# magicat777/Audio-Analyzer-OMEGA

Measured on NVIDIA B200. Metric: stream-seconds of 48 kHz stereo analysed/sec (multi-res FFT+LUFS+TP), higher is better.
Workload: dtype f32 (FFT, combine, K-weighting in a float32 delta-form state, sample peaks of the true-peak meter; its four transforms per frame pair in f16x2; tensor-core GEMM on (hi, lo) half operands with fp32 accumulators for the few-bin resolutions) + f64 (meter statistics)

## Files before the change

### audio-analyzer-omega_b200/csrc/blockdft_tc_kernel.cuh

```cuda
#pragma once
#include <cuda_runtime.h>
#include <cuda_fp16.h>
#include <stdint.h>

namespace o4 {

#ifndef TC_F16
#define TC_F16 1
#endif
constexpr int TC_BM = 128;
constexpr int TC_BN = 256;
constexpr int TC_KC = TC_F16 ? 32 : 16;
constexpr float TC_LO_SCALE = 2048.f;
constexpr int TC_STAGES = 3;
constexpr int TC_TMEM_COLS = 2 * TC_BN;
constexpr int TC_MAX_GROUPS = 64;
#ifndef TC_EXPERIMENT_KS
#define TC_EXPERIMENT_KS 2
#endif
#define TC_PG TC_STAGES
constexpr int TC_THREADS = 64 * TC_STAGES;
constexpr int TC_WARP_MMA = TC_THREADS / 32;
constexpr int TC_WARP_B = TC_WARP_MMA + 1;
constexpr int TC_WARP_EPI = TC_WARP_MMA + 2;
constexpr int TC_EPI_WARPS = 8;
constexpr int TC_CTA_THREADS = 32 * (TC_WARP_EPI + TC_EPI_WARPS);
static_assert(TC_WARP_EPI % 4 == 0, "epilogue warp w must own TMEM lane quarter w % 4");
constexpr int TC_A_BYTES = TC_BM * 64;
constexpr int TC_B_BYTES = TC_BN * 64;
constexpr int TC_STAGE_BYTES = 2 * TC_A_BYTES + 2 * TC_B_BYTES;
constexpr int TC_XROW = 17;
constexpr int TC_SPAD = 15;
constexpr int TC_STRIP_BYTES = (128 + 2 * TC_SPAD) * TC_XROW * 8;

struct BlockDftTcArgs {
    const float* x;
    long long ch_stride;
    int hop;
    int n_ch;
    int j0, nb;
    int n_halves;
    int n_tiles;
    const uint8_t* Eimg;
    const float* row_inv;
    float e_inv;
    float* Q;
    int qs;
    float2* X;
    int n_frames;
    int nkx;
    short gB[TC_MAX_GROUPS];
    short gX[TC_MAX_GROUPS];
    short gN[TC_MAX_GROUPS];
    short gS[TC_MAX_GROUPS];
};
#ifdef TC_TIMELINE
__device__ long long tc_tl[64][16];
#define TC_STAMP(cond, i) do { if ((cond) && (blockIdx.x & 3) == 0 && (blockIdx.x >> 2) < 64) tc_tl[blockIdx.x >> 2][i] = clock64(); } while (0)
#else
#define TC_STAMP(cond, i) do { } while (0)
#endif

__host__ __device__ __forceinline__ int tc_sw64_offset(int row, int c) {
    return (row >> 3) * 512 + (row & 7) * 64 + ((c ^ ((row >> 1) & 3)) << 4);
}

__device__ __forceinline__ uint32_t tc_smem_u32(const void* p) { return (uint32_t)__cvta_generic_to_shared(p); }

__device__ __forceinline__ void tc_mbar_init(uint64_t* bar, int count) {
    asm volatile("mbarrier.init.shared::cta.b64 [%0], %1;" ::"r"(tc_smem_u32(bar)), "r"(count) : "memory");
}
__device__ __forceinline__ void tc_mbar_expect_tx(uint64_t* bar, uint32_t bytes) {
    asm volatile("mbarrier.arrive.expect_tx.shared::cta.b64 _, [%0], %1;" ::"r"(tc_smem_u32(bar)), "r"(bytes) : "memory");
}
__device__ __forceinline__ void tc_mbar_wait(uint64_t* bar, uint32_t parity) {
    const uint32_t a = tc_smem_u32(bar);
    uint32_t done = 0;
    while (!done) {
        asm volatile(
            "{\n\t.reg .pred p;\n\t"
            "mbarrier.try_wait.parity.shared::cta.b64 p, [%1], %2;\n\t"
            "selp.u32 %0, 1, 0, p;\n\t}"
            : "=r"(done) : "r"(a), "r"(parity) : "memory");
    }
}
__device__ __forceinline__ void tc_bulk_g2s(void* dst, const void* src, uint32_t bytes, uint64_t* bar) {
    asm volatile("cp.async.bulk.shared::cluster.global.mbarrier::complete_tx::bytes [%0], [%1], %2, [%3];"
                 ::"r"(tc_smem_u32(dst)), "l"(src), "r"(bytes), "r"(tc_smem_u32(bar)) : "memory");
}

__device__ __forceinline__ uint64_t tc_desc_sw64(uint32_t smem_addr) {
    uint64_t d = 0;
    d |= (uint64_t)((smem_addr >> 4) & 0x3FFF);
    d |= (uint64_t)1 << 16;
    d |= (uint64_t)(512 >> 4) << 32;
    d |= (uint64_t)1 << 46;
    d |= (uint64_t)4 << 61;
    return d;
}

constexpr uint32_t TC_FMT = TC_F16 ? 0u : 2u;
constexpr uint32_t TC_IDESC = (1u << 4) | (TC_FMT << 7) | (TC_FMT << 10) | ((uint32_t)(TC_BN >> 3) << 17) | ((128u >> 4) << 24);

__device__ __forceinline__ void tc_mma(uint32_t tmem_d, uint64_t da, uint64_t db, uint32_t accumulate) {
    asm volatile(
        "{\n\t.reg .pred p;\n\t"
        "setp.ne.b32 p, %4, 0;\n\t"
#if TC_F16
        "tcgen05.mma.cta_group::1.kind::f16 [%0], %1, %2, %3, p;\n\t}"
#else
        "tcgen05.mma.cta_group::1.kind::tf32 [%0], %1, %2, %3, p;\n\t}"
#endif

        ::"r"(tmem_d), "l"(da), "l"(db), "r"(TC_IDESC), "r"(accumulate) : "memory");
}
__device__ __forceinline__ void tc_commit(uint64_t* bar) {
    asm volatile("tcgen05.commit.cta_group::1.mbarrier::arrive::one.shared::cluster.b64 [%0];" ::"r"(tc_smem_u32(bar)) : "memory");
}

__device__ __forceinline__ void tc_tmem_ld32(uint32_t taddr, uint32_t (&v)[32]) {
    asm volatile(
        "tcgen05.ld.sync.aligned.32x32b.x32.b32 "
        "{%0, %1, %2, %3, %4, %5, %6, %7, %8, %9, %10, %11, %12, %13, %14, %15, "
        "%16, %17, %18, %19, %20, %21, %22, %23, %24, %25, %26, %27, %28, %29, %30, %31}, [%32];"
        : "=r"(v[0]), "=r"(v[1]), "=r"(v[2]), "=r"(v[3]), "=r"(v[4]), "=r"(v[5]), "=r"(v[6]), "=r"(v[7]),
          "=r"(v[8]), "=r"(v[9]), "=r"(v[10]), "=r"(v[11]), "=r"(v[12]), "=r"(v[13]), "=r"(v[14]), "=r"(v[15]),
          "=r"(v[16]), "=r"(v[17]), "=r"(v[18]), "=r"(v[19]), "=r"(v[20]), "=r"(v[21]), "=r"(v[22]), "=r"(v[23]),
          "=r"(v[24]), "=r"(v[25]), "=r"(v[26]), "=r"(v[27]), "=r"(v[28]), "=r"(v[29]), "=r"(v[30]), "=r"(v[31])
        : "r"(taddr) : "memory");
}

__device__ __forceinline__ void tc_mbar_arrive(uint64_t* bar) {
    asm volatile("mbarrier.arrive.shared::cta.b64 _, [%0];" ::"r"(tc_smem_u32(bar)) : "memory");
}

__device__ __forceinline__ void tc_split_h2(float a0, float a1, uint32_t& hi, uint32_t& lo) {
    const __half2 h = __floats2half2_rn(a0, a1);
    const float2 hf = __half22float2(h);
    const __half2 l = __floats2half2_rn((a0 - hf.x) * TC_LO_SCALE, (a1 - hf.y) * TC_LO_SCALE);
    hi = *reinterpret_cast<const uint32_t*>(&h);
    lo = *reinterpret_cast<const uint32_t*>(&l);
}
__device__ __forceinline__ float tc_acc(uint32_t v, uint32_t c, float rs) {
#if TC_F16
    return fmaf(__uint_as_float(c), 1.f / TC_LO_SCALE, __uint_as_float(v)) * rs;
#else
    return __uint_as_float(v) + __uint_as_float(c);
#endif
}
__device__ __forceinline__ float hop_row_scale(float m) {
    int e = (int)((__float_as_uint(m) >> 23) & 0xffu);
    float inv = 1.f;
    if (m > 0.f && e < 255) {
        e = e > 250 ? 250 : e;
        inv = __uint_as_float((uint32_t)(e + 1) << 23);
    }
    return inv;
}
struct HopScaleArgs { const float* x; long long ch_stride; int hop, n_ch, j0, nb, ncols; float* inv; };
__global__ void __launch_bounds__(256)
hopblock_scale_kernel(const HopScaleArgs a) {
    const int lane = threadIdx.x & 31;
    const long long row = (long long)blockIdx.x * 8 + (threadIdx.x >> 5);
    if (row >= (long long)a.n_ch * a.ncols) return;
    const int ch = (int)(row / a.ncols), j = (int)(row % a.ncols);
    const float4* px = reinterpret_cast<const float4*>(a.x + (long long)ch * a.ch_stride + ((long long)a.j0 + j) * a.hop);
    float m = 0.f;
    for (int i = lane; i < a.hop / 4; i += 32) {
        const float4 v = __ldg(px + i);
        m = fmaxf(fmaxf(m, fmaxf(fabsf(v.x), fabsf(v.y))), fmaxf(fabsf(v.z), fabsf(v.w)));
    }
#pragma unroll
    for (int o = 16; o > 0; o >>= 1) m = fmaxf(m, __shfl_xor_sync(0xffffffffu, m, o));
    if (lane == 0) a.inv[(size_t)ch * a.nb + j] = hop_row_scale(m);
}


template <int B>
__device__ __forceinline__ void tc_frame_sums(const BlockDftTcArgs& a, const float2* S, int r, int row0, int ch, int nbin, int xb0,
                                              int shift = -1) {
    constexpr int PER = 16 / B;
#pragma unroll
    for (int task = 0; task < 2; ++task) {
        if (task == 1 && r >= B - 1) break;
        const int R = task == 0 ? r : 128 + r;
        const long long f = (long long)a.j0 + row0 + R + (shift > 0 ? shift : 0);
        if (f < 0 || f >= a.n_frames) continue;
        const bool whole = (R - B + 1 >= 0) && (R <= 127) && shift < 0;
        const float2* Sf = S + (R - B + 1 + TC_SPAD) * TC_XROW;
#pragma unroll
        for (int q = 0; q < PER; ++q) {
            if (q >= nbin) break;
            float2 u[B];
#pragma unroll
            for (int b = 0; b < B; ++b) u[b] = Sf[b * TC_XROW + q * B + b];
#pragma unroll
            for (int w = B / 2; w > 0; w >>= 1)
#pragma unroll
                for (int b = 0; b < w; ++b) { u[b].x += u[b + w].x; u[b].y += u[b + w].y; }
            float2* dst = a.X + ((size_t)ch * a.nkx + xb0 + q) * a.n_frames + f;
            if (whole) *dst = u[0];
            else { atomicAdd(&dst->x, u[0].x); atomicAdd(&dst->y, u[0].y); }
        }
    }
}

__global__ void __launch_bounds__(TC_CTA_THREADS, 1)
blockdft_tc_kernel(const __grid_constant__ BlockDftTcArgs a) {
    extern __shared__ __align__(16) uint8_t tc_smem_raw[];
    uint8_t* tiles = tc_smem_raw + ((1024u - (tc_smem_u32(tc_smem_raw) & 1023u)) & 1023u);
    float2* S_all = reinterpret_cast<float2*>(tiles + TC_STAGES * TC_STAGE_BYTES);
    uint64_t* bar_a = reinterpret_cast<uint64_t*>(tiles + TC_STAGES * TC_STAGE_BYTES + (TC_EPI_WARPS / 4) * TC_STRIP_BYTES);
    uint64_t* bar_b = bar_a + TC_STAGES;
    uint64_t* bar_m = bar_b + TC_STAGES;
    uint64_t* bar_full = bar_m + TC_STAGES;
    uint64_t* bar_empty = bar_full + 1;
    uint32_t* tmem_slot = reinterpret_cast<uint32_t*>(bar_empty + 1);

    const int tid = threadIdx.x, warp = tid >> 5, lane = tid & 31;
    const int tiles_per_ch = (a.nb + TC_BM - 1) / TC_BM;
    const int n_kc = a.hop / TC_KC;

    if (warp == TC_WARP_B && lane == 0) {
        for (int s = 0; s < TC_STAGES; ++s) {
            tc_mbar_init(bar_a + s, TC_THREADS / 32 / TC_PG); tc_mbar_init(bar_b + s, 1); tc_mbar_init(bar_m + s, 1);
        }
        tc_mbar_init(bar_full, 1);
        tc_mbar_init(bar_empty, TC_EPI_WARPS);
        asm volatile("fence.mbarrier_init.release.cluster;" ::: "memory");
    }
    if (warp == 0) {
        __syncwarp();
        asm volatile("tcgen05.alloc.cta_group::1.sync.aligned.shared::cta.b32 [%0], %1;" ::"r"(tc_smem_u32(tmem_slot)), "n"(TC_TMEM_COLS) : "memory");
        asm volatile("tcgen05.relinquish_alloc_permit.cta_group::1.sync.aligned;" ::: "memory");
    }
    asm volatile("tcgen05.fence::before_thread_sync;" ::: "memory");
    __syncthreads();
    asm volatile("tcgen05.fence::after_thread_sync;" ::: "memory");
    const uint32_t tmem = *tmem_slot;

    if (warp == TC_WARP_B) {
        if (lane == 0) {
            int kcg = 0;
            for (int tile = blockIdx.x; tile < a.n_tiles; tile += gridDim.x) {
                const uint8_t* eimg = a.Eimg + (size_t)(tile % a.n_halves) * n_kc * 2 * TC_B_BYTES;
                for (int kb = 0; kb < n_kc; ++kb, ++kcg) {
                    const int sb = kcg % TC_STAGES;
                    if (kcg >= TC_STAGES) tc_mbar_wait(bar_m + sb, (uint32_t)(kcg / TC_STAGES - 1) & 1);
#ifdef TC_EXPERIMENT_B_DIV
                    tc_mbar_expect_tx(bar_b + sb, 2 * TC_B_BYTES / TC_EXPERIMENT_B_DIV);
                    tc_bulk_g2s(tiles + sb * TC_STAGE_BYTES + 2 * TC_A_BYTES, eimg + (size_t)kb * 2 * TC_B_BYTES, 2 * TC_B_BYTES / TC_EXPERIMENT_B_DIV, bar_b + sb);
#else
                    tc_mbar_expect_tx(bar_b + sb, 2 * TC_B_BYTES);
                    tc_bulk_g2s(tiles + sb * TC_STAGE_BYTES + 2 * TC_A_BYTES, eimg + (size_t)kb * 2 * TC_B_BYTES, 2 * TC_B_BYTES, bar_b + sb);
#endif
                }
            }
        }
    } else if (warp == TC_WARP_MMA) {
        if (lane == 0) {
            int kcg = 0, it = 0;
            for (int tile = blockIdx.x; tile < a.n_tiles; tile += gridDim.x, ++it) {
                TC_STAMP(it == 1, 0);
                TC_STAMP(it == 2, 6);
                if (it > 0) {
                    tc_mbar_wait(bar_empty, (uint32_t)(it - 1) & 1);
                    asm volatile("tcgen05.fence::after_thread_sync;" ::: "memory");
                }
                for (int kc = 0; kc < n_kc; ++kc, ++kcg) {
                    const int s = kcg % TC_STAGES;
                    const uint32_t use = (uint32_t)(kcg / TC_STAGES);
                    tc_mbar_wait(bar_a + s, use & 1);
                    tc_mbar_wait(bar_b + s, use & 1);
                    asm volatile("tcgen05.fence::after_thread_sync;" ::: "memory");
                    TC_STAMP(it == 1 && kc == 0, 1);
                    const uint32_t sa = tc_smem_u32(tiles + s * TC_STAGE_BYTES);
#pragma unroll
                    for (int ks = 0; ks < TC_EXPERIMENT_KS; ++ks) {
                        const uint64_t d_ahi = tc_desc_sw64(sa + ks * 32);
                        const uint64_t d_alo = tc_desc_sw64(sa + TC_A_BYTES + ks * 32);
                        const uint64_t d_bhi = tc_desc_sw64(sa + 2 * TC_A_BYTES + ks * 32);
                        const uint64_t d_blo = tc_desc_sw64(sa + 2 * TC_A_BYTES + TC_B_BYTES + ks * 32);
                        tc_mma(tmem, d_ahi, d_bhi, (kc | ks) != 0);
                        tc_mma(tmem + TC_BN, d_ahi, d_blo, (kc | ks) != 0);
                        tc_mma(tmem + TC_BN, d_alo, d_bhi, 1);
                    }
                    tc_commit(bar_m + s);
                }
                tc_commit(bar_full);
                TC_STAMP(it == 1, 2);
            }
        }
    } else if (warp < TC_WARP_MMA) {
        constexpr int PGT = TC_THREADS / TC_PG;
        constexpr int NQ = TC_BM * 4 / PGT;
        constexpr int PF4 = TC_F16 ? 2 : 1;
        const int pg = tid / PGT, tg = tid % PGT;
        int a_off[NQ];
#pragma unroll
        for (int q = 0; q < NQ; ++q) a_off[q] = tc_sw64_offset((tg + PGT * q) >> 2, (tg + PGT * q) & 3);
        int it = 0;
        for (int tile = blockIdx.x; tile < a.n_tiles; tile += gridDim.x, ++it) {
            const int bid = tile / a.n_halves;
            const int row0 = (bid % tiles_per_ch) * TC_BM;
            const int ch = bid / tiles_per_ch;
            const float* xa = a.x + (long long)ch * a.ch_stride + (long long)a.j0 * a.hop;
            const float4* a_src[NQ];
            float sc[NQ];
#pragma unroll
            for (int q = 0; q < NQ; ++q) {
                const int p = tg + PGT * q;
                int r = row0 + (p >> 2);
                if (r >= a.nb) r = a.nb - 1;
                a_src[q] = reinterpret_cast<const float4*>(xa + (long long)r * a.hop) + (p & 3) * PF4;
#if TC_F16
                sc[q] = __ldg(a.row_inv + (size_t)ch * a.nb + r);
#else
                sc[q] = 1.f;
#endif
            }
#if TC_F16
#pragma unroll
            for (int q = 0; q < NQ; ++q) sc[q] = __uint_as_float(0x7F000000u - __float_as_uint(sc[q]));
#endif
            const int kcg0 = it * n_kc;
            for (int kc = ((pg - kcg0) % TC_PG + TC_PG) % TC_PG; kc < n_kc; kc += TC_PG) {
                const int kcg = kcg0 + kc;
                const int s = kcg % TC_STAGES;
                uint8_t* st = tiles + s * TC_STAGE_BYTES;
                float4 cur[NQ][PF4];
#ifndef TC_EXPERIMENT_NO_LDG
#pragma unroll
                for (int q = 0; q < NQ; ++q)
#pragma unroll
                    for (int h = 0; h < PF4; ++h) cur[q][h] = __ldg(a_src[q] + kc * (TC_KC / 4) + h);
#else
#pragma unroll
                for (int q = 0; q < NQ; ++q)
#pragma unroll
                    for (int h = 0; h < PF4; ++h) cur[q][h] = make_float4(0.f, 0.f, 0.f, 0.f);
#endif
                if (kcg >= TC_STAGES) tc_mbar_wait(bar_m + s, (uint32_t)(kcg / TC_STAGES - 1) & 1);
#pragma unroll
                for (int q = 0; q < NQ; ++q) {
#if TC_F16
                    uint4 hi, lo;
                    tc_split_h2(cur[q][0].x * sc[q], cur[q][0].y * sc[q], hi.x, lo.x);
                    tc_split_h2(cur[q][0].z * sc[q], cur[q][0].w * sc[q], hi.y, lo.y);
                    tc_split_h2(cur[q][1].x * sc[q], cur[q][1].y * sc[q], hi.z, lo.z);
                    tc_split_h2(cur[q][1].z * sc[q], cur[q][1].w * sc[q], hi.w, lo.w);
                    *reinterpret_cast<uint4*>(st + a_off[q]) = hi;
                    *reinterpret_cast<uint4*>(st + TC_A_BYTES + a_off[q]) = lo;
#else
                    float4 hi, lo;
                    hi.x = __uint_as_float(__float_as_uint(cur[q][0].x) & 0xFFFFE000u); lo.x = cur[q][0].x - hi.x;
                    hi.y = __uint_as_float(__float_as_uint(cur[q][0].y) & 0xFFFFE000u); lo.y = cur[q][0].y - hi.y;
                    hi.z = __uint_as_float(__float_as_uint(cur[q][0].z) & 0xFFFFE000u); lo.z = cur[q][0].z - hi.z;
                    hi.w = __uint_as_float(__float_as_uint(cur[q][0].w) & 0xFFFFE000u); lo.w = cur[q][0].w - hi.w;
                    *reinterpret_cast<float4*>(st + a_off[q]) = hi;
                    *reinterpret_cast<float4*>(st + TC_A_BYTES + a_off[q]) = lo;
#endif
                }
                asm volatile("fence.proxy.async.shared::cta;" ::: "memory");
                __syncwarp();
                if (lane == 0) tc_mbar_arrive(bar_a + s);
            }
        }
    } else {
        const int quad = warp & 3, grp = (warp - TC_WARP_EPI) >> 2;
        const int r = quad * 32 + lane;
        constexpr int NCG = TC_BN / 32 / (TC_EPI_WARPS / 4);
        const uint32_t taddr0 = tmem + ((uint32_t)(quad * 32) << 16) + (uint32_t)(grp * NCG * 32);
        float2* S = S_all + grp * (TC_STRIP_BYTES / 8);
        for (int i = (tid - TC_WARP_EPI * 32) & 127; i < TC_SPAD * TC_XROW; i += 128) {
            S[i] = make_float2(0.f, 0.f);
            S[(128 + TC_SPAD) * TC_XROW + i] = make_float2(0.f, 0.f);
        }
        int it = 0;
        for (int tile = blockIdx.x; tile < a.n_tiles; tile += gridDim.x, ++it) {
            const int half = tile % a.n_halves;
            const int bid = tile / a.n_halves;
            const int row0 = (bid % tiles_per_ch) * TC_BM;
            const int ch = bid / tiles_per_ch;
            const int row = row0 + r;
            float rs = 1.f;
#if TC_F16
            rs = __ldg(a.row_inv + (size_t)ch * a.nb + (row < a.nb ? row : a.nb - 1)) * a.e_inv;
#endif
            float* qrow = a.X ? nullptr : a.Q + ((size_t)ch * a.nb + (row < a.nb ? row : 0)) * a.qs + half * TC_BN;
            tc_mbar_wait(bar_full, (uint32_t)it & 1);
            asm volatile("tcgen05.fence::after_thread_sync;" ::: "memory");
            TC_STAMP(it == 1 && tid == TC_WARP_EPI * 32, 3);
            uint32_t v[32], c[32];
            tc_tmem_ld32(taddr0, v);
            tc_tmem_ld32(taddr0 + TC_BN, c);
#pragma unroll 1
            for (int cg = 0; cg < NCG; ++cg) {
                TC_STAMP(it == 1 && cg == 2 && tid == TC_WARP_EPI * 32, 8);
                asm volatile("tcgen05.wait::ld.sync.aligned;" ::: "memory");
                TC_STAMP(it == 1 && cg == 2 && tid == TC_WARP_EPI * 32, 9);
                const int gi = half * (TC_BN / 32) + grp * NCG + cg;
                const int B = a.X ? a.gB[gi] : 0;
#ifdef TC_EXPERIMENT_NO_EPI
                const bool live = false;
#else
                const bool live = B > 0;
#endif
                if (a.X) {
                    if (live) {
#pragma unroll
                        for (int i = 0; i < 16; ++i)
                            S[(r + TC_SPAD) * TC_XROW + i] = make_float2(tc_acc(v[2 * i], c[2 * i], rs), tc_acc(v[2 * i + 1], c[2 * i + 1], rs));
                    }
                } else if (row < a.nb) {
                    float4* dst = reinterpret_cast<float4*>(qrow + (grp * NCG + cg) * 32);
#pragma unroll
                    for (int i = 0; i < 8; ++i)
                        dst[i] = make_float4(tc_acc(v[4 * i], c[4 * i], rs), tc_acc(v[4 * i + 1], c[4 * i + 1], rs),
                                             tc_acc(v[4 * i + 2], c[4 * i + 2], rs), tc_acc(v[4 * i + 3], c[4 * i + 3], rs));
                }
                TC_STAMP(it == 1 && cg == 2 && tid == TC_WARP_EPI * 32, 10);
                if (cg + 1 < NCG) {
                    tc_tmem_ld32(taddr0 + (uint32_t)((cg + 1) * 32), v);
                    tc_tmem_ld32(taddr0 + (uint32_t)(TC_BN + (cg + 1) * 32), c);
                } else {
                    asm volatile("tcgen05.fence::before_thread_sync;" ::: "memory");
                    __syncwarp();
                    if (lane == 0) tc_mbar_arrive(bar_empty);
                    TC_STAMP(it == 1 && tid == TC_WARP_EPI * 32, 4);
                }
                if (a.X) {
                    TC_STAMP(it == 1 && cg == 2 && tid == TC_WARP_EPI * 32, 11);
                    asm volatile("bar.sync %0, 128;" ::"r"(grp + 1) : "memory");
                    TC_STAMP(it == 1 && cg == 2 && tid == TC_WARP_EPI * 32, 12);
                    if (live) {
                        const int nbin = a.gN[gi], xb0 = a.gX[gi];
                        if (B == 16) tc_frame_sums<16>(a, S, r, row0, ch, nbin, xb0, a.gS[gi]);
                        else if (B == 8) tc_frame_sums<8>(a, S, r, row0, ch, nbin, xb0);
                        else if (B == 4) tc_frame_sums<4>(a, S, r, row0, ch, nbin, xb0);
                        else tc_frame_sums<2>(a, S, r, row0, ch, nbin, xb0);
                    }
                    TC_STAMP(it == 1 && cg == 2 && tid == TC_WARP_EPI * 32, 13);
                    asm volatile("bar.sync %0, 128;" ::"r"(grp + 1) : "memory");
                    TC_STAMP(it == 1 && cg == 2 && tid == TC_WARP_EPI * 32, 14);
                }
            }
            TC_STAMP(it == 1 && tid == TC_WARP_EPI * 32, 5);
        }
    }
    asm volatile("tcgen05.fence::before_thread_sync;" ::: "memory");
    __syncthreads();
    if (warp == 0)
        asm volatile("tcgen05.dealloc.cta_group::1.sync.aligned.b32 %0, %1;" ::"r"(tmem), "n"(TC_TMEM_COLS) : "memory");
}

inline size_t blockdft_tc_smem_bytes() { return (size_t)TC_STAGES * TC_STAGE_BYTES + (TC_EPI_WARPS / 4) * TC_STRIP_BYTES + (3 * TC_STAGES + 2) * 8 + 16 + 1024; }

}
```

### audio-analyzer-omega_b200/csrc/kweight32_kernel.cuh

```cuda
#pragma once
#include <cuda_runtime.h>
#include "kweight_kernel.cuh"
#include "blockdft_tc_kernel.cuh"

namespace o4 {

struct Kw32Sec {
    float b0, a2, gamma, bb;
    float phi[5][4];
    float c16[4], c17[4];
    float g[KW_SUBMAX][2];
    float2 ga0[16], ga1[16];
};

struct Kweight32Args {
    const float* x;
    long long ch_stride, frame_stride, frame_off0;
    int n_ch, n_frames, first_frame, frames_per_warp;
    const float* hann;
    double* lufs_out;
    int rms_gate, _align;
    float* hop_inv;
    int hop_inv_nb, hop_inv_j0;
    Kw32Sec s[2];
};

__device__ __forceinline__ float2 kw32_mat(const float* m, float2 s) {
    return make_float2(fmaf(m[0], s.x, m[1] * s.y), fmaf(m[2], s.x, m[3] * s.y));
}

struct Kw32R { float r0; float2 a[16]; float2 b[16]; };

__device__ __forceinline__ float& kwr(Kw32R& q, int i) {
    if (i == 0) return q.r0;
    if (i <= 16) return q.a[i - 1].x;
    if (i <= 32) return q.b[i - 17].x;
    if (i <= 48) return q.b[i - 33].y;
    return q.a[i - 49].y;
}
__device__ __forceinline__ float2 bc2(float v) { return make_float2(v, v); }

template <bool BACKWARD>
__device__ __forceinline__ void kw32_pass(Kw32R& q, const Kw32Sec& c, int lane) {
    const int pos = BACKWARD ? 31 - lane : lane;
    const float b0 = c.b0, a2 = c.a2, ngamma = -c.gamma, bb = c.bb;
    float xa_in, dxa_in;
    {
        const float p1 = BACKWARD ? __shfl_down_sync(0xffffffffu, kwr(q, 0), 1) : __shfl_up_sync(0xffffffffu, kwr(q, KW_L - 1), 1);
        const float p2 = BACKWARD ? __shfl_down_sync(0xffffffffu, kwr(q, 1), 1) : __shfl_up_sync(0xffffffffu, kwr(q, KW_L - 2), 1);
        const float x0 = BACKWARD ? kwr(q, KW_L - 1) : kwr(q, 0);
        xa_in = pos == 0 ? x0 : p1;
        dxa_in = pos == 0 ? 0.f : p1 - p2;
    }
    const float2 s0 = make_float2(-b0 * xa_in, 0.f);
    float2 xaA, dxaA, xaB, dxaB;
    if (!BACKWARD) {
        xaA = make_float2(xa_in, kwr(q, 48)); dxaA = make_float2(dxa_in, kwr(q, 48) - kwr(q, 47));
        xaB = make_float2(kwr(q, 16), kwr(q, 32)); dxaB = make_float2(kwr(q, 16) - kwr(q, 15), kwr(q, 32) - kwr(q, 31));
    } else {
        xaA = make_float2(kwr(q, 17), xa_in); dxaA = make_float2(kwr(q, 17) - kwr(q, 18), dxa_in);
        xaB = make_float2(kwr(q, 33), kwr(q, 49)); dxaB = make_float2(kwr(q, 33) - kwr(q, 34), kwr(q, 49) - kwr(q, 50));
    }
    float2 zA = bc2(0.f), dA = bc2(0.f), yA = make_float2(b0 * xaA.x, b0 * xaA.y);
    float2 zB = bc2(0.f), dB = bc2(0.f), yB = make_float2(b0 * xaB.x, b0 * xaB.y);
    if (!BACKWARD) {
        const float x = q.r0;
        const float t = fmaf(a2, dA.x, dxaA.x);
        const float d = fmaf(ngamma, yA.x, t);
        const float z = fmaf(bb, d, zA.x);
        const float y = fmaf(b0, x, z);
        dxaA.x = x - xaA.x; xaA.x = x; zA.x = z; dA.x = d; yA.x = y;
        q.r0 = y;
    }
    const float2 A2 = bc2(a2), NG = bc2(ngamma), BB = bc2(bb), B0 = bc2(b0);
#pragma unroll
    for (int n = 0; n < 16; ++n) {
        const int k = BACKWARD ? 15 - n : n;
        {
            const float2 x = q.a[k];
            const float2 t = __ffma2_rn(A2, dA, dxaA);
            const float2 d = __ffma2_rn(NG, yA, t);
            const float2 z = __ffma2_rn(BB, d, zA);
            const float2 y = __ffma2_rn(B0, x, z);
            dxaA = __fadd2_rn(x, make_float2(-xaA.x, -xaA.y)); xaA = x; zA = z; dA = d; yA = y;
            q.a[k] = y;
        }
        {
            const float2 x = q.b[k];
            const float2 t = __ffma2_rn(A2, dB, dxaB);
            const float2 d = __ffma2_rn(NG, yB, t);
            const float2 z = __ffma2_rn(BB, d, zB);
            const float2 y = __ffma2_rn(B0, x, z);
            dxaB = __fadd2_rn(x, make_float2(-xaB.x, -xaB.y)); xaB = x; zB = z; dB = d; yB = y;
            q.b[k] = y;
        }
    }
    if (BACKWARD) {
        const float x = q.r0;
        const float t = fmaf(a2, dA.x, dxaA.x);
        const float d = fmaf(ngamma, yA.x, t);
        const float z = fmaf(bb, d, zA.x);
        const float y = fmaf(b0, x, z);
        zA.x = z; dA.x = d;
        q.r0 = y;
    }
    float2 e[KW_NSUB];
    if (!BACKWARD) { e[0] = make_float2(zA.x, dA.x); e[1] = make_float2(zB.x, dB.x); e[2] = make_float2(zB.y, dB.y); e[3] = make_float2(zA.y, dA.y); }
    else           { e[0] = make_float2(zA.y, dA.y); e[1] = make_float2(zB.y, dB.y); e[2] = make_float2(zB.x, dB.x); e[3] = make_float2(zA.x, dA.x); }
    float2 v = e[0];
#pragma unroll
    for (int m = 1; m < KW_NSUB; ++m) {
        const int j = BACKWARD ? KW_NSUB - 1 - m : m;
        const float* cm = (kw_off(j + 1) - kw_off(j) == 17) ? c.c17 : c.c16;
        const float2 w = kw32_mat(cm, v);
        v = make_float2(w.x + e[m].x, w.y + e[m].y);
    }
    if (pos == 0) {
        const float2 w = kw32_mat(c.phi[0], s0);
        v.x += w.x; v.y += w.y;
    }
#pragma unroll
    for (int jj = 0; jj < 5; ++jj) {
        const int dd = 1 << jj;
        const float rx = BACKWARD ? __shfl_down_sync(0xffffffffu, v.x, dd) : __shfl_up_sync(0xffffffffu, v.x, dd);
        const float ry = BACKWARD ? __shfl_down_sync(0xffffffffu, v.y, dd) : __shfl_up_sync(0xffffffffu, v.y, dd);
        if (pos >= dd) {
            const float2 w = kw32_mat(c.phi[jj], make_float2(rx, ry));
            v.x += w.x; v.y += w.y;
        }
    }
    float2 sin[KW_NSUB];
    sin[0].x = BACKWARD ? __shfl_down_sync(0xffffffffu, v.x, 1) : __shfl_up_sync(0xffffffffu, v.x, 1);
    sin[0].y = BACKWARD ? __shfl_down_sync(0xffffffffu, v.y, 1) : __shfl_up_sync(0xffffffffu, v.y, 1);
    if (pos == 0) sin[0] = s0;
#pragma unroll
    for (int m = 1; m < KW_NSUB; ++m) {
        const int jp = BACKWARD ? KW_NSUB - m : m - 1;
        const float* cm = (kw_off(jp + 1) - kw_off(jp) == 17) ? c.c17 : c.c16;
        const float2 w = kw32_mat(cm, sin[m - 1]);
        sin[m] = make_float2(w.x + e[m - 1].x, w.y + e[m - 1].y);
    }
    const float2 s_c0 = BACKWARD ? sin[3] : sin[0], s_c1 = BACKWARD ? sin[2] : sin[1];
    const float2 s_c2 = BACKWARD ? sin[1] : sin[2], s_c3 = BACKWARD ? sin[0] : sin[3];
    const float2 SXA = make_float2(s_c0.x, s_c3.x), SYA = make_float2(s_c0.y, s_c3.y);
    const float2 SXB = make_float2(s_c1.x, s_c2.x), SYB = make_float2(s_c1.y, s_c2.y);
    if (!BACKWARD) {
        q.r0 = fmaf(c.g[0][0], s_c0.x, fmaf(c.g[0][1], s_c0.y, q.r0));
#pragma unroll
        for (int k = 0; k < 16; ++k) {
            q.a[k] = __ffma2_rn(c.ga0[k], SXA, __ffma2_rn(c.ga1[k], SYA, q.a[k]));
            q.b[k] = __ffma2_rn(bc2(c.g[k][0]), SXB, __ffma2_rn(bc2(c.g[k][1]), SYB, q.b[k]));
        }
    } else {
#pragma unroll
        for (int k = 0; k < 16; ++k) {
            const float2 G0 = bc2(c.g[15 - k][0]), G1 = bc2(c.g[15 - k][1]);
            q.a[k] = __ffma2_rn(G0, SXA, __ffma2_rn(G1, SYA, q.a[k]));
            q.b[k] = __ffma2_rn(G0, SXB, __ffma2_rn(G1, SYB, q.b[k]));
        }
        q.r0 = fmaf(c.g[16][0], s_c0.x, fmaf(c.g[16][1], s_c0.y, q.r0));
    }
}

__device__ __forceinline__ void kw32_odd_pad(Kw32R& q, int lane) {
    if (lane == 0) {
#pragma unroll
        for (int j = 0; j < KW_PAD; ++j) kwr(q, j) = 2.f * kwr(q, KW_PAD) - kwr(q, 2 * KW_PAD - j);
    }
    if (lane == 31) {
        constexpr int E = KW_LAST - KW_PAD;
#pragma unroll
        for (int j = 0; j < KW_PAD; ++j) kwr(q, E + 1 + j) = 2.f * kwr(q, E) - kwr(q, E - 1 - j);
#pragma unroll
        for (int i = KW_LAST + 1; i < KW_L; ++i) kwr(q, i) = kwr(q, KW_LAST);
    }
}

__device__ __forceinline__ void kw32_fill_slack(Kw32R& q, int lane) {
    if (lane == 31) {
#pragma unroll
        for (int i = KW_LAST + 1; i < KW_L; ++i) kwr(q, i) = kwr(q, KW_LAST);
    }
}

__device__ __forceinline__ void kw32_zero_pads(Kw32R& q, int lane) {
    if (lane == 0) {
#pragma unroll
        for (int i = 0; i < KW_PAD; ++i) kwr(q, i) = 0.f;
    }
    if (lane == 31) {
#pragma unroll
        for (int i = KW_LAST - KW_PAD + 1; i < KW_L; ++i) kwr(q, i) = 0.f;
    }
}

constexpr int KW32_WARPS = 4;
#ifndef KW32_MIN_BLOCKS
#define KW32_MIN_BLOCKS 3
#endif

__global__ void __launch_bounds__(KW32_WARPS * 32, KW32_MIN_BLOCKS)
kweight32_kernel(const __grid_constant__ Kweight32Args a) {
    extern __shared__ __align__(16) unsigned char smem_raw[];
    float* hann_x = reinterpret_cast<float*>(smem_raw);
    float* stage_all = hann_x + 32 * KW_L;
    const int lane = threadIdx.x & 31;
    const int warp = threadIdx.x >> 5;
    float* stg = stage_all + warp * KW_STG;

    for (int p = threadIdx.x; p < 32 * KW_L; p += blockDim.x) {
        const int n = p - KW_PAD;
        hann_x[p] = (n >= 0 && n < KW_W) ? a.hann[n] : 0.f;
    }
    __syncthreads();

    const int frames_per_cta = a.frames_per_warp * KW32_WARPS;
    const int tiles_per_ch = (a.n_frames + frames_per_cta - 1) / frames_per_cta;
    const int ch = blockIdx.x / tiles_per_ch;
    const int tile = blockIdx.x % tiles_per_ch;

    for (int it = 0; it < a.frames_per_warp; ++it) {
        const int f = tile * frames_per_cta + it * KW32_WARPS + warp;
        if (f >= a.n_frames || f < a.first_frame) continue;
        const long long off = (long long)ch * a.ch_stride + a.frame_off0 + (long long)f * a.frame_stride;

        const float4* px = reinterpret_cast<const float4*>(a.x + off);
        float4* s4 = reinterpret_cast<float4*>(stg + KW_PAD + KW_STG_SHIFT);
        float4 tmp[KW_W / 4 / 32];
#pragma unroll
        for (int j = 0; j < KW_W / 4 / 32; ++j) tmp[j] = __ldg(px + lane + 32 * j);
        if (a.hop_inv) {
            float m = 0.f;
#pragma unroll
            for (int j = 3 * KW_W / 4 / 4 / 32; j < KW_W / 4 / 32; ++j)
                m = fmaxf(fmaxf(m, fmaxf(fabsf(tmp[j].x), fabsf(tmp[j].y))), fmaxf(fabsf(tmp[j].z), fabsf(tmp[j].w)));
#pragma unroll
            for (int o = 16; o > 0; o >>= 1) m = fmaxf(m, __shfl_xor_sync(0xffffffffu, m, o));
            if (lane == 0) a.hop_inv[(size_t)ch * a.hop_inv_nb + (f - a.hop_inv_j0)] = hop_row_scale(m);
        }
        if (lane < KW_PAD) stg[KW_STG_SHIFT + lane] = 0.f;
        if (lane < KW_SLACK + KW_PAD + KW_STG_SHIFT) stg[KW_STG_SHIFT + KW_PAD + KW_W + lane] = 0.f;
#pragma unroll
        for (int j = 0; j < KW_W / 4 / 32; ++j) s4[lane + 32 * j] = tmp[j];
        __syncwarp();
        float* sl = stg + KW_STG_SHIFT + KW_L * lane;
        const float* hl = hann_x + KW_L * lane;
        Kw32R r;
        float sumsq = 0.f;
#pragma unroll
        for (int i = 0; i < KW_L; ++i) {
            const float xv = sl[i] * hl[i];
            sumsq = fmaf(xv, xv, sumsq);
            kwr(r, i) = xv;
        }
        __syncwarp();
#pragma unroll
        for (int o = 16; o > 0; o >>= 1) sumsq += __shfl_xor_sync(0xffffffffu, sumsq, o);
        const bool gated = a.rms_gate && sqrtf(sumsq * (1.f / KW_W)) < 1e-6f;

        double ms = 0.0;
        if (!gated) {
#ifdef KW32_UNROLL_SECTIONS
#pragma unroll
#else
#pragma unroll 1
#endif
            for (int si = 0; si < 2; ++si) {
                const Kw32Sec& c = a.s[si];
                kw32_odd_pad(r, lane);
                kw32_pass<false>(r, c, lane);
                kw32_fill_slack(r, lane);
                kw32_pass<true>(r, c, lane);
                if (si == 0) {
                    kw32_zero_pads(r, lane);
#pragma unroll
                    for (int i = 0; i < KW_L; ++i) sl[i] = kwr(r, i);
                }
            }
            kw32_zero_pads(r, lane);
            float acc = 0.f;
#pragma unroll
            for (int i = 0; i < KW_L; ++i) {
                const float fv = sl[i];
                const float w = fmaf(kwr(r, i) - fv, 0.3f, fv);
                acc = fmaf(w, w, acc);
            }
#pragma unroll
            for (int o = 16; o > 0; o >>= 1) acc += __shfl_xor_sync(0xffffffffu, acc, o);
            ms = (double)acc / (double)KW_W;
            __syncwarp();
        }
        if (lane == 0)
            a.lufs_out[(size_t)ch * a.n_frames + f] = (ms > 1e-10) ? (-0.691 + 10.0 * log10(ms)) : -100.0;
    }
}

inline size_t kweight32_smem_bytes() {
    return (size_t)32 * KW_L * sizeof(float) + (size_t)KW32_WARPS * KW_STG * sizeof(float);
}

}
```

### audio-analyzer-omega_b200/csrc/omega4_cuda.cu

```cuda
#include "../../include/omega4_cuda.h"

#include <cuda_runtime.h>
#include <math.h>
#include <stdio.h>
#include <stdlib.h>
#include <string.h>

#include <algorithm>
#include <map>
#include <mutex>
#include <set>
#include <string>
#include <vector>

#include "bars_kernel.cuh"
#include "blockdft_kernel.cuh"
#include "blockdft_tc_kernel.cuh"
#include "fft_core.cuh"
#include "kweight_kernel.cuh"
#include "kweight32_kernel.cuh"
#include "misc_kernels.cuh"
#include "multires_kernel.cuh"
#include "stats_kernel.cuh"
#include "truepeak_kernel.cuh"
#include "truepeak16_kernel.cuh"
#include "waterfall_kernel.cuh"

using namespace o4;

static thread_local std::string g_err;

static int fail(int code, const std::string& msg) {
    g_err = msg;
    return code;
}
#define CK(expr)                                                                                   \
    do {                                                                                           \
        cudaError_t e__ = (expr);                                                                  \
        if (e__ != cudaSuccess) {                                                                  \
            char b__[512];                                                                         \
            snprintf(b__, sizeof b__, "%s failed: %s (%s:%d)", #expr, cudaGetErrorString(e__),     \
                     __FILE__, __LINE__);                                                          \
            return fail(OMEGA4_ERR_CUDA, b__);                                                     \
        }                                                                                          \
    } while (0)

extern "C" const char* omega4_last_error(void) { return g_err.c_str(); }
extern "C" int omega4_abi_version(void) { return OMEGA4_ABI_VERSION; }
extern "C" int omega4_device_count(void) {
    int n = 0;
    if (cudaGetDeviceCount(&n) != cudaSuccess) { cudaGetLastError(); return 0; }
    return n;
}

static int ilog2(int n) { int l = 0; while ((1 << l) < n) ++l; return l; }
static bool is_pow2(int n) { return n > 0 && (n & (n - 1)) == 0; }

struct Twiddles { float2* twM = nullptr; float2* twN = nullptr; float2* tw4W = nullptr; };
static std::mutex g_tw_mu;
static std::map<std::pair<int, int>, Twiddles> g_tw;

static int get_twiddles(int device, int log2m, Twiddles* out) {
    std::lock_guard<std::mutex> lk(g_tw_mu);
    auto key = std::make_pair(device, log2m);
    auto it = g_tw.find(key);
    if (it != g_tw.end()) { *out = it->second; return OMEGA4_OK; }
    const int M = 1 << log2m, N = 2 * M;
    const double two_pi = 6.283185307179586476925287;
    std::vector<float2> a(M), b(M / 2 + 1), c(3 * M + 1);
    for (int e = 0; e < M; ++e) a[e] = make_float2((float)cos(two_pi * e / M), (float)-sin(two_pi * e / M));
    for (int k = 0; k <= M / 2; ++k) b[k] = make_float2((float)cos(two_pi * k / N), (float)-sin(two_pi * k / N));
    for (int j = 0; j <= 3 * M; ++j) c[j] = make_float2((float)cos(two_pi * j / (4.0 * N)), (float)sin(two_pi * j / (4.0 * N)));
    Twiddles t;
    CK(cudaMalloc(&t.twM, a.size() * sizeof(float2)));
    CK(cudaMalloc(&t.twN, b.size() * sizeof(float2)));
    CK(cudaMalloc(&t.tw4W, c.size() * sizeof(float2)));
    CK(cudaMemcpy(t.twM, a.data(), a.size() * sizeof(float2), cudaMemcpyHostToDevice));
    CK(cudaMemcpy(t.twN, b.data(), b.size() * sizeof(float2), cudaMemcpyHostToDevice));
    CK(cudaMemcpy(t.tw4W, c.data(), c.size() * sizeof(float2), cudaMemcpyHostToDevice));
    g_tw[key] = t;
    *out = t;
    return OMEGA4_OK;
}

template <int L>
static int launch_multires_t(const MultiresArgs& a, cudaStream_t s) {
    using S = FftShape<L>;
    const int fpc = a.rounds * S::CONC;
    const long long tiles = (a.n_frames + fpc - 1) / fpc;
    const long long grid = tiles * a.n_ch;
    if (grid <= 0) return OMEGA4_OK;
    if (grid > 2147483647LL) return fail(OMEGA4_ERR_INVALID, "multires grid too large");
    if constexpr (L <= 12) {
        const size_t smem = multires_local_smem_bytes<L>(a.need_cnt, a.n_tb);
        CK(cudaFuncSetAttribute(multires_local_kernel<L>, cudaFuncAttributeMaxDynamicSharedMemorySize, (int)smem));
        multires_local_kernel<L><<<(unsigned)grid, 256, smem, s>>>(a);
    } else {
        const size_t smem = multires_smem_bytes<L>(a.need_cnt);
        CK(cudaFuncSetAttribute(multires_kernel<L>, cudaFuncAttributeMaxDynamicSharedMemorySize, (int)smem));
        multires_kernel<L><<<(unsigned)grid, S::NT, smem, s>>>(a);
    }
    CK(cudaGetLastError());
    return OMEGA4_OK;
}

static int launch_multires(int log2m, const MultiresArgs& a, cudaStream_t s) {
    switch (log2m) {
        case 8: return launch_multires_t<8>(a, s);
        case 9: return launch_multires_t<9>(a, s);
        case 10: return launch_multires_t<10>(a, s);
        case 11: return launch_multires_t<11>(a, s);
        case 12: return launch_multires_t<12>(a, s);
        case 13: return launch_multires_t<13>(a, s);
        case 14: return launch_multires_t<14>(a, s);
    }
    return fail(OMEGA4_ERR_UNSUPPORTED, "fft size must be a power of two in 512 .. 32768");
}

static int default_rounds(int n_frames, int conc) {
    int r = 16;
    while (r > 1 && (long long)r * conc > n_frames) r >>= 1;
    return r;
}

static void fill_truepeak_steps(TruePeakArgs* t) {
    const double two_pi = 6.283185307179586476925287;
    for (int p = 1; p <= 3; ++p) {
        for (int j = 0; j < 16; ++j) {
            const int jj = j < 8 ? j : j - 16;
            t->step[p - 1][j] = make_float2((float)cos(two_pi * p * jj / 64.0), (float)sin(two_pi * p * jj / 64.0));
        }
        t->nyq[p - 1] = (float)cos(two_pi * p / 8.0);
    }
}

static int launch_truepeak(const TruePeakArgs& a, cudaStream_t s) {
    constexpr int L = 11;
    using S = FftShape<L>;
    const size_t smem = truepeak_smem_bytes<L>();
    CK(cudaFuncSetAttribute(truepeak_kernel<L>, cudaFuncAttributeMaxDynamicSharedMemorySize, (int)smem));
    const int ppc = a.rounds * S::CONC;
    const int n_pairs = (a.n_frames + 1) / 2;
    const long long grid = (long long)((n_pairs + ppc - 1) / ppc) * a.n_ch;
    if (grid <= 0) return OMEGA4_OK;
    if (grid > 2147483647LL) return fail(OMEGA4_ERR_INVALID, "truepeak grid too large");
    truepeak_kernel<L><<<(unsigned)grid, S::NT, smem, s>>>(a);
    CK(cudaGetLastError());
    return OMEGA4_OK;
}

static int launch_truepeak16(const TruePeakArgs& a, cudaStream_t s) {
    constexpr int L = 11;
    using S = FftShape<L>;
    const size_t smem = truepeak16_smem_bytes<L>();
    CK(cudaFuncSetAttribute(truepeak16_kernel<L>, cudaFuncAttributeMaxDynamicSharedMemorySize, (int)smem));
    const int ppc = a.rounds * S::CONC;
    const int n_pairs = (a.n_frames + 1) / 2;
    const long long grid = (long long)((n_pairs + ppc - 1) / ppc) * a.n_ch;
    if (grid <= 0) return OMEGA4_OK;
    if (grid > 2147483647LL) return fail(OMEGA4_ERR_INVALID, "truepeak grid too large");
    truepeak16_kernel<L><<<(unsigned)grid, S::NT, smem, s>>>(a);
    CK(cudaGetLastError());
    return OMEGA4_OK;
}

template <bool F64, bool WT>
static int launch_kweight_t(const KweightArgs& a, cudaStream_t s) {
    const size_t smem = kweight_smem_bytes();
    CK(cudaFuncSetAttribute(kweight_kernel<F64, WT>, cudaFuncAttributeMaxDynamicSharedMemorySize, (int)smem));
    const int fpc = a.frames_per_warp * KW_WARPS;
    const long long grid = (long long)((a.n_frames + fpc - 1) / fpc) * a.n_ch;
    if (grid <= 0) return OMEGA4_OK;
    if (grid > 2147483647LL) return fail(OMEGA4_ERR_INVALID, "kweight grid too large");
    kweight_kernel<F64, WT><<<(unsigned)grid, KW_WARPS * 32, smem, s>>>(a);
    CK(cudaGetLastError());
    return OMEGA4_OK;
}

static int launch_kweight(const KweightArgs& a, cudaStream_t s) {
    if (a.x_is_f64) return a.weighted_out ? launch_kweight_t<true, true>(a, s) : launch_kweight_t<true, false>(a, s);
    return a.weighted_out ? launch_kweight_t<false, true>(a, s) : launch_kweight_t<false, false>(a, s);
}

static int launch_kweight32(const Kweight32Args& a, cudaStream_t s) {
    const size_t smem = kweight32_smem_bytes();
    CK(cudaFuncSetAttribute(kweight32_kernel, cudaFuncAttributeMaxDynamicSharedMemorySize, (int)smem));
    const int fpc = a.frames_per_warp * KW32_WARPS;
    const long long grid = (long long)((a.n_frames + fpc - 1) / fpc) * a.n_ch;
    if (grid <= 0) return OMEGA4_OK;
    if (grid > 2147483647LL) return fail(OMEGA4_ERR_INVALID, "kweight grid too large");
    kweight32_kernel<<<(unsigned)grid, KW32_WARPS * 32, smem, s>>>(a);
    CK(cudaGetLastError());
    return OMEGA4_OK;
}

static int launch_stats(const StatsArgs& a, cudaStream_t s) {
    if (a.n_ch <= 0) return OMEGA4_OK;
    if (!a.fresh && a.n_frames == 1 && a.first_frame == 0 && !getenv("OMEGA4_STATS_WALK")) {
        stats_push1_kernel<<<a.n_ch, ST_P1_THREADS, 0, s>>>(a);
    } else if (a.fresh) {
        const size_t smem = stats_smem_bytes<false>();
        CK(cudaFuncSetAttribute(stats_kernel<false>, cudaFuncAttributeMaxDynamicSharedMemorySize, (int)smem));
        stats_kernel<false><<<a.n_ch, ST_THREADS, smem, s>>>(a);
    } else {
        const size_t smem = stats_smem_bytes<true>();
        CK(cudaFuncSetAttribute(stats_kernel<true>, cudaFuncAttributeMaxDynamicSharedMemorySize, (int)smem));
        stats_kernel<true><<<a.n_ch, ST_THREADS, smem, s>>>(a);
    }
    CK(cudaGetLastError());
    return OMEGA4_OK;
}

static int launch_s16_convert(const int16_t* in, long long stream_stride, int il, int n_streams, long long n_frames,
                              float* out, long long out_stride, cudaStream_t s) {
    if (n_streams <= 0 || n_frames <= 0) return OMEGA4_OK;
    if (n_streams > 65535) return fail(OMEGA4_ERR_INVALID, "too many streams for one int16 conversion launch (max 65535)");
    const long long per_stream = n_frames * il;
    dim3 grid((unsigned)((per_stream + 1023) / 1024), (unsigned)n_streams);
    s16_deinterleave_kernel<<<grid, 256, 0, s>>>(in, stream_stride, il, n_frames, out, out_stride);
    CK(cudaGetLastError());
    return OMEGA4_OK;
}

static void mat2_mul(const double* a, const double* b, double* c) {
    double r[4] = {a[0] * b[0] + a[1] * b[2], a[0] * b[1] + a[1] * b[3],
                   a[2] * b[0] + a[3] * b[2], a[2] * b[1] + a[3] * b[3]};
    memcpy(c, r, sizeof r);
}

static void build_biquad(const double* b, const double* a, int order, KwBiquad* q) {
    memset(q, 0, sizeof *q);
    const double a0 = a[0];
    q->b0 = b[0] / a0; q->b1 = b[1] / a0; q->b2 = order >= 2 ? b[2] / a0 : 0.0;
    q->a1 = a[1] / a0; q->a2 = order >= 2 ? a[2] / a0 : 0.0;
    q->pad = 3 * (order + 1);
    if (order >= 2) {
        double zi0, zi1;
        const double m00 = 1.0 + q->a1, m01 = -1.0, m10 = q->a2, m11 = 1.0;
        const double r0 = q->b1 - q->a1 * q->b0, r1 = q->b2 - q->a2 * q->b0;
        const double det = m00 * m11 - m01 * m10;
        zi0 = (r0 * m11 - m01 * r1) / det;
        zi1 = (m00 * r1 - m10 * r0) / det;
        q->yi0 = -zi1 / q->a2;
        q->yi1 = (-zi0 + q->a1 * zi1 / q->a2) / q->a2;
    } else {
        const double zi0 = (q->b1 - q->a1 * q->b0) / (1.0 + q->a1);
        q->yi0 = -zi0 / q->a1;
        q->yi1 = 0.0;
    }
    const double Cm[4] = {-q->a1, -q->a2, 1.0, 0.0};
    double P[4] = {Cm[0], Cm[1], Cm[2], Cm[3]};
    for (int i = 0; i < KW_L; ++i) {
        if (i < KW_SUBMAX) { q->g[i][0] = P[0]; q->g[i][1] = P[1]; }
        if (i + 1 == 16) memcpy(q->c16, P, sizeof P);
        if (i + 1 == 17) memcpy(q->c17, P, sizeof P);
        if (i + 1 < KW_L) mat2_mul(Cm, P, P);
    }
    memcpy(q->phi[0], P, sizeof P);
    for (int j = 1; j < 5; ++j) mat2_mul(q->phi[j - 1], q->phi[j - 1], q->phi[j]);
    auto inv_pow = [&](int k, double* out) {
        if (k == 0) { out[0] = 1; out[1] = 0; out[2] = 0; out[3] = 1; return; }
        if (order >= 2) {
            const double det1 = Cm[0] * Cm[3] - Cm[1] * Cm[2];
            const double Ci[4] = {Cm[3] / det1, -Cm[1] / det1, -Cm[2] / det1, Cm[0] / det1};
            double R[4] = {Ci[0], Ci[1], Ci[2], Ci[3]};
            for (int i = 1; i < k; ++i) mat2_mul(Ci, R, R);
            memcpy(out, R, sizeof R);
        } else {
            out[0] = pow(-q->a1, -(double)k); out[1] = 0; out[2] = 0; out[3] = 0;
        }
    };
    inv_pow(KW_PAD - q->pad, q->cinv_f);
    inv_pow(KW_SLACK + KW_PAD - q->pad, q->cinv_b);
}

struct ResInfo {
    int n = 0, log2m = 0, bins = 0;
    float weight = 1.f;
    float* window = nullptr;
    float* binw = nullptr;
    int n_tb = 0;
    int* tb_idx = nullptr;
    int* tb_lo = nullptr;
    float* tb_frac = nullptr;
    int need_lo = 0, need_cnt = 0;
    Twiddles tw;
};

struct SparseRes {
    int r = 0, nk = 0, nt = 0, B = 0, col0 = 0;
    bool td = false;
    int xoff = 0;
    float2* T = nullptr;
    float* kw = nullptr;
    int* tb_pos = nullptr;
};

struct SparseSet {
    int n = 0;
    SparseRes sp[OMEGA4_MAX_RES];
    int of_res[OMEGA4_MAX_RES];
    int cols = 0, qs = 0;
    float* E = nullptr;
    uint8_t* Eimg = nullptr;
    float e_inv = 1.f;
    int n_halves = 0;
    bool fusable = false;
    int nkx = 0;
    short gB[TC_MAX_GROUPS], gX[TC_MAX_GROUPS], gN[TC_MAX_GROUPS], gS[TC_MAX_GROUPS];
    SparseSet() { for (int i = 0; i < OMEGA4_MAX_RES; ++i) of_res[i] = -1; }
    void release() {
        for (int i = 0; i < OMEGA4_MAX_RES; ++i) { cudaFree(sp[i].T); cudaFree(sp[i].kw); cudaFree(sp[i].tb_pos); }
        cudaFree(E); cudaFree(Eimg);
    }
};

struct DevBuf {
    void* p = nullptr;
    size_t cap = 0;
    int ensure(size_t bytes) {
        if (bytes <= cap) return OMEGA4_OK;
        if (p) cudaFree(p);
        p = nullptr; cap = 0;
        CK(cudaMalloc(&p, bytes));
        cap = bytes;
        return OMEGA4_OK;
    }
    void release() { if (p) cudaFree(p); p = nullptr; cap = 0; }
};

struct omega4_bars {
    int device = 0, T = 0, n_valid = 0, p_lo = 0, normalize_max = 0;
    float p_frac = 0.f, scale = 0.8f;
    int* bands = nullptr; float* gain = nullptr; float* sf = nullptr; float* sfc = nullptr;
    DevBuf h_spec, h_out, h_peak, h_state, state_in;
};

static int bars_launch(omega4_bars* b, cudaStream_t s, const float* spec, int n_ch, int n_hops, float* state, int fresh,
                       float* band_values, float* peak_values, DevBuf* state_copy) {
    BarsArgs a;
    memset(&a, 0, sizeof a);
    a.T = b->T; a.n_ch = n_ch; a.n_hops = n_hops; a.n_valid = b->n_valid; a.bands = b->bands; a.gain = b->gain;
    a.sf = b->sf; a.sfc = b->sfc; a.p_lo = b->p_lo; a.p_frac = b->p_frac; a.scale = b->scale;
    a.normalize_max = b->normalize_max; a.fresh = (fresh || !state) ? 1 : 0;
    a.spec = spec; a.bars_out = band_values; a.peaks_out = peak_values; a.state = state;
    const size_t st_bytes = (size_t)n_ch * (1 + b->n_valid) * sizeof(float);
    const size_t smem = bars_smem_bytes(b->T, b->n_valid);
    if (smem > 200 * 1024) return fail(OMEGA4_ERR_UNSUPPORTED, "spectrum too long for the bars kernel");
    if (b->T > 32 * BARS_MAXV) return fail(OMEGA4_ERR_UNSUPPORTED, "spectrum too long for the bars kernel (max 1024 bins)");
    if (b->T <= 512) CK(cudaFuncSetAttribute(bars_kernel<16>, cudaFuncAttributeMaxDynamicSharedMemorySize, (int)smem));
    else CK(cudaFuncSetAttribute(bars_kernel<32>, cudaFuncAttributeMaxDynamicSharedMemorySize, (int)smem));
    a.seg = n_ch >= 1024 ? 4 * BARS_SEG : BARS_SEG;
    const long long grid = (long long)n_ch * ((n_hops + a.seg - 1) / a.seg);
    if (grid > 2147483647LL) return fail(OMEGA4_ERR_INVALID, "bars grid too large");
    if (a.state && !a.fresh && n_hops > a.seg) {
        int rc = state_copy->ensure(st_bytes); if (rc) return rc;
        CK(cudaMemcpyAsync(state_copy->p, a.state, st_bytes, cudaMemcpyDeviceToDevice, s));
        a.state_in = (const float*)state_copy->p;
    }
    if (b->T <= 512) bars_kernel<16><<<(unsigned)grid, BARS_WARPS * 32, smem, s>>>(a);
    else bars_kernel<32><<<(unsigned)grid, BARS_WARPS * 32, smem, s>>>(a);
    CK(cudaGetLastError());
    return OMEGA4_OK;
}

struct BarsReq {
    omega4_bars* b = nullptr;
    float* band_values = nullptr; float* peak_values = nullptr; float* state = nullptr;
    int fresh = 1;
};

struct KernelTime { char name[32]; cudaEvent_t e0, e1; };

struct SideCtx {
    cudaStream_t side = nullptr;
    cudaEvent_t ev_fork = nullptr, ev_tp = nullptr, ev_join = nullptr;
    int ensure() {
        if (side) return OMEGA4_OK;
        CK(cudaStreamCreateWithFlags(&side, cudaStreamNonBlocking));
        CK(cudaEventCreateWithFlags(&ev_fork, cudaEventDisableTiming));
        CK(cudaEventCreateWithFlags(&ev_tp, cudaEventDisableTiming));
        CK(cudaEventCreateWithFlags(&ev_join, cudaEventDisableTiming));
        return OMEGA4_OK;
    }
    void release() {
        if (side) cudaStreamDestroy(side);
        if (ev_fork) cudaEventDestroy(ev_fork);
        if (ev_tp) cudaEventDestroy(ev_tp);
        if (ev_join) cudaEventDestroy(ev_join);
        side = nullptr; ev_fork = ev_tp = ev_join = nullptr;
    }
};

struct omega4_plan {
    int device = 0;
    int sample_rate = 48000, hop = 512, n_res = 0, T = 0, W = OMEGA4_METER_WINDOW;
    double gate = -70.0;
    ResInfo res[OMEGA4_MAX_RES];
    bool disjoint = true;
    int* csr_ptr = nullptr; int* csr_res = nullptr; int* csr_lo = nullptr; float* csr_frac = nullptr;
    double* hann64 = nullptr;
    float* hann32 = nullptr;
    KwBiquad kw_default[2];
    KwBiquad kw[4];
    int kw_nsec = 2, kw_blend = 1, kw_gate = 1;
    double kw_gain = 1.0;
    Twiddles tw_meter;
    float2* tp_rot = nullptr;
    unsigned* tp_rot_h = nullptr;
    SparseSet set_cc;
    SparseSet set_tc;
    bool tensor_default = true;
    DevBuf scratch_lufs, scratch_tp, scratch_mag[OMEGA4_MAX_RES], scratch_q, scratch_f32, scratch_comb, scratch_bstate, scratch_inv;
    DevBuf h_in, h_comb, h_meters, h_state, h_mag[OMEGA4_MAX_RES], h_f64a, h_f64b, h_f64c;
    struct Slot {
        cudaStream_t s = nullptr;
        DevBuf in, in16, comb, met, lufs, tp, state, q, mag[OMEGA4_MAX_RES];
        DevBuf bars, peaks, bstate, bstate_copy;
        SideCtx sc;
    };
#ifndef OMEGA4_HOST_SLOTS
#define OMEGA4_HOST_SLOTS 4
#endif
    static constexpr int N_SLOTS = OMEGA4_HOST_SLOTS;
    Slot slots[N_SLOTS];
    size_t host_chunk_bytes = (size_t)1024 << 20;
    SideCtx sc;
    long long launches = 0;
    std::vector<KernelTime> times;
    size_t n_times = 0;
};

static void set_weighting_k(omega4_plan* p) {
    p->kw[0] = p->kw_default[0]; p->kw[1] = p->kw_default[1];
    p->kw_nsec = 2; p->kw_blend = 1; p->kw_gate = 1; p->kw_gain = 1.0;
}

static double max_pole_radius(const KwBiquad& q) {
    if (q.a2 == 0.0) return fabs(q.a1);
    const double disc = q.a1 * q.a1 - 4.0 * q.a2;
    if (disc < 0.0) return sqrt(q.a2);
    return fmax(fabs(-q.a1 + sqrt(disc)), fabs(-q.a1 - sqrt(disc))) * 0.5;
}

static void to_float(const KwBiquad& s, KwBiquadF* d) {
    d->b0 = (float)s.b0; d->b1 = (float)s.b1; d->b2 = (float)s.b2; d->a1 = (float)s.a1; d->a2 = (float)s.a2;
    d->yi0 = (float)s.yi0; d->yi1 = (float)s.yi1; d->pad = s.pad; d->_align = 0;
    for (int j = 0; j < 5; ++j) for (int e = 0; e < 4; ++e) d->phi[j][e] = (float)s.phi[j][e];
    for (int e = 0; e < 4; ++e) {
        d->cinv_f[e] = (float)s.cinv_f[e]; d->cinv_b[e] = (float)s.cinv_b[e];
        d->c16[e] = (float)s.c16[e]; d->c17[e] = (float)s.c17[e];
    }
    for (int i = 0; i < KW_SUBMAX; ++i) { d->g[i][0] = (float)s.g[i][0]; d->g[i][1] = (float)s.g[i][1]; }
}

static bool is_highpass_biquad(const KwBiquad& q) {
    return q.pad == 9 && q.a2 != 0.0 && fabs(q.b1 + 2.0 * q.b0) <= 1e-12 * fabs(q.b0) && fabs(q.b2 - q.b0) <= 1e-12 * fabs(q.b0);
}

static void build_kw32(const KwBiquad& q, Kw32Sec* o) {
    const double alpha = 1.0 + q.a1 + q.a2, beta = 1.0 - q.a2;
    const double bb = -q.b0 * beta, gamma = alpha / bb;
    o->b0 = (float)q.b0; o->a2 = (float)q.a2; o->gamma = (float)gamma; o->bb = (float)bb;
    const double M[4] = {1.0 - alpha, bb * q.a2, -gamma, q.a2};
    double P[4] = {M[0], M[1], M[2], M[3]};
    for (int i = 0; i < KW_L; ++i) {
        if (i < KW_SUBMAX) { o->g[i][0] = (float)P[0]; o->g[i][1] = (float)P[1]; }
        if (i + 1 == 16) for (int e = 0; e < 4; ++e) o->c16[e] = (float)P[e];
        if (i + 1 == 17) for (int e = 0; e < 4; ++e) o->c17[e] = (float)P[e];
        if (i + 1 < KW_L) mat2_mul(M, P, P);
    }
    for (int k = 0; k < 16; ++k) {
        o->ga0[k] = make_float2(o->g[k + 1][0], o->g[k][0]);
        o->ga1[k] = make_float2(o->g[k + 1][1], o->g[k][1]);
    }
    double Q[4] = {P[0], P[1], P[2], P[3]};
    for (int j = 0; j < 5; ++j) {
        for (int e = 0; e < 4; ++e) o->phi[j][e] = (float)Q[e];
        mat2_mul(Q, Q, Q);
    }
}

static bool use_kweight32(const omega4_plan* p) {
    return p->W == KW_W && p->kw_nsec == 2 && p->kw_blend && p->kw_gain == 1.0 && is_highpass_biquad(p->kw[0]) &&
           is_highpass_biquad(p->kw[1]) && !getenv("OMEGA4_KW_F64");
}

static void fill_weighting(const omega4_plan* p, KweightArgs* k) {
    k->n_sec = p->kw_nsec; k->blend = p->kw_blend; k->rms_gate = p->kw_gate; k->gain = p->kw_gain;
    for (int i = 0; i < p->kw_nsec; ++i) { k->f[i] = p->kw[i]; to_float(p->kw[i], &k->ff[i]); }
    int from = p->kw_nsec;
    while (from > 1 && max_pole_radius(p->kw[from - 1]) < 0.95) --from;
    k->f32_from = getenv("OMEGA4_KW_F64") ? p->kw_nsec : from;
}

static int upload(void** dst, const void* src, size_t bytes) {
    CK(cudaMalloc(dst, bytes ? bytes : 1));
    if (bytes) CK(cudaMemcpy(*dst, src, bytes, cudaMemcpyHostToDevice));
    return OMEGA4_OK;
}

static size_t boff_of(const omega4_plan_desc* d, int r) {
    size_t o = 0;
    for (int i = 0; i < r; ++i) o += (size_t)d->fft_sizes[i] / 2 + 1;
    return o;
}

static int build_sparse_set(omega4_plan* p, const omega4_plan_desc* d, const std::vector<std::vector<int>>& idx,
                            const std::vector<std::vector<int>>& lo, bool tensor, SparseSet* set) {
    const int H = d->hop;
    if ((H % (tensor ? TC_KC : BD_KC)) != 0) return OMEGA4_OK;
    const int max_cols = tensor ? TC_MAX_GROUPS * 32 : 128;
    const bool allow_td = tensor && !getenv("OMEGA4_BLOCKDFT_FD");
    int order[OMEGA4_MAX_RES];
    for (int r = 0; r < d->n_res; ++r) order[r] = r;
    for (int i = 0; i < d->n_res; ++i)
        for (int j = i + 1; j < d->n_res; ++j)
            if (p->res[order[j]].n > p->res[order[i]].n) { int t = order[i]; order[i] = order[j]; order[j] = t; }
    std::vector<std::vector<float>> ecols;
    int cols = 0;
    size_t woff2[OMEGA4_MAX_RES];
    { size_t o = 0; for (int r = 0; r < d->n_res; ++r) { woff2[r] = o; o += d->fft_sizes[r]; } }
    for (int oi = 0; oi < d->n_res; ++oi) {
        const int r = order[oi];
        const ResInfo& ri = p->res[r];
        const int N = ri.n;
        if (N % H != 0 || N / H < 2 || N / H > 64) continue;
        std::vector<int> bins;
        for (int l : lo[r]) if (l >= 0) { bins.push_back(l); bins.push_back(l + 1); }
        std::sort(bins.begin(), bins.end());
        bins.erase(std::unique(bins.begin(), bins.end()), bins.end());
        if (bins.empty()) continue;
        const float* w = d->windows + woff2[r];
        const double two_pi = 6.283185307179586476925287;
        const int nk = (int)bins.size();
        const double fft_cost = 2.5 * N * (ri.log2m + 1);
        if (allow_td && N / H <= 64 && (double)(2 * nk * (N / H)) * H <= 6.6 * fft_cost &&
            ((cols + 31) & ~31) + 2 * nk * (N / H) <= max_cols) {
            cols = (cols + 31) & ~31;
            SparseRes& sp = set->sp[set->n];
            sp.r = r; sp.nk = nk; sp.nt = N / H; sp.B = N / H; sp.col0 = cols; sp.td = true;
            const int rc_cols = 2 * nk * sp.B;
            std::vector<float> ec((size_t)H * rc_cols);
            std::vector<float> kw(nk);
            for (int ki = 0; ki < nk; ++ki) {
                kw[ki] = d->bin_weights ? d->bin_weights[boff_of(d, r) + bins[ki]] : 1.f;
                for (int b = 0; b < sp.B; ++b)
                    for (int n2 = 0; n2 < H; ++n2) {
                        const int i = H * b + n2;
                        const long long ph = ((long long)bins[ki] * i) % N;
                        const double ang = -two_pi * (double)ph / (double)N;
                        ec[(size_t)n2 * rc_cols + 2 * (ki * sp.B + b)] = (float)((double)w[i] * cos(ang));
                        ec[(size_t)n2 * rc_cols + 2 * (ki * sp.B + b) + 1] = (float)((double)w[i] * sin(ang));
                    }
            }
            std::vector<int> pos(idx[r].size(), -1);
            for (size_t j = 0; j < lo[r].size(); ++j)
                if (lo[r][j] >= 0) pos[j] = (int)(std::lower_bound(bins.begin(), bins.end(), lo[r][j]) - bins.begin());
            int rc = upload((void**)&sp.kw, kw.data(), kw.size() * sizeof(float)); if (rc) return rc;
            rc = upload((void**)&sp.tb_pos, pos.data(), pos.size() * sizeof(int)); if (rc) return rc;
            set->of_res[r] = set->n++;
            ecols.push_back(std::move(ec));
            cols += rc_cols;
            cols = (cols + 31) & ~31;
            continue;
        }
        const double phi = 6.283185307179586476925287 / (double)(N - 1);
        double G[3][4] = {{0}};
        for (int i = 0; i < N; ++i) {
            const double c[3] = {1.0, cos(phi * i), cos(2.0 * phi * i)};
            for (int u = 0; u < 3; ++u) { for (int v = 0; v < 3; ++v) G[u][v] += c[u] * c[v]; G[u][3] += c[u] * (double)w[i]; }
        }
        bool singular = false;
        for (int u = 0; u < 3 && !singular; ++u) {
            int piv = u;
            for (int v = u + 1; v < 3; ++v) if (fabs(G[v][u]) > fabs(G[piv][u])) piv = v;
            if (fabs(G[piv][u]) < 1e-9) { singular = true; break; }
            if (piv != u) for (int c2 = 0; c2 < 4; ++c2) { double t = G[u][c2]; G[u][c2] = G[piv][c2]; G[piv][c2] = t; }
            for (int v = 0; v < 3; ++v) {
                if (v == u) continue;
                const double f = G[v][u] / G[u][u];
                for (int c2 = 0; c2 < 4; ++c2) G[v][c2] -= f * G[u][c2];
            }
        }
        if (singular) continue;
        double am[3] = {G[0][3] / G[0][0], G[1][3] / G[1][1], G[2][3] / G[2][2]};
        double resid = 0.0;
        for (int i = 0; i < N; ++i) {
            const double fit = am[0] + am[1] * cos(phi * i) + am[2] * cos(2.0 * phi * i);
            resid = fmax(resid, fabs(fit - (double)w[i]));
        }
        if (resid > 1.5e-7) continue;
        int tm[5]; double tc[5]; int nt = 0;
        tm[nt] = 0; tc[nt] = am[0]; ++nt;
        for (int m = 1; m <= 2; ++m)
            if (fabs(am[m]) > 1e-9) { tm[nt] = m; tc[nt] = 0.5 * am[m]; ++nt; tm[nt] = -m; tc[nt] = 0.5 * am[m]; ++nt; }
        const int rc_cols = 2 * nk * nt;
        if (!tensor && (double)rc_cols * H * 2.0 > fft_cost) continue;
        if (tensor && (double)rc_cols * H > 6.6 * fft_cost) continue;
        if (cols + rc_cols > max_cols) continue;
        SparseRes& sp = set->sp[set->n];
        sp.r = r; sp.nk = nk; sp.nt = nt; sp.B = N / H; sp.col0 = cols;
        std::vector<float> ec((size_t)H * rc_cols);
        std::vector<float2> T((size_t)nk * sp.B * nt);
        std::vector<float> kw(nk);
        for (int ki = 0; ki < nk; ++ki) {
            kw[ki] = d->bin_weights ? d->bin_weights[boff_of(d, r) + bins[ki]] : 1.f;
            for (int t = 0; t < nt; ++t) {
                const double th = tm[t] * phi - two_pi * (double)bins[ki] / (double)N;
                for (int n2 = 0; n2 < H; ++n2) {
                    const double ang = fmod(th * n2, two_pi);
                    ec[(size_t)n2 * rc_cols + 2 * (ki * nt + t)] = (float)cos(ang);
                    ec[(size_t)n2 * rc_cols + 2 * (ki * nt + t) + 1] = (float)sin(ang);
                }
                for (int b = 0; b < sp.B; ++b) {
                    const double ang = fmod(th * (double)H * b, two_pi);
                    T[((size_t)ki * sp.B + b) * nt + t] = make_float2((float)(tc[t] * cos(ang)), (float)(tc[t] * sin(ang)));
                }
            }
        }
        std::vector<int> pos(idx[r].size(), -1);
        for (size_t j = 0; j < lo[r].size(); ++j)
            if (lo[r][j] >= 0) pos[j] = (int)(std::lower_bound(bins.begin(), bins.end(), lo[r][j]) - bins.begin());
        int rc = upload((void**)&sp.T, T.data(), T.size() * sizeof(float2)); if (rc) return rc;
        rc = upload((void**)&sp.kw, kw.data(), kw.size() * sizeof(float)); if (rc) return rc;
        rc = upload((void**)&sp.tb_pos, pos.data(), pos.size() * sizeof(int)); if (rc) return rc;
        set->of_res[r] = set->n++;
        ecols.push_back(std::move(ec));
        cols += rc_cols;
    }
    if (set->n == 0) return OMEGA4_OK;
    set->cols = cols;
    if (!tensor) {
        set->qs = cols <= 32 ? 32 : (cols <= 64 ? 64 : 128);
        std::vector<float> E((size_t)H * set->qs, 0.f);
        for (int si = 0; si < set->n; ++si) {
            const SparseRes& sp = set->sp[si];
            const int rc_cols = 2 * sp.nk * sp.nt;
            for (int n2 = 0; n2 < H; ++n2)
                memcpy(&E[(size_t)n2 * set->qs + sp.col0], &ecols[si][(size_t)n2 * rc_cols], rc_cols * sizeof(float));
        }
        return upload((void**)&set->E, E.data(), E.size() * sizeof(float));
    }
    set->n_halves = (cols + TC_BN - 1) / TC_BN;
    set->qs = set->n_halves * TC_BN;
    {
        bool ok = set->n_halves * (TC_BN / 32) <= TC_MAX_GROUPS;
        int xo = 0;
        for (int si = 0; si < set->n; ++si) {
            SparseRes& sp = set->sp[si];
            ok = ok && sp.td && (sp.B == 2 || sp.B == 4 || sp.B == 8 || sp.B == 16 || sp.B == 32 || sp.B == 64) && (sp.col0 % 32) == 0;
            sp.xoff = xo; xo += sp.nk;
        }
        set->nkx = xo;
        for (int g = 0; g < TC_MAX_GROUPS; ++g) { set->gB[g] = 0; set->gX[g] = 0; set->gN[g] = 0; set->gS[g] = -1; }
        if (ok)
            for (int si = 0; si < set->n; ++si) {
                const SparseRes& sp = set->sp[si];
                if (sp.B > 16) {
                    const int parts = sp.B / 16;
                    for (int k0 = 0; k0 < sp.nk; ++k0)
                        for (int pt = 0; pt < parts; ++pt) {
                            const int g = (sp.col0 + 2 * (k0 * sp.B + 16 * pt)) / 32;
                            set->gB[g] = 16; set->gX[g] = (short)(sp.xoff + k0); set->gN[g] = 1;
                            set->gS[g] = (short)(sp.B - 16 * (pt + 1));
                        }
                    continue;
                }
                const int per = 16 / sp.B;
                for (int k0 = 0; k0 < sp.nk; k0 += per) {
                    const int g = (sp.col0 + 2 * k0 * sp.B) / 32;
                    set->gB[g] = (short)sp.B; set->gX[g] = (short)(sp.xoff + k0);
                    set->gN[g] = (short)((sp.nk - k0 < per) ? sp.nk - k0 : per);
                }
            }
        set->fusable = ok && !getenv("OMEGA4_BLOCKDFT_UNFUSED");
    }
    const int nkc = H / TC_KC;
    std::vector<uint8_t> img((size_t)set->n_halves * nkc * 2 * TC_B_BYTES, 0);
#if TC_F16
    float emax = 0.f;
    for (const auto& ec : ecols) for (float v : ec) emax = fmaxf(emax, fabsf(v));
    int eexp = 0;
    if (emax > 0.f) frexpf(emax, &eexp);
    const float escale = ldexpf(1.f, -eexp);
    set->e_inv = ldexpf(1.f, eexp);
#endif
    for (int si = 0; si < set->n; ++si) {
        const SparseRes& sp = set->sp[si];
        const int rc_cols = 2 * sp.nk * sp.nt;
        for (int cc = 0; cc < rc_cols; ++cc) {
            const int col = sp.col0 + cc, h = col / TC_BN, n = col % TC_BN;
            for (int k = 0; k < H; ++k) {
                const float v = ecols[si][(size_t)k * rc_cols + cc];
#if TC_F16
                const float vs = v * escale;
                const __half hh = __float2half_rn(vs);
                const __half hl = __float2half_rn((vs - __half2float(hh)) * TC_LO_SCALE);
                const int kc = k / TC_KC, e = k % TC_KC;
                const size_t base = ((size_t)(h * nkc + kc) * 2) * TC_B_BYTES;
                const int off = tc_sw64_offset(n, e >> 3) + (e & 7) * 2;
                memcpy(&img[base + off], &hh, 2);
                memcpy(&img[base + TC_B_BYTES + off], &hl, 2);
#else
                uint32_t bits; memcpy(&bits, &v, 4); bits &= 0xFFFFE000u;
                float hi; memcpy(&hi, &bits, 4);
                const float lo2 = v - hi;
                const int kc = k / TC_KC, e = k % TC_KC;
                const size_t base = ((size_t)(h * nkc + kc) * 2) * TC_B_BYTES;
                const int off = tc_sw64_offset(n, e >> 2) + (e & 3) * 4;
                memcpy(&img[base + off], &hi, 4);
                memcpy(&img[base + TC_B_BYTES + off], &lo2, 4);
#endif
            }
        }
    }
    return upload((void**)&set->Eimg, img.data(), img.size());
}

static int plan_build(omega4_plan* p, const omega4_plan_desc* d) {
    if (d->n_res < 1 || d->n_res > OMEGA4_MAX_RES) return fail(OMEGA4_ERR_INVALID, "n_res must be 1..8");
    if (d->hop <= 0 || (d->hop % 4) != 0) return fail(OMEGA4_ERR_INVALID, "hop must be a positive multiple of 4");
    if (d->target_bins < 1) return fail(OMEGA4_ERR_INVALID, "target_bins must be >= 1");
    if (d->meter_window != OMEGA4_METER_WINDOW) return fail(OMEGA4_ERR_UNSUPPORTED, "meter_window must be 2048");
    if (!d->fft_sizes || !d->windows || !d->tb_count || !d->res_weight || !d->meter_hann || !d->kw_coeffs)
        return fail(OMEGA4_ERR_INVALID, "plan_desc has NULL tables");
    p->sample_rate = d->sample_rate; p->hop = d->hop; p->n_res = d->n_res; p->T = d->target_bins;
    p->gate = d->gate_threshold;
    std::vector<int> owners(d->target_bins, 0);
    size_t woff = 0, boff = 0, toff = 0;
    std::vector<std::vector<int>> idx(d->n_res), lo(d->n_res);
    std::vector<std::vector<float>> fr(d->n_res);
    for (int r = 0; r < d->n_res; ++r) {
        ResInfo& ri = p->res[r];
        const int n = d->fft_sizes[r];
        if (!is_pow2(n) || n < 512 || n > 32768) return fail(OMEGA4_ERR_UNSUPPORTED, "fft size must be a power of two in 512 .. 32768");
        ri.n = n; ri.log2m = ilog2(n) - 1; ri.bins = n / 2 + 1; ri.weight = d->res_weight[r];
        if (ri.weight <= 0.f) return fail(OMEGA4_ERR_INVALID, "resolution weight must be positive");
        int rc = upload((void**)&ri.window, d->windows + woff, (size_t)n * sizeof(float));
        if (rc) return rc;
        if (d->bin_weights) { rc = upload((void**)&ri.binw, d->bin_weights + boff, (size_t)ri.bins * sizeof(float)); if (rc) return rc; }
        woff += n; boff += ri.bins;
        const int cnt = d->tb_count[r];
        if (cnt < 0) return fail(OMEGA4_ERR_INVALID, "negative tb_count");
        for (int j = 0; j < cnt; ++j) {
            const int ti = d->tb_idx[toff + j], l = d->tb_lo[toff + j];
            if (ti < 0 || ti >= d->target_bins || l < 0 || l + 1 >= ri.bins)
                return fail(OMEGA4_ERR_INVALID, "combine table entry out of range");
            idx[r].push_back(ti); lo[r].push_back(l); fr[r].push_back(d->tb_frac[toff + j]);
            owners[ti]++;
        }
        toff += cnt;
        rc = get_twiddles(p->device, ri.log2m, &ri.tw);
        if (rc) return rc;
    }
    p->disjoint = true;
    for (int t = 0; t < d->target_bins; ++t) if (owners[t] > 1) p->disjoint = false;
    {
        std::vector<int> ptr(d->target_bins + 1, 0), cres, clo;
        std::vector<float> cfr;
        for (int t = 0; t < d->target_bins; ++t) {
            for (int r = 0; r < d->n_res; ++r)
                for (size_t j = 0; j < idx[r].size(); ++j)
                    if (idx[r][j] == t) { cres.push_back(r); clo.push_back(lo[r][j]); cfr.push_back(fr[r][j]); }
            ptr[t + 1] = (int)cres.size();
        }
        int rc = upload((void**)&p->csr_ptr, ptr.data(), ptr.size() * sizeof(int)); if (rc) return rc;
        rc = upload((void**)&p->csr_res, cres.data(), cres.size() * sizeof(int)); if (rc) return rc;
        rc = upload((void**)&p->csr_lo, clo.data(), clo.size() * sizeof(int)); if (rc) return rc;
        rc = upload((void**)&p->csr_frac, cfr.data(), cfr.size() * sizeof(float)); if (rc) return rc;
    }
    for (int r = 0; r < d->n_res; ++r) {
        ResInfo& ri = p->res[r];
        int mn = 1 << 30, mx = -1;
        for (int l : lo[r]) { if (l < mn) mn = l; if (l > mx) mx = l; }
        if (mx >= 0) { ri.need_lo = mn; ri.need_cnt = mx + 2 - mn; } else { ri.need_lo = 0; ri.need_cnt = 0; }
        if (r == 0)
            for (int t = 0; t < d->target_bins; ++t)
                if (owners[t] == 0) { idx[0].push_back(t); lo[0].push_back(-1); fr[0].push_back(0.f); }
        ri.n_tb = (int)idx[r].size();
        int rc = upload((void**)&ri.tb_idx, idx[r].data(), idx[r].size() * sizeof(int)); if (rc) return rc;
        rc = upload((void**)&ri.tb_lo, lo[r].data(), lo[r].size() * sizeof(int)); if (rc) return rc;
        rc = upload((void**)&ri.tb_frac, fr[r].data(), fr[r].size() * sizeof(float)); if (rc) return rc;
    }
    if (p->disjoint) {
        int rc = build_sparse_set(p, d, idx, lo, false, &p->set_cc); if (rc) return rc;
        rc = build_sparse_set(p, d, idx, lo, true, &p->set_tc); if (rc) return rc;
    }
    int rc = upload((void**)&p->hann64, d->meter_hann, (size_t)p->W * sizeof(double)); if (rc) return rc;
    std::vector<float> h32(p->W);
    for (int i = 0; i < p->W; ++i) h32[i] = (float)d->meter_hann[i];
    rc = upload((void**)&p->hann32, h32.data(), h32.size() * sizeof(float)); if (rc) return rc;
    build_biquad(d->kw_coeffs + 0, d->kw_coeffs + 3, 2, &p->kw_default[0]);
    build_biquad(d->kw_coeffs + 6, d->kw_coeffs + 9, 2, &p->kw_default[1]);
    set_weighting_k(p);
    rc = get_twiddles(p->device, ilog2(p->W), &p->tw_meter); if (rc) return rc;
    {
        const int W = p->W;
        std::vector<float2> rot((size_t)3 * W);
        const double two_pi = 6.283185307179586476925287;
        for (int ph = 1; ph <= 3; ++ph)
            for (int k = 0; k < W; ++k) {
                float2 v;
                if (k == W / 2) v = make_float2((float)cos(two_pi * ph / 8.0), 0.f);
                else {
                    const double f = (k < W / 2) ? (double)k : (double)k - W;
                    const double ang = two_pi * f * ph / (4.0 * W);
                    v = make_float2((float)cos(ang), (float)sin(ang));
                }
                rot[(size_t)(ph - 1) * W + k] = v;
            }
        rc = upload((void**)&p->tp_rot, rot.data(), rot.size() * sizeof(float2)); if (rc) return rc;
        std::vector<unsigned> roth(rot.size());
        for (size_t i = 0; i < rot.size(); ++i) {
            const __half2 h = __floats2half2_rn(rot[i].x, rot[i].y);
            memcpy(&roth[i], &h, sizeof(unsigned));
        }
        rc = upload((void**)&p->tp_rot_h, roth.data(), roth.size() * sizeof(unsigned)); if (rc) return rc;
    }
    return OMEGA4_OK;
}

extern "C" omega4_plan* omega4_plan_create(const omega4_plan_desc* desc, int device) {
    if (!desc) { fail(OMEGA4_ERR_INVALID, "desc is NULL"); return nullptr; }
    int ndev = 0;
    if (cudaGetDeviceCount(&ndev) != cudaSuccess || ndev == 0) {
        cudaGetLastError();
        fail(OMEGA4_ERR_NO_DEVICE, "no CUDA device visible: libomega4_cuda has no CPU fallback");
        return nullptr;
    }
    if (device < 0 || device >= ndev) { fail(OMEGA4_ERR_INVALID, "bad device index"); return nullptr; }
    if (cudaSetDevice(device) != cudaSuccess) { fail(OMEGA4_ERR_CUDA, "cudaSetDevice failed"); return nullptr; }
    omega4_plan* p = new omega4_plan();
    p->device = device;
    if (const char* e = getenv("OMEGA4_TENSOR")) p->tensor_default = atoi(e) != 0;
    if (const char* e = getenv("OMEGA4_HOST_CHUNK_MB")) {
        long mb = atol(e);
        if (mb >= 16 && mb <= 16384) p->host_chunk_bytes = (size_t)mb << 20;
    }
    if (plan_build(p, desc) != OMEGA4_OK) { std::string keep = g_err; omega4_plan_destroy(p); g_err = keep; return nullptr; }
    return p;
}

static void stream_ctx_release(omega4_plan* p);

extern "C" void omega4_plan_destroy(omega4_plan* p) {
    if (!p) return;
    cudaSetDevice(p->device);
    stream_ctx_release(p);
    for (int r = 0; r < OMEGA4_MAX_RES; ++r) {
        ResInfo& ri = p->res[r];
        cudaFree(ri.window); cudaFree(ri.binw); cudaFree(ri.tb_idx); cudaFree(ri.tb_lo); cudaFree(ri.tb_frac);
        p->scratch_mag[r].release(); p->h_mag[r].release();
    }
    cudaFree(p->csr_ptr); cudaFree(p->csr_res); cudaFree(p->csr_lo); cudaFree(p->csr_frac);
    cudaFree(p->hann64); cudaFree(p->hann32); cudaFree(p->tp_rot); cudaFree(p->tp_rot_h);
    p->scratch_lufs.release(); p->scratch_tp.release(); p->scratch_q.release(); p->scratch_f32.release(); p->scratch_inv.release();
    p->scratch_comb.release(); p->scratch_bstate.release();
    p->set_cc.release(); p->set_tc.release();
    p->h_in.release(); p->h_comb.release(); p->h_meters.release(); p->h_state.release();
    p->h_f64a.release(); p->h_f64b.release(); p->h_f64c.release();
    for (auto& sl : p->slots) {
        sl.in.release(); sl.comb.release(); sl.met.release(); sl.lufs.release(); sl.tp.release(); sl.state.release();
        sl.q.release(); sl.in16.release(); sl.sc.release();
        sl.bars.release(); sl.peaks.release(); sl.bstate.release(); sl.bstate_copy.release();
        for (auto& m : sl.mag) m.release();
        if (sl.s) cudaStreamDestroy(sl.s);
    }
    for (auto& t : p->times) { cudaEventDestroy(t.e0); cudaEventDestroy(t.e1); }
    p->sc.release();
    cudaGetLastError();
    delete p;
}

extern "C" long long omega4_plan_launches(const omega4_plan* p) { return p ? p->launches : 0; }

extern "C" int omega4_plan_set_weighting(omega4_plan* p, const omega4_weighting* w) {
    if (!p) return fail(OMEGA4_ERR_INVALID, "plan is NULL");
    if (!w) { set_weighting_k(p); return OMEGA4_OK; }
    if (w->n_sections < 0 || w->n_sections > 4) return fail(OMEGA4_ERR_INVALID, "0..4 weighting sections");
    if (w->blend && w->n_sections != 2) return fail(OMEGA4_ERR_INVALID, "the K blend needs exactly two sections");
    KwBiquad tmp[4];
    for (int i = 0; i < w->n_sections; ++i) {
        const int order = w->order[i];
        if (order != 1 && order != 2) return fail(OMEGA4_ERR_UNSUPPORTED, "weighting sections must be first or second order");
        if (w->a[i][0] == 0.0 || w->a[i][1] == 0.0 || (order == 2 && w->a[i][2] == 0.0))
            return fail(OMEGA4_ERR_UNSUPPORTED, "weighting sections need non-zero denominator coefficients");
        build_biquad(w->b[i], w->a[i], order, &tmp[i]);
    }
    for (int i = 0; i < w->n_sections; ++i) p->kw[i] = tmp[i];
    p->kw_nsec = w->n_sections; p->kw_blend = w->blend ? 1 : 0; p->kw_gate = w->rms_gate ? 1 : 0;
    p->kw_gain = w->blend ? 1.0 : w->gain;
    return OMEGA4_OK;
}

struct Bracket {
    omega4_plan* p; cudaStream_t s; bool on; KernelTime* kt = nullptr;
    Bracket(omega4_plan* p_, cudaStream_t s_, bool on_, const char* name) : p(p_), s(s_), on(on_) {
        p->launches++;
        if (!on) return;
        if (p->n_times == p->times.size()) {
            KernelTime t; memset(&t, 0, sizeof t);
            cudaEventCreate(&t.e0); cudaEventCreate(&t.e1);
            p->times.push_back(t);
        }
        kt = &p->times[p->n_times++];
        snprintf(kt->name, sizeof kt->name, "%s", name);
        cudaEventRecord(kt->e0, s);
    }
    ~Bracket() { if (on && kt) cudaEventRecord(kt->e1, s); }
};

extern "C" int omega4_plan_kernel_times(omega4_plan* p, char* names, float* ms, int max_n) {
    if (!p) return fail(OMEGA4_ERR_INVALID, "plan is NULL");
    int n = 0;
    for (size_t i = 0; i < p->n_times && n < max_n; ++i, ++n) {
        float t = 0.f;
        if (cudaEventElapsedTime(&t, p->times[i].e0, p->times[i].e1) != cudaSuccess) { cudaGetLastError(); t = -1.f; }
        if (names) { memcpy(names + 32 * n, p->times[i].name, 32); }
        if (ms) ms[n] = t;
    }
    return n;
}

template <int BN>
static int launch_blockdft_gemm_t(const BlockDftGemmArgs& a, cudaStream_t s) {
    const size_t smem = blockdft_gemm_smem_bytes<BN>();
    CK(cudaFuncSetAttribute(blockdft_gemm_kernel<BN>, cudaFuncAttributeMaxDynamicSharedMemorySize, (int)smem));
    const long long grid = (long long)((a.nb + BD_BM - 1) / BD_BM) * a.n_ch;
    if (grid > 2147483647LL) return fail(OMEGA4_ERR_INVALID, "blockdft grid too large");
    blockdft_gemm_kernel<BN><<<(unsigned)grid, BD_THREADS, smem, s>>>(a);
    CK(cudaGetLastError());
    return OMEGA4_OK;
}

static int launch_blockdft_gemm(int bn, const BlockDftGemmArgs& a, cudaStream_t s) {
    if (a.nb <= 0 || a.n_ch <= 0) return OMEGA4_OK;
    switch (bn) {
        case 32: return launch_blockdft_gemm_t<32>(a, s);
        case 64: return launch_blockdft_gemm_t<64>(a, s);
        case 128: return launch_blockdft_gemm_t<128>(a, s);
    }
    return fail(OMEGA4_ERR_INVALID, "bad blockdft column tile");
}

static int analyze_device(omega4_plan* p, cudaStream_t s, const float* x, long long ch_stride, int n_ch,
                          int n_hops, int hist, float* combined, float* const* mags, float* meters,
                          double* lufs, double* tp, double* state, int flags, DevBuf* qbuf, SideCtx* sc) {
    const bool timing = (flags & OMEGA4_FLAG_TIME_KERNELS) != 0;
    if (timing) p->n_times = 0;
    if (((uintptr_t)x & 15) != 0 || (ch_stride % 4) != 0)
        return fail(OMEGA4_ERR_INVALID, "samples must be 16-byte aligned with ch_stride a multiple of 4");
    const bool want_meters = meters || lufs || tp;
    const bool concurrent = want_meters && (flags & OMEGA4_FLAG_CONCURRENT_METERS);
    const bool stats_aside = !concurrent && meters && combined && !(flags & OMEGA4_FLAG_SERIAL_STATS);
    cudaStream_t ms = s;
    cudaStream_t ss = s;
    if (concurrent || stats_aside) {
        int rc = sc->ensure(); if (rc) return rc;
        ss = sc->side;
    }
    if (concurrent) {
        ms = sc->side;
        CK(cudaEventRecord(sc->ev_fork, s));
        CK(cudaStreamWaitEvent(ms, sc->ev_fork, 0));
    }
    const bool fused = p->disjoint;
    int first[OMEGA4_MAX_RES];
    bool use_sparse[OMEGA4_MAX_RES] = {false};
    bool any_sparse = false;
    const bool tensor = p->set_tc.n > 0 && (p->tensor_default ? !(flags & OMEGA4_FLAG_NO_TENSOR) : (flags & OMEGA4_FLAG_TENSOR) != 0);
    const SparseSet& set = tensor ? p->set_tc : p->set_cc;
    for (int r = 0; r < p->n_res; ++r) {
        use_sparse[r] = combined && fused && set.of_res[r] >= 0 && !(mags && mags[r]) &&
                        !(flags & OMEGA4_FLAG_NO_BLOCKDFT);
        any_sparse = any_sparse || use_sparse[r];
        long long need = (long long)p->res[r].n - hist;
        first[r] = need <= 0 ? 0 : (int)((need + p->hop - 1) / p->hop - 1);
    }
    int sp_j0 = 1 << 30;
    for (int r = 0; r < p->n_res; ++r)
        if (use_sparse[r]) { const int j = first[r] + 1 - set.sp[set.of_res[r]].B; if (j < sp_j0) sp_j0 = j; }
    const int sp_nb = any_sparse ? n_hops - sp_j0 : 0;
    float* row_inv = nullptr;
    int inv_from_kw = -1;
#if TC_F16
    if (tensor && any_sparse && sp_nb > 0) {
        int rc = p->scratch_inv.ensure((size_t)n_ch * sp_nb * sizeof(float)); if (rc) return rc;
        row_inv = (float*)p->scratch_inv.p;
    }
#endif
    if (want_meters) {
        const size_t nser = (size_t)n_ch * n_hops * sizeof(double);
        if (!lufs) { int rc = p->scratch_lufs.ensure(nser); if (rc) return rc; lufs = (double*)p->scratch_lufs.p; }
        if (!tp) { int rc = p->scratch_tp.ensure(nser); if (rc) return rc; tp = (double*)p->scratch_tp.p; }
        long long need = (long long)p->W - hist;
        const int first_m = need <= 0 ? 0 : (int)((need + p->hop - 1) / p->hop - 1);
        if (use_kweight32(p)) {
            Kweight32Args k;
            memset(&k, 0, sizeof k);
            k.x = x; k.ch_stride = ch_stride; k.frame_stride = p->hop;
            k.frame_off0 = (long long)p->hop - p->W;
            k.n_ch = n_ch; k.n_frames = n_hops; k.first_frame = first_m;
            k.frames_per_warp = n_hops >= 64 ? 8 : (n_hops >= 8 ? 2 : 1);
            k.hann = p->hann32; k.lufs_out = lufs; k.rms_gate = p->kw_gate;
            if (row_inv && !concurrent && p->hop * 4 == p->W && first_m < n_hops && !getenv("OMEGA4_NO_SCALE_FOLD")) {
                k.hop_inv = row_inv; k.hop_inv_nb = sp_nb; k.hop_inv_j0 = sp_j0;
                inv_from_kw = first_m;
            }
            build_kw32(p->kw[0], &k.s[0]); build_kw32(p->kw[1], &k.s[1]);
            Bracket b(p, ms, timing, "kweight_lufs");
            int rc = launch_kweight32(k, ms);
            if (rc) return rc;
        } else {
            KweightArgs k;
            memset(&k, 0, sizeof k);
            k.x = x; k.x_is_f64 = 0; k.ch_stride = ch_stride; k.frame_stride = p->hop;
            k.frame_off0 = (long long)p->hop - p->W;
            k.n_ch = n_ch; k.n_frames = n_hops; k.first_frame = first_m;
            k.frames_per_warp = n_hops >= 64 ? 8 : (n_hops >= 8 ? 2 : 1);
            k.hann = p->hann64; k.lufs_out = lufs; k.weighted_out = nullptr;
            fill_weighting(p, &k);
            Bracket b(p, ms, timing, "kweight_lufs");
            int rc = launch_kweight(k, ms);
            if (rc) return rc;
        }
        {
            TruePeakArgs t;
            memset(&t, 0, sizeof t);
            t.x = x; t.x_is_f64 = 0; t.ch_stride = ch_stride; t.frame_stride = p->hop;
            t.frame_off0 = (long long)p->hop - p->W;
            t.n_ch = n_ch; t.n_frames = n_hops; t.first_frame = first_m;
            t.rounds = default_rounds((n_hops + 1) / 2, 2);
            t.window = p->hann32; t.twM = p->tw_meter.twM; t.rot = p->tp_rot; t.rot_h = p->tp_rot_h;
            fill_truepeak_steps(&t);
            t.tp_out = tp;
            Bracket b(p, s, timing, "true_peak");
            const bool exact_tp = (flags & OMEGA4_FLAG_EXACT_TRUE_PEAK) || getenv("OMEGA4_TP_F32");
            int rc = exact_tp ? launch_truepeak(t, s) : launch_truepeak16(t, s);
            if (rc) return rc;
        }
        if (meters) {
            if (concurrent || stats_aside) {
                CK(cudaEventRecord(sc->ev_tp, s));
                CK(cudaStreamWaitEvent(ss, sc->ev_tp, 0));
            }
            StatsArgs st;
            memset(&st, 0, sizeof st);
            st.lufs = lufs; st.tp = tp; st.n_ch = n_ch; st.n_frames = n_hops; st.first_frame = first_m;
            st.gate = p->gate; st.out = meters;
            st.fresh = (state == nullptr) || (flags & OMEGA4_FLAG_FRESH_METERS) ? 1 : 0;
            if (!state) {
                int rc = p->h_state.ensure((size_t)n_ch * ST_STATE * sizeof(double));
                if (rc) return rc;
                state = (double*)p->h_state.p;
            }
            st.state = state;
            Bracket b(p, ss, timing, "meter_stats");
            int rc = launch_stats(st, ss);
            if (rc) return rc;
        }
        if (concurrent || stats_aside) CK(cudaEventRecord(sc->ev_join, ss));
    }
    float* mag_ptr[OMEGA4_MAX_RES];
    for (int r = 0; r < p->n_res; ++r) {
        ResInfo& ri = p->res[r];
        mag_ptr[r] = mags ? mags[r] : nullptr;
        if (combined && !fused && !mag_ptr[r]) {
            int rc = p->scratch_mag[r].ensure((size_t)n_ch * n_hops * ri.bins * sizeof(float));
            if (rc) return rc;
            mag_ptr[r] = (float*)p->scratch_mag[r].p;
        }
        if (!combined && !mag_ptr[r]) continue;
        if (use_sparse[r]) continue;
        MultiresArgs a;
        memset(&a, 0, sizeof a);
        a.x = x; a.ch_stride = ch_stride; a.frame_stride = p->hop; a.frame_off0 = (long long)p->hop - ri.n;
        a.n_ch = n_ch; a.n_frames = n_hops; a.first_frame = first[r];
        a.rounds = default_rounds(n_hops, (1 << ri.log2m) >= 4096 ? 1 : 4096 >> ri.log2m);
        a.window = ri.window; a.binw = ri.binw; a.twM = ri.tw.twM; a.twN = ri.tw.twN;
        a.mag_out = mag_ptr[r]; a.cplx_out = nullptr;
        a.comb_out = (combined && fused) ? combined : nullptr;
        a.T = p->T; a.n_tb = ri.n_tb; a.tb_idx = ri.tb_idx; a.tb_lo = ri.tb_lo; a.tb_frac = ri.tb_frac;
        a.wnum = ri.weight; a.wden = ri.weight;
        a.need_lo = ri.need_lo; a.need_cnt = (combined && fused) ? ri.need_cnt : 0;
        char name[32];
        snprintf(name, sizeof name, "multires_fft_%d", ri.n);
        Bracket b(p, s, timing, name);
        int rc = launch_multires(ri.log2m, a, s);
        if (rc) return rc;
    }
    if (any_sparse) {
        const int j0 = sp_j0, nb = sp_nb;
        const float* Q = nullptr;
        const bool fusedx = tensor && set.fusable;
        if (nb > 0) {
            const size_t qbytes = fusedx ? (size_t)n_ch * set.nkx * n_hops * sizeof(float2)
                                         : (size_t)n_ch * nb * set.qs * sizeof(float);
            int rc = qbuf->ensure(qbytes);
            if (rc) return rc;
            Q = (float*)qbuf->p;
            if (tensor) {
                BlockDftTcArgs g;
                memset(&g, 0, sizeof g);
                g.x = x; g.ch_stride = ch_stride; g.hop = p->hop; g.n_ch = n_ch; g.j0 = j0; g.nb = nb;
                g.n_halves = set.n_halves; g.Eimg = set.Eimg; g.Q = (float*)qbuf->p; g.qs = set.qs;
#if TC_F16
                {
                    HopScaleArgs h;
                    h.x = x; h.ch_stride = ch_stride; h.hop = p->hop; h.n_ch = n_ch; h.j0 = j0; h.nb = nb;
                    h.ncols = inv_from_kw >= 0 ? inv_from_kw - j0 : nb;
                    h.inv = row_inv;
                    g.row_inv = h.inv; g.e_inv = set.e_inv;
                    const long long rows = (long long)n_ch * h.ncols;
                    if (rows > 0) {
                        Bracket b(p, s, timing, "blockdft_row_scale");
                        hopblock_scale_kernel<<<(unsigned)((rows + 7) / 8), 256, 0, s>>>(h);
                        CK(cudaGetLastError());
                    }
                }
#endif
                if (fusedx) {
                    g.X = (float2*)qbuf->p; g.n_frames = n_hops; g.nkx = set.nkx;
                    memcpy(g.gB, set.gB, sizeof g.gB); memcpy(g.gX, set.gX, sizeof g.gX); memcpy(g.gN, set.gN, sizeof g.gN);
                    memcpy(g.gS, set.gS, sizeof g.gS);
                    CK(cudaMemsetAsync(qbuf->p, 0, qbytes, s));
                }
                const size_t smem = blockdft_tc_smem_bytes();
                CK(cudaFuncSetAttribute(blockdft_tc_kernel, cudaFuncAttributeMaxDynamicSharedMemorySize, (int)smem));
                const long long n_tiles = (long long)((nb + TC_BM - 1) / TC_BM) * n_ch * set.n_halves;
                if (n_tiles > 2147483647LL) return fail(OMEGA4_ERR_INVALID, "blockdft grid too large");
                g.n_tiles = (int)n_tiles;
                static int n_sm = 0;
                if (!n_sm) { int dev = 0; CK(cudaGetDevice(&dev)); CK(cudaDeviceGetAttribute(&n_sm, cudaDevAttrMultiProcessorCount, dev)); }
                const bool persistent = !getenv("OMEGA4_TC_ONE_TILE_PER_CTA");
                const long long grid = persistent ? std::min<long long>(n_tiles, n_sm) : n_tiles;
                Bracket b(p, s, timing, "blockdft_tc_gemm");
                blockdft_tc_kernel<<<(unsigned)grid, TC_CTA_THREADS, smem, s>>>(g);
                CK(cudaGetLastError());
#ifdef TC_TIMELINE
                {
                    static long long h[64][16];
                    CK(cudaStreamSynchronize(s));
                    CK(cudaMemcpyFromSymbol(h, tc_tl, sizeof h));
                    const int n = (int)std::min<long long>(64, (grid + 3) / 4);
                    const char* nm[12] = {"wait_empty+operands", "mma_issue_loop", "commit->full_seen", "tmem_drain", "epilogue_rest", "tile_period",
                                          "cg2 wait::ld", "cg2 acc+sts", "cg2 ld issue", "cg2 bar1", "cg2 sums", "cg2 bar2"};
                    const int from[12] = {0, 1, 2, 3, 4, 0, 8, 9, 10, 11, 12, 13}, to[12] = {1, 2, 3, 4, 5, 6, 9, 10, 11, 12, 13, 14};
                    for (int k = 0; k < 12; ++k) {
                        std::vector<long long> d;
                        for (int i = 0; i < n; ++i) d.push_back(h[i][to[k]] - h[i][from[k]]);
                        std::sort(d.begin(), d.end());
                        fprintf(stderr, "tc_timeline %-20s median %lld  p10 %lld  p90 %lld\n", nm[k], d[n / 2], d[n / 10], d[n * 9 / 10]);
                    }
                }
#endif
            } else {
                BlockDftGemmArgs g;
                memset(&g, 0, sizeof g);
                g.x = x; g.ch_stride = ch_stride; g.hop = p->hop; g.n_ch = n_ch; g.j0 = j0; g.nb = nb;
                g.E = set.E; g.Q = (float*)qbuf->p;
                Bracket b(p, s, timing, "blockdft_gemm");
                rc = launch_blockdft_gemm(set.qs, g, s);
                if (rc) return rc;
            }
        }
        for (int r = 0; r < p->n_res; ++r) {
            if (!use_sparse[r]) continue;
            const ResInfo& ri = p->res[r];
            const SparseRes& sp = set.sp[set.of_res[r]];
            if (sp.td && fusedx) {
                BlockDftFinishArgs a;
                memset(&a, 0, sizeof a);
                a.X = (const float2*)Q; a.nkx = set.nkx; a.xoff = sp.xoff; a.nk = sp.nk; a.kw = sp.kw;
                a.n_ch = n_ch; a.n_frames = n_hops; a.first_frame = first[r];
                a.comb_out = combined; a.Tbins = p->T; a.n_tb = ri.n_tb; a.tb_idx = ri.tb_idx; a.tb_pos = sp.tb_pos;
                a.tb_frac = ri.tb_frac; a.wnum = ri.weight; a.wden = ri.weight;
                const size_t smem = blockdft_finish_smem_bytes(sp.nk);
                CK(cudaFuncSetAttribute(blockdft_finish_kernel, cudaFuncAttributeMaxDynamicSharedMemorySize, (int)smem));
                const long long grid = (long long)((n_hops + BD_FIN_FRAMES - 1) / BD_FIN_FRAMES) * n_ch;
                if (grid > 2147483647LL) return fail(OMEGA4_ERR_INVALID, "blockdft finish grid too large");
                char name[32];
                snprintf(name, sizeof name, "blockdft_asm_%d", ri.n);
                Bracket b(p, s, timing, name);
                blockdft_finish_kernel<<<(unsigned)grid, 256, smem, s>>>(a);
                CK(cudaGetLastError());
                continue;
            }
            if (sp.td) {
                BlockDftSumArgs a;
                memset(&a, 0, sizeof a);
                a.Q = Q; a.qs = set.qs; a.col0 = sp.col0; a.nb = nb > 0 ? nb : 0; a.j0 = j0;
                a.nk = sp.nk; a.B = sp.B; a.kw = sp.kw;
                a.n_ch = n_ch; a.n_frames = n_hops; a.first_frame = first[r];
                a.comb_out = combined; a.Tbins = p->T; a.n_tb = ri.n_tb; a.tb_idx = ri.tb_idx; a.tb_pos = sp.tb_pos;
                a.tb_frac = ri.tb_frac; a.wnum = ri.weight; a.wden = ri.weight;
                a.fa = blockdft_sum_frames(sp.nk, sp.B);
                const size_t smem = blockdft_sum_smem_bytes(sp.nk, sp.B, a.fa);
                CK(cudaFuncSetAttribute(blockdft_sum_kernel, cudaFuncAttributeMaxDynamicSharedMemorySize, (int)smem));
                const long long grid = (long long)((n_hops + a.fa - 1) / a.fa) * n_ch;
                if (grid > 2147483647LL) return fail(OMEGA4_ERR_INVALID, "blockdft assemble grid too large");
                char name[32];
                snprintf(name, sizeof name, "blockdft_asm_%d", ri.n);
                Bracket b(p, s, timing, name);
                blockdft_sum_kernel<<<(unsigned)grid, 256, smem, s>>>(a);
                CK(cudaGetLastError());
                continue;
            }
            BlockDftAsmArgs a;
            memset(&a, 0, sizeof a);
            a.Q = Q; a.qs = set.qs; a.col0 = sp.col0; a.nb = nb > 0 ? nb : 0; a.j0 = j0;
            a.nk = sp.nk; a.nt = sp.nt; a.B = sp.B; a.T = sp.T; a.kw = sp.kw;
            a.n_ch = n_ch; a.n_frames = n_hops; a.first_frame = first[r];
            a.comb_out = combined; a.Tbins = p->T; a.n_tb = ri.n_tb; a.tb_idx = ri.tb_idx; a.tb_pos = sp.tb_pos;
            a.tb_frac = ri.tb_frac; a.wnum = ri.weight; a.wden = ri.weight;
            a.fa = blockdft_assemble_frames(sp.nk, sp.nt, sp.B);
            const size_t smem = blockdft_assemble_smem_bytes(sp.nk, sp.nt, sp.B, a.fa);
            auto kern = sp.nt == 5 ? blockdft_assemble_kernel<5> : (sp.nt == 3 ? blockdft_assemble_kernel<3> : blockdft_assemble_kernel<1>);
            CK(cudaFuncSetAttribute(kern, cudaFuncAttributeMaxDynamicSharedMemorySize, (int)smem));
            const long long grid = (long long)((n_hops + a.fa - 1) / a.fa) * n_ch;
            if (grid > 2147483647LL) return fail(OMEGA4_ERR_INVALID, "blockdft assemble grid too large");
            char name[32];
            snprintf(name, sizeof name, "blockdft_asm_%d", ri.n);
            Bracket b(p, s, timing, name);
            kern<<<(unsigned)grid, 256, smem, s>>>(a);
            CK(cudaGetLastError());
        }
    }
    if (combined && !fused) {
        CombineArgs c;
        memset(&c, 0, sizeof c);
        for (int r = 0; r < p->n_res; ++r) {
            c.mag[r] = mag_ptr[r]; c.bins[r] = p->res[r].bins; c.first_frame[r] = first[r]; c.weight[r] = p->res[r].weight;
        }
        c.n_hops = n_hops; c.n_rows = n_ch * n_hops; c.T = p->T;
        c.csr_ptr = p->csr_ptr; c.csr_res = p->csr_res; c.csr_lo = p->csr_lo; c.csr_frac = p->csr_frac;
        c.out = combined;
        const long long total = (long long)c.n_rows * c.T;
        Bracket b(p, s, timing, "combine");
        combine_kernel<<<(unsigned)((total + 255) / 256), 256, 0, s>>>(c);
        CK(cudaGetLastError());
    }
    if (concurrent || stats_aside) CK(cudaStreamWaitEvent(s, sc->ev_join, 0));
    return OMEGA4_OK;
}

static int analyze_any(omega4_plan* p, void* stream, int mem, const float* samples, const int16_t* s16, int il,
                       long long ch_stride, int n_ch, int n_hops, int hist_samples, float* combined,
                       float* const* magnitudes, float* meters, double* lufs_inst, double* tp_db,
                       double* meter_state, int flags, const BarsReq* br = nullptr) {
    if (!p) return fail(OMEGA4_ERR_INVALID, "plan is NULL");
    if (br && !br->b) br = nullptr;
    if (br) {
        if (!br->band_values) return fail(OMEGA4_ERR_INVALID, "band_values is NULL");
        if (br->b->device != p->device || br->b->T != p->T)
            return fail(OMEGA4_ERR_INVALID, "the bars object must live on the plan's device and take spectra of target_bins values");
    }
    if ((!samples && !s16) || n_ch < 0 || n_hops < 0 || hist_samples < 0) return fail(OMEGA4_ERR_INVALID, "bad samples / sizes");
    if (s16 && (il < 1 || il > 64 || n_ch % il != 0)) return fail(OMEGA4_ERR_INVALID, "bad interleave");
    if (n_ch == 0 || n_hops == 0) return OMEGA4_OK;
    CK(cudaSetDevice(p->device));
    cudaStream_t s = (cudaStream_t)stream;
    if (mem == OMEGA4_MEM_DEVICE) {
        if (s16) {
            const long long hist_al = ((long long)hist_samples + 3) / 4 * 4;
            const long long len = (long long)hist_samples + (long long)n_hops * p->hop;
            const long long dstride = (hist_al + (long long)n_hops * p->hop + 3) / 4 * 4;
            int rc = p->scratch_f32.ensure((size_t)n_ch * dstride * sizeof(float)); if (rc) return rc;
            float* d_in = (float*)p->scratch_f32.p;
            p->launches++;
            rc = launch_s16_convert(s16 - (long long)hist_samples * il, ch_stride, il, n_ch / il, len,
                                    d_in + (hist_al - hist_samples), dstride, s);
            if (rc) return rc;
            samples = d_in + hist_al; ch_stride = dstride;
        }
        float* d_comb = combined;
        if (br && !d_comb) {
            int rc = p->scratch_comb.ensure((size_t)n_ch * n_hops * p->T * sizeof(float)); if (rc) return rc;
            d_comb = (float*)p->scratch_comb.p;
        }
        int rc = analyze_device(p, s, samples, ch_stride, n_ch, n_hops, hist_samples, d_comb, magnitudes, meters,
                                lufs_inst, tp_db, meter_state, flags, &p->scratch_q, &p->sc);
        if (rc || !br) return rc;
        p->launches++;
        return bars_launch(br->b, s, d_comb, n_ch, n_hops, br->state, br->fresh, br->band_values, br->peak_values, &p->scratch_bstate);
    }
    if (mem != OMEGA4_MEM_HOST) return fail(OMEGA4_ERR_INVALID, "mem must be OMEGA4_MEM_HOST or OMEGA4_MEM_DEVICE");

    CK(cudaStreamSynchronize(s));
    const long long hist = hist_samples;
    const long long hist_al = (hist + 3) / 4 * 4;
    const long long new_len = (long long)n_hops * p->hop;
    const long long dstride = (hist_al + new_len + 3) / 4 * 4;
    size_t per_ch = (size_t)dstride * sizeof(float) + (size_t)n_hops * 2 * sizeof(double) + ST_STATE * sizeof(double);
    if (combined || br) per_ch += (size_t)n_hops * p->T * sizeof(float);
    if (br) per_ch += (size_t)n_hops * br->b->n_valid * sizeof(float) * (br->peak_values ? 2 : 1);
    {
        const bool tensor_sel = p->set_tc.n > 0 && (p->tensor_default ? !(flags & OMEGA4_FLAG_NO_TENSOR) : (flags & OMEGA4_FLAG_TENSOR) != 0);
        const SparseSet& sset = tensor_sel ? p->set_tc : p->set_cc;
        if ((combined || br) && sset.n > 0 && !(flags & OMEGA4_FLAG_NO_BLOCKDFT))
            per_ch += (tensor_sel && sset.fusable) ? (size_t)(n_hops + 64) * sset.nkx * sizeof(float2)
                                                   : (size_t)(n_hops + 64) * sset.qs * sizeof(float);
    }
    if (meters) per_ch += (size_t)n_hops * 5 * sizeof(float);
    bool want_mag[OMEGA4_MAX_RES] = {false};
    for (int r = 0; r < p->n_res; ++r) {
        want_mag[r] = (magnitudes && magnitudes[r]) || ((combined || br) && !p->disjoint);
        if (want_mag[r]) per_ch += (size_t)n_hops * p->res[r].bins * sizeof(float);
    }
    if (s16) per_ch += (size_t)(hist + new_len) * sizeof(int16_t);
    int chunk = (int)(p->host_chunk_bytes / per_ch);
    if (chunk < 1) chunk = 1;
    if (chunk > n_ch) chunk = n_ch;
    if (s16) { chunk = chunk / il * il; if (chunk < il) chunk = il; }
    const bool want_series = meters || lufs_inst || tp_db;
    int idx = 0;
    for (int c0 = 0; c0 < n_ch; c0 += chunk, ++idx) {
        const int nc = (n_ch - c0 < chunk) ? n_ch - c0 : chunk;
        omega4_plan::Slot& sl = p->slots[idx % omega4_plan::N_SLOTS];
        if (!sl.s) CK(cudaStreamCreateWithFlags(&sl.s, cudaStreamNonBlocking));
        const size_t rows = (size_t)nc * n_hops;
        int rc = sl.in.ensure((size_t)nc * dstride * sizeof(float)); if (rc) return rc;
        float* d_in = (float*)sl.in.p;
        if (s16) {
            const int ns = nc / il;
            const size_t row16 = (size_t)(hist + new_len) * il;
            rc = sl.in16.ensure((size_t)ns * row16 * sizeof(int16_t)); if (rc) return rc;
            CK(cudaMemcpy2DAsync(sl.in16.p, row16 * sizeof(int16_t),
                                 s16 + (long long)(c0 / il) * ch_stride - hist * il, ch_stride * sizeof(int16_t),
                                 row16 * sizeof(int16_t), ns, cudaMemcpyHostToDevice, sl.s));
            p->launches++;
            rc = launch_s16_convert((const int16_t*)sl.in16.p, (long long)row16, il, ns, hist + new_len,
                                    d_in + (hist_al - hist), dstride, sl.s);
            if (rc) return rc;
        } else {
            CK(cudaMemcpy2DAsync(d_in + (hist_al - hist), dstride * sizeof(float),
                                 samples + (long long)c0 * ch_stride - hist, ch_stride * sizeof(float),
                                 (size_t)(hist + new_len) * sizeof(float), nc, cudaMemcpyHostToDevice, sl.s));
        }
        float* d_comb = nullptr; float* d_met = nullptr; double* d_state = nullptr;
        double* d_lufs = nullptr; double* d_tp = nullptr;
        float* d_mag[OMEGA4_MAX_RES] = {nullptr};
        if (combined || br) { rc = sl.comb.ensure(rows * p->T * sizeof(float)); if (rc) return rc; d_comb = (float*)sl.comb.p; }
        float* d_bars = nullptr; float* d_peaks = nullptr; float* d_bstate = nullptr;
        const size_t bst_row = br ? (size_t)(1 + br->b->n_valid) : 0;
        if (br) {
            rc = sl.bars.ensure(rows * br->b->n_valid * sizeof(float)); if (rc) return rc; d_bars = (float*)sl.bars.p;
            if (br->peak_values) { rc = sl.peaks.ensure(rows * br->b->n_valid * sizeof(float)); if (rc) return rc; d_peaks = (float*)sl.peaks.p; }
            if (br->state) {
                rc = sl.bstate.ensure((size_t)nc * bst_row * sizeof(float)); if (rc) return rc; d_bstate = (float*)sl.bstate.p;
                if (!br->fresh)
                    CK(cudaMemcpyAsync(d_bstate, br->state + (size_t)c0 * bst_row, (size_t)nc * bst_row * sizeof(float), cudaMemcpyHostToDevice, sl.s));
            }
        }
        if (meters) { rc = sl.met.ensure(rows * 5 * sizeof(float)); if (rc) return rc; d_met = (float*)sl.met.p; }
        if (want_series) {
            rc = sl.lufs.ensure(rows * sizeof(double)); if (rc) return rc; d_lufs = (double*)sl.lufs.p;
            rc = sl.tp.ensure(rows * sizeof(double)); if (rc) return rc; d_tp = (double*)sl.tp.p;
        }
        if (meters) {
            rc = sl.state.ensure((size_t)nc * ST_STATE * sizeof(double)); if (rc) return rc;
            d_state = (double*)sl.state.p;
            if (meter_state && !(flags & OMEGA4_FLAG_FRESH_METERS))
                CK(cudaMemcpyAsync(d_state, meter_state + (size_t)c0 * ST_STATE, (size_t)nc * ST_STATE * sizeof(double),
                                   cudaMemcpyHostToDevice, sl.s));
        }
        bool any_mag = false;
        for (int r = 0; r < p->n_res; ++r)
            if (want_mag[r]) {
                rc = sl.mag[r].ensure(rows * p->res[r].bins * sizeof(float)); if (rc) return rc;
                d_mag[r] = (float*)sl.mag[r].p; any_mag = true;
            }
        const int fl = (flags & ~OMEGA4_FLAG_CONCURRENT_METERS) | ((meter_state == nullptr) ? OMEGA4_FLAG_FRESH_METERS : 0);
        rc = analyze_device(p, sl.s, d_in + hist_al, dstride, nc, n_hops, (int)hist, d_comb, any_mag ? d_mag : nullptr,
                            d_met, d_lufs, d_tp, d_state, fl, &sl.q, &sl.sc);
        if (rc) return rc;
        const size_t r0 = (size_t)c0 * n_hops;
        if (br) {
            p->launches++;
            rc = bars_launch(br->b, sl.s, d_comb, nc, n_hops, d_bstate, br->fresh, d_bars, d_peaks, &sl.bstate_copy);
            if (rc) return rc;
            const size_t nv = (size_t)br->b->n_valid;
            CK(cudaMemcpyAsync(br->band_values + r0 * nv, d_bars, rows * nv * sizeof(float), cudaMemcpyDeviceToHost, sl.s));
            if (br->peak_values) CK(cudaMemcpyAsync(br->peak_values + r0 * nv, d_peaks, rows * nv * sizeof(float), cudaMemcpyDeviceToHost, sl.s));
            if (br->state) CK(cudaMemcpyAsync(br->state + (size_t)c0 * bst_row, d_bstate, (size_t)nc * bst_row * sizeof(float), cudaMemcpyDeviceToHost, sl.s));
        }
        if (combined) CK(cudaMemcpyAsync(combined + r0 * p->T, d_comb, rows * p->T * sizeof(float), cudaMemcpyDeviceToHost, sl.s));
        if (meters) CK(cudaMemcpyAsync(meters + r0 * 5, d_met, rows * 5 * sizeof(float), cudaMemcpyDeviceToHost, sl.s));
        if (lufs_inst) CK(cudaMemcpyAsync(lufs_inst + r0, d_lufs, rows * sizeof(double), cudaMemcpyDeviceToHost, sl.s));
        if (tp_db) CK(cudaMemcpyAsync(tp_db + r0, d_tp, rows * sizeof(double), cudaMemcpyDeviceToHost, sl.s));
        if (meters && meter_state)
            CK(cudaMemcpyAsync(meter_state + (size_t)c0 * ST_STATE, d_state, (size_t)nc * ST_STATE * sizeof(double),
                               cudaMemcpyDeviceToHost, sl.s));
        if (magnitudes)
            for (int r = 0; r < p->n_res; ++r)
                if (magnitudes[r])
                    CK(cudaMemcpyAsync(magnitudes[r] + r0 * p->res[r].bins, d_mag[r], rows * p->res[r].bins * sizeof(float),
                                       cudaMemcpyDeviceToHost, sl.s));
    }
    for (auto& sl : p->slots)
        if (sl.s) CK(cudaStreamSynchronize(sl.s));
    return OMEGA4_OK;
}

extern "C" int omega4_analyze(omega4_plan* p, void* stream, int mem, const float* samples, long long ch_stride,
                              int n_ch, int n_hops, int hist_samples, float* combined, float* const* magnitudes,
                              float* meters, double* lufs_inst, double* tp_db, double* meter_state, int flags) {
    if (!samples) return fail(OMEGA4_ERR_INVALID, "bad samples / sizes");
    return analyze_any(p, stream, mem, samples, nullptr, 1, ch_stride, n_ch, n_hops, hist_samples, combined, magnitudes,
                       meters, lufs_inst, tp_db, meter_state, flags);
}

extern "C" int omega4_analyze_s16(omega4_plan* p, void* stream, int mem, const int16_t* frames, long long stream_stride,
                                  int n_streams, int n_interleaved, int n_hops, int hist_frames, float* combined,
                                  float* const* magnitudes, float* meters, double* lufs_inst, double* tp_db,
                                  double* meter_state, int flags) {
    if (!frames || n_streams < 0 || n_interleaved < 1) return fail(OMEGA4_ERR_INVALID, "bad frames / sizes");
    if (mem == OMEGA4_MEM_DEVICE && ((uintptr_t)frames & 1)) return fail(OMEGA4_ERR_INVALID, "frames must be 2-byte aligned");
    return analyze_any(p, stream, mem, nullptr, frames, n_interleaved, stream_stride, n_streams * n_interleaved, n_hops,
                       hist_frames, combined, magnitudes, meters, lufs_inst, tp_db, meter_state, flags);
}

extern "C" int omega4_analyze_io(omega4_plan* p, void* stream, int mem, const omega4_io* io) {
    if (!io) return fail(OMEGA4_ERR_INVALID, "io is NULL");
    if ((io->samples != nullptr) == (io->frames_s16 != nullptr))
        return fail(OMEGA4_ERR_INVALID, "exactly one of samples / frames_s16 must be given");
    BarsReq br;
    br.b = io->bars; br.band_values = io->band_values; br.peak_values = io->peak_values; br.state = io->bars_state;
    br.fresh = (!io->bars_state || (io->flags & OMEGA4_FLAG_FRESH_BARS)) ? 1 : 0;
    if (io->frames_s16) {
        if (io->n_interleaved < 1 || io->n_ch % io->n_interleaved != 0) return fail(OMEGA4_ERR_INVALID, "bad interleave");
        if (mem == OMEGA4_MEM_DEVICE && ((uintptr_t)io->frames_s16 & 1)) return fail(OMEGA4_ERR_INVALID, "frames must be 2-byte aligned");
        return analyze_any(p, stream, mem, nullptr, io->frames_s16, io->n_interleaved, io->stride, io->n_ch, io->n_hops, io->hist,
                           io->combined, io->magnitudes, io->meters, io->lufs_inst, io->tp_db, io->meter_state, io->flags, &br);
    }
    return analyze_any(p, stream, mem, io->samples, nullptr, 1, io->stride, io->n_ch, io->n_hops, io->hist, io->combined,
                       io->magnitudes, io->meters, io->lufs_inst, io->tp_db, io->meter_state, io->flags, &br);
}

struct StreamCtx {
    cudaStream_t s = nullptr;
    float* h_in = nullptr; float* h_out = nullptr;
    size_t h_in_cap = 0, h_out_cap = 0;
    DevBuf d_in, d_out;
    double* h64 = nullptr; size_t h64_cap = 0;
    DevBuf d64;
    std::map<unsigned, cudaGraphExec_t> graphs;
    std::set<unsigned> seen;
    void drop_graphs() { for (auto& kv : graphs) cudaGraphExecDestroy(kv.second); graphs.clear(); seen.clear(); }
    int ensure(size_t in_bytes, size_t out_bytes) {
        if (!s) CK(cudaStreamCreateWithFlags(&s, cudaStreamNonBlocking));
        if (in_bytes > h_in_cap) { if (h_in) cudaFreeHost(h_in); h_in = nullptr; h_in_cap = 0; CK(cudaMallocHost(&h_in, in_bytes)); h_in_cap = in_bytes; }
        if (out_bytes > h_out_cap) { if (h_out) cudaFreeHost(h_out); h_out = nullptr; h_out_cap = 0; CK(cudaMallocHost(&h_out, out_bytes)); h_out_cap = out_bytes; }
        int rc = d_in.ensure(in_bytes); if (rc) return rc;
        return d_out.ensure(out_bytes);
    }
    int ensure64(size_t bytes) {
        if (!s) CK(cudaStreamCreateWithFlags(&s, cudaStreamNonBlocking));
        if (bytes > h64_cap) { if (h64) cudaFreeHost(h64); h64 = nullptr; h64_cap = 0; CK(cudaMallocHost(&h64, bytes)); h64_cap = bytes; }
        return d64.ensure(bytes);
    }
    void release() {
        drop_graphs();
        if (h_in) cudaFreeHost(h_in); if (h_out) cudaFreeHost(h_out); if (h64) cudaFreeHost(h64);
        d_in.release(); d_out.release(); d64.release();
        if (s) cudaStreamDestroy(s);
        h_in = h_out = nullptr; h64 = nullptr; s = nullptr; h_in_cap = h_out_cap = h64_cap = 0;
    }
};
// ... 577 lines not shown
```

### audio-analyzer-omega_b200/csrc/truepeak16_kernel.cuh

```cuda
#pragma once
#include <cuda_fp16.h>
#include "truepeak_kernel.cuh"

namespace o4 {

struct c2h { __half2 x, y; };

__device__ __forceinline__ c2h hc_add(c2h a, c2h b) { c2h r; r.x = __hadd2(a.x, b.x); r.y = __hadd2(a.y, b.y); return r; }
__device__ __forceinline__ c2h hc_sub(c2h a, c2h b) { c2h r; r.x = __hsub2(a.x, b.x); r.y = __hsub2(a.y, b.y); return r; }
__device__ __forceinline__ c2h hc_mul_mi(c2h a) { c2h r; r.x = a.y; r.y = __hneg2(a.x); return r; }
__device__ __forceinline__ c2h hc_mul(c2h a, __half2 w) {
    const __half2 wr = __low2half2(w), wi = __high2half2(w);
    c2h r;
    r.x = __hfma2(a.x, wr, __hneg2(__hmul2(a.y, wi)));
    r.y = __hfma2(a.x, wi, __hmul2(a.y, wr));
    return r;
}
__device__ __forceinline__ c2h hc_mul_c(c2h a, float cr, float ci) { return hc_mul(a, __floats2half2_rn(cr, ci)); }
__device__ __forceinline__ c2h hc_rot_m45(c2h a) {
    const __half2 r = __float2half2_rn(0.70710678118654752440f);
    c2h o; o.x = __hmul2(__hadd2(a.x, a.y), r); o.y = __hmul2(__hsub2(a.y, a.x), r); return o;
}
__device__ __forceinline__ c2h hc_rot_m135(c2h a) {
    const __half2 r = __float2half2_rn(0.70710678118654752440f);
    c2h o; o.x = __hmul2(__hsub2(a.y, a.x), r); o.y = __hneg2(__hmul2(__hadd2(a.x, a.y), r)); return o;
}

__device__ __forceinline__ void hbf4(c2h& x0, c2h& x1, c2h& x2, c2h& x3) {
    const c2h a = hc_add(x0, x2), b = hc_sub(x0, x2), c = hc_add(x1, x3), d = hc_mul_mi(hc_sub(x1, x3));
    x0 = hc_add(a, c); x1 = hc_add(b, d); x2 = hc_sub(a, c); x3 = hc_sub(b, d);
}
__device__ __forceinline__ void hbf8(c2h* v) {
    c2h e0 = v[0], e1 = v[2], e2 = v[4], e3 = v[6];
    c2h o0 = v[1], o1 = v[3], o2 = v[5], o3 = v[7];
    hbf4(e0, e1, e2, e3);
    hbf4(o0, o1, o2, o3);
    o1 = hc_rot_m45(o1);
    o2 = hc_mul_mi(o2);
    o3 = hc_rot_m135(o3);
    v[0] = hc_add(e0, o0); v[4] = hc_sub(e0, o0);
    v[1] = hc_add(e1, o1); v[5] = hc_sub(e1, o1);
    v[2] = hc_add(e2, o2); v[6] = hc_sub(e2, o2);
    v[3] = hc_add(e3, o3); v[7] = hc_sub(e3, o3);
}
__device__ __forceinline__ void hbf16(c2h* v) {
    const float c1 = 0.92387953251128675613f, s1 = 0.38268343236508977173f;
#pragma unroll
    for (int a = 0; a < 4; ++a) hbf4(v[a], v[a + 4], v[a + 8], v[a + 12]);
    v[1 + 4] = hc_mul_c(v[1 + 4], c1, -s1);
    v[1 + 8] = hc_rot_m45(v[1 + 8]);
    v[1 + 12] = hc_mul_c(v[1 + 12], s1, -c1);
    v[2 + 4] = hc_rot_m45(v[2 + 4]);
    v[2 + 8] = hc_mul_mi(v[2 + 8]);
    v[2 + 12] = hc_rot_m135(v[2 + 12]);
    v[3 + 4] = hc_mul_c(v[3 + 4], s1, -c1);
    v[3 + 8] = hc_rot_m135(v[3 + 8]);
    v[3 + 12] = hc_mul_c(v[3 + 12], -c1, s1);
#pragma unroll
    for (int c = 0; c < 4; ++c) hbf4(v[4 * c], v[4 * c + 1], v[4 * c + 2], v[4 * c + 3]);
#pragma unroll
    for (int c = 0; c < 4; ++c)
#pragma unroll
        for (int d = c + 1; d < 4; ++d) { const c2h tmp = v[4 * c + d]; v[4 * c + d] = v[4 * d + c]; v[4 * d + c] = tmp; }
}
struct TwH15 { __half2 w[15]; };
struct LocalTwH { TwH15 s1, s2; };
__device__ __forceinline__ void h_apply_twiddles(c2h* v, const TwH15& t) {
#pragma unroll
    for (int k = 1; k < 16; ++k) v[k] = hc_mul(v[k], t.w[k - 1]);
}
template <int LOG2M>
__device__ __forceinline__ void pack_local_twiddles(const LocalTwFull<LOG2M>& a, LocalTwH& o) {
#pragma unroll
    for (int k = 0; k < 15; ++k) {
        o.s1.w[k] = __floats2half2_rn(a.s1.w[k].x, a.s1.w[k].y);
        o.s2.w[k] = __floats2half2_rn(a.s2.w[k].x, a.s2.w[k].y);
    }
}

template <int LOG2M, class TW>
__device__ __forceinline__ void fft_local_h2(c2h* v, c2h* X, const TW& st, int t, int g) {
    constexpr int M = 1 << LOG2M, TPF = M / 16, G2 = M / 256, S = 17 * G2;
    static_assert(G2 == 8, "written for 2048 complex points");
    hbf16(v);
    h_apply_twiddles(v, st.s1);
#pragma unroll
    for (int k = 0; k < 16; ++k) X[k * S + t] = v[k];
    group_sync<TPF>(g);
    const int q = t / G2, p = t % G2;
    c2h* Xq = X + q * S;
#pragma unroll
    for (int j = 0; j < 16; ++j) v[j] = Xq[p + G2 * j];
    hbf16(v);
    h_apply_twiddles(v, st.s2);
    __syncwarp();
#pragma unroll
    for (int k = 0; k < 16; ++k) Xq[17 * p + k] = v[k];
    __syncwarp();
#pragma unroll
    for (int i = 0; i < 16 / G2; ++i) {
        const int k = p + G2 * i;
#pragma unroll
        for (int pp = 0; pp < G2; ++pp) v[i * G2 + pp] = Xq[17 * pp + k];
        hbf8(v + i * 8);
    }
}

template <int LOG2M, class TW>
__device__ __forceinline__ void fft_forward_h2_z(c2h* v, c2h* X, c2h* Zc, const TW& st, int t, int g) {
    constexpr int M = 1 << LOG2M, TPF = M / 16, G2 = M / 256, S = 17 * G2;
    static_assert(G2 == 8, "written for 2048 complex points");
    hbf16(v);
    h_apply_twiddles(v, st.s1);
#pragma unroll
    for (int k = 0; k < 16; ++k) X[k * S + t] = v[k];
    group_sync<TPF>(g);
    const int q = t / G2, p = t % G2;
    const int zq = zaddr<LOG2M>(q + 16 * p);
    c2h* Xq = X + q * S;
#pragma unroll
    for (int j = 0; j < 16; ++j) v[j] = Xq[p + G2 * j];
    hbf16(v);
    h_apply_twiddles(v, st.s2);
    __syncwarp();
#pragma unroll
    for (int k = 0; k < 16; ++k) Xq[17 * p + k] = v[k];
    __syncwarp();
#pragma unroll
    for (int i = 0; i < 16 / G2; ++i) {
        const int k = p + G2 * i;
#pragma unroll
        for (int pp = 0; pp < G2; ++pp) v[i * G2 + pp] = Xq[17 * pp + k];
        hbf8(v + i * 8);
#pragma unroll
        for (int pq = 0; pq < G2; ++pq) Zc[zq + 16 * G2 * i + 256 * pq] = v[i * G2 + pq];
    }
    group_sync<TPF>(g);
}

template <int LOG2M>
__global__ void __launch_bounds__(256, 2)
truepeak16_kernel(const __grid_constant__ TruePeakArgs a) {
    using S = FftShape<LOG2M>;
    constexpr int M = S::M, TPF = S::TPF, CONC = S::CONC, BUF = S::BUF;
    constexpr int WARPS = TPF / 32;
    static_assert(TPF >= 32 && S::NT == 256 && LOG2M == 11, "true-peak kernel: 2048 complex points, whole warps per transform");
    extern __shared__ __align__(16) unsigned char smem_raw[];
    float2* bufs = reinterpret_cast<float2*>(smem_raw);
    float4* red_all = reinterpret_cast<float4*>(bufs + (size_t)CONC * (BUF + M));

    const int tid = threadIdx.x;
    const int g = tid / TPF;
    const int t = tid % TPF;
    c2h* Xh = reinterpret_cast<c2h*>(bufs + (size_t)g * (BUF + M));
    c2h* Zc = Xh + BUF;
    float4* red = red_all + g * 2 * WARPS;

    const int pairs_per_cta = a.rounds * CONC;
    const int n_pairs = (a.n_frames + 1) >> 1;
    const int tiles_per_ch = (n_pairs + pairs_per_cta - 1) / pairs_per_cta;
    const int ch = blockIdx.x / tiles_per_ch;
    const int tile = blockIdx.x % tiles_per_ch;

    LocalTwH st;
    {
        LocalTw<LOG2M> st4;
        LocalTwFull<LOG2M> stf;
        load_local_twiddles<LOG2M>(st4, a.twM, t);
        expand_local_twiddles<LOG2M>(st4, stf);
        pack_local_twiddles<LOG2M>(stf, st);
    }
    const float inv_m = 1.0f / (float)M;
    auto group_max4 = [&](float4 v, int slot) -> float4 {
#pragma unroll
        for (int o = 16; o > 0; o >>= 1) {
            v.x = fmaxf(v.x, __shfl_xor_sync(0xffffffffu, v.x, o));
            v.y = fmaxf(v.y, __shfl_xor_sync(0xffffffffu, v.y, o));
            v.z = fmaxf(v.z, __shfl_xor_sync(0xffffffffu, v.z, o));
            v.w = fmaxf(v.w, __shfl_xor_sync(0xffffffffu, v.w, o));
        }
        if ((t & 31) == 0) red[slot * WARPS + (t >> 5)] = v;
        group_sync<TPF>(g);
        float4 m = red[slot * WARPS];
#pragma unroll
        for (int w = 1; w < WARPS; ++w) {
            const float4 o = red[slot * WARPS + w];
            m.x = fmaxf(m.x, o.x); m.y = fmaxf(m.y, o.y); m.z = fmaxf(m.z, o.z); m.w = fmaxf(m.w, o.w);
        }
        return m;
    };

    const int zt = zaddr<LOG2M>(t);
    auto load_pair = [&](int pi, float2 (&v)[16], bool& act_a, bool& act_b) {
        const int fa = 2 * pi, fb = fa + 1;
        act_a = (fa < a.n_frames) && (fa >= a.first_frame);
        act_b = (fb < a.n_frames) && (fb >= a.first_frame);
#pragma unroll
        for (int j = 0; j < 16; ++j) v[j] = make_float2(0.f, 0.f);
        if (!(act_a || act_b)) return;
        const float* pa = reinterpret_cast<const float*>(a.x) + (long long)ch * a.ch_stride + a.frame_off0 + (long long)fa * a.frame_stride + t;
        const float* pb = pa + a.frame_stride;
#pragma unroll
        for (int j = 0; j < 16; ++j) {
            if (act_a) v[j].x = __ldg(pa + j * TPF);
            if (act_b) v[j].y = __ldg(pb + j * TPF);
        }
        if (a.window) {
#pragma unroll
            for (int j = 0; j < 16; ++j) { const float w = __ldg(a.window + t + j * TPF); v[j].x *= w; v[j].y *= w; }
        }
    };

    for (int u = 0; 2 * u < a.rounds; ++u) {
        const int pa_i = tile * pairs_per_cta + (2 * u) * CONC + g;
        const int pb_i = tile * pairs_per_cta + (2 * u + 1) * CONC + g;
        const bool has_b = (2 * u + 1) < a.rounds;
        bool aa, ab, ba = false, bb = false;
        float4 pk4 = make_float4(0.f, 0.f, 0.f, 0.f);
        c2h h[16];
        {
            float2 va[16], vb[16];
            load_pair(pa_i, va, aa, ab);
            if (has_b) load_pair(pb_i, vb, ba, bb);
            else {
#pragma unroll
                for (int j = 0; j < 16; ++j) vb[j] = make_float2(0.f, 0.f);
            }
#pragma unroll
            for (int j = 0; j < 16; ++j) {
                pk4.x = fmaxf(pk4.x, fabsf(va[j].x)); pk4.y = fmaxf(pk4.y, fabsf(va[j].y));
                pk4.z = fmaxf(pk4.z, fabsf(vb[j].x)); pk4.w = fmaxf(pk4.w, fabsf(vb[j].y));
            }
            pk4 = group_max4(pk4, 0);
            const float s0 = pk4.x > 1e-20f ? 1.f / pk4.x : 0.f, s1 = pk4.y > 1e-20f ? 1.f / pk4.y : 0.f;
            const float s2 = pk4.z > 1e-20f ? 1.f / pk4.z : 0.f, s3 = pk4.w > 1e-20f ? 1.f / pk4.w : 0.f;
#pragma unroll
            for (int j = 0; j < 16; ++j) {
                h[j].x = __floats2half2_rn(va[j].x * s0, vb[j].x * s2);
                h[j].y = __floats2half2_rn(va[j].y * s1, vb[j].y * s3);
            }
        }
        __half2 mre = __float2half2_rn(0.f), mim = mre;
        if (aa || ab || ba || bb) {
            fft_forward_h2_z<LOG2M>(h, Xh, Zc, st, t, g);
#pragma unroll 1
            for (int p = 1; p <= 3; ++p) {
                const unsigned* rot_p = a.rot_h + (p - 1) * M + t;
#pragma unroll
                for (int j = 0; j < 16; ++j) {
                    const unsigned rku = __ldg(rot_p + j * TPF);
                    const __half2 rkh = *reinterpret_cast<const __half2*>(&rku);
                    const c2h s = hc_mul(Zc[zt + j * TPF], rkh);
                    h[j].x = s.x; h[j].y = __hneg2(s.y);
                }
                fft_local_h2<LOG2M>(h, Xh, st, t, g);
#pragma unroll
                for (int j = 0; j < 16; ++j) { mre = __hmax2(mre, __habs2(h[j].x)); mim = __hmax2(mim, __habs2(h[j].y)); }
                group_sync<TPF>(g);
            }
        }
        const float2 fre = __half22float2(mre), fim = __half22float2(mim);
        const float4 pko = group_max4(make_float4(fre.x, fim.x, fre.y, fim.y), 1);
        if (t == 0) {
            const float pk[4] = {pk4.x, pk4.y, pk4.z, pk4.w};
            const float po[4] = {pko.x, pko.y, pko.z, pko.w};
            const bool act[4] = {aa, ab, ba, bb};
            const int fr[4] = {2 * pa_i, 2 * pa_i + 1, 2 * pb_i, 2 * pb_i + 1};
#pragma unroll
            for (int i = 0; i < 4; ++i) {
                if (!act[i]) continue;
                const double peak = (double)pk[i] * (double)fmaxf(1.f, po[i] * inv_m);
                a.tp_out[(size_t)ch * a.n_frames + fr[i]] = (peak < 1e-10) ? -100.0 : 20.0 * log10(peak);
            }
        }
        group_sync<TPF>(g);
    }
}

template <int LOG2M>
inline size_t truepeak16_smem_bytes() {
    using S = FftShape<LOG2M>;
    return (size_t)S::CONC * (S::BUF + S::M) * sizeof(float2) + (size_t)S::CONC * 2 * (S::TPF / 32) * sizeof(float4) + 16;
}

}
```

### audio-analyzer-omega_b200/csrc/truepeak_kernel.cuh

```cuda
#pragma once
#include "fft_core.cuh"

namespace o4 {

struct TruePeakArgs {
    const void* x;
    int x_is_f64;
    long long ch_stride;
    long long frame_stride;
    long long frame_off0;
    int n_ch;
    int n_frames;
    int first_frame;
    int rounds;
    const float* window;
    const float2* twM;
    const float2* rot;
    const unsigned* rot_h;
    double* tp_out;
    float2 step[3][16];
    float nyq[3];
};

template <int LOG2M>
__global__ void __launch_bounds__(256, 2)
truepeak_kernel(const __grid_constant__ TruePeakArgs a) {
    using S = FftShape<LOG2M>;
    constexpr int M = S::M, TPF = S::TPF, CONC = S::CONC, BUF = S::BUF;
    constexpr int WARPS = TPF / 32;
    static_assert(TPF >= 32 && S::NT == 256 && LOG2M <= 12, "true-peak kernel: whole warps per transform, local FFT variant");
    extern __shared__ __align__(16) unsigned char smem_raw[];
    float2* bufs = reinterpret_cast<float2*>(smem_raw);
    float2* red_all = bufs + (size_t)CONC * (BUF + M);

    const int tid = threadIdx.x;
    const int g = tid / TPF;
    const int t = tid % TPF;
    float2* X = bufs + (size_t)g * (BUF + M);
    float2* Z = X + BUF;
    float2* red = red_all + g * 2 * WARPS;

    const int pairs_per_cta = a.rounds * CONC;
    const int n_pairs = (a.n_frames + 1) >> 1;
    const int tiles_per_ch = (n_pairs + pairs_per_cta - 1) / pairs_per_cta;
    const int ch = blockIdx.x / tiles_per_ch;
    const int tile = blockIdx.x % tiles_per_ch;

    LocalTwFull<LOG2M> st;
    {
        LocalTw<LOG2M> st4;
        load_local_twiddles<LOG2M>(st4, a.twM, t);
        expand_local_twiddles<LOG2M>(st4, st);
    }
    const float inv_m = 1.0f / (float)M;
    auto nop = []() {};
    auto group_max2 = [&](float2 v, int slot) -> float2 {
#pragma unroll
        for (int o = 16; o > 0; o >>= 1) {
            v.x = fmaxf(v.x, __shfl_xor_sync(0xffffffffu, v.x, o));
            v.y = fmaxf(v.y, __shfl_xor_sync(0xffffffffu, v.y, o));
        }
        if ((t & 31) == 0) red[slot * WARPS + (t >> 5)] = v;
        group_sync<TPF>(g);
        float2 m = red[slot * WARPS];
#pragma unroll
        for (int w = 1; w < WARPS; ++w) { const float2 o = red[slot * WARPS + w]; m.x = fmaxf(m.x, o.x); m.y = fmaxf(m.y, o.y); }
        return m;
    };

    const int zt = zaddr<LOG2M>(t);
    const float2 rbase1 = __ldg(a.rot + t), rbase2 = __ldg(a.rot + M + t), rbase3 = __ldg(a.rot + 2 * M + t);
    auto load_pair = [&](int pi, float2 (&v)[16]) {
        const int fa = 2 * pi, fb = fa + 1;
        const bool act_a = (fa < a.n_frames) && (fa >= a.first_frame);
        const bool act_b = (fb < a.n_frames) && (fb >= a.first_frame);
#pragma unroll
        for (int j = 0; j < 16; ++j) v[j] = make_float2(0.f, 0.f);
        if (!(act_a || act_b)) return;
        const long long off_a = (long long)ch * a.ch_stride + a.frame_off0 + (long long)fa * a.frame_stride + t;
        if (a.x_is_f64) {
            const double* pa = reinterpret_cast<const double*>(a.x) + off_a;
            const double* pb = pa + a.frame_stride;
#pragma unroll
            for (int j = 0; j < 16; ++j) {
                if (act_a) v[j].x = (float)pa[j * TPF];
                if (act_b) v[j].y = (float)pb[j * TPF];
            }
        } else {
            const float* pa = reinterpret_cast<const float*>(a.x) + off_a;
            const float* pb = pa + a.frame_stride;
#pragma unroll
            for (int j = 0; j < 16; ++j) {
                if (act_a) v[j].x = __ldg(pa + j * TPF);
                if (act_b) v[j].y = __ldg(pb + j * TPF);
            }
        }
    };
    float2 v[16];
    load_pair(tile * pairs_per_cta + g, v);
    for (int r = 0; r < a.rounds; ++r) {
        const int pi = tile * pairs_per_cta + r * CONC + g;
        const int fa = 2 * pi, fb = fa + 1;
        const bool act_a = (fa < a.n_frames) && (fa >= a.first_frame);
        const bool act_b = (fb < a.n_frames) && (fb >= a.first_frame);
        const bool active = act_a || act_b;
        if (a.window) {
#pragma unroll
            for (int j = 0; j < 16; ++j) { const float w = __ldg(a.window + t + j * TPF); v[j].x *= w; v[j].y *= w; }
        }
        float2 pk = make_float2(0.f, 0.f);
#pragma unroll
        for (int j = 0; j < 16; ++j) { pk.x = fmaxf(pk.x, fabsf(v[j].x)); pk.y = fmaxf(pk.y, fabsf(v[j].y)); }
        pk = group_max2(pk, 0);
        const float sa = pk.x > 1e-20f ? 1.f / pk.x : 0.f, sb = pk.y > 1e-20f ? 1.f / pk.y : 0.f;
#pragma unroll
        for (int j = 0; j < 16; ++j) { v[j].x *= sa; v[j].y *= sb; }
        fft_forward_local<LOG2M, false>(v, X, Z, st, t, g, active, nop);
        float2 pko = make_float2(0.f, 0.f);
#pragma unroll 1
        for (int p = 1; p <= 3; ++p) {
            if (active) {
                const float2 rb = (p == 1) ? rbase1 : (p == 2 ? rbase2 : rbase3);
#pragma unroll
                for (int j = 0; j < 16; ++j) {
                    const int k = t + j * TPF;
                    float2 rk = cmul(rb, a.step[p - 1][j]);
                    if (j == 8 && t == 0) rk = make_float2(a.nyq[p - 1], 0.f);
                    const float2 s = cmul(Z[zt + j * TPF], rk);
                    v[j] = make_float2(s.x, -s.y);
                }
            }
            fft_forward_local<LOG2M, true>(v, X, Z, st, t, g, active, nop);
            if (active) {
#pragma unroll
                for (int j = 0; j < 16; ++j) { pko.x = fmaxf(pko.x, fabsf(v[j].x)); pko.y = fmaxf(pko.y, fabsf(v[j].y)); }
            }
            group_sync<TPF>(g);
        }
        if (r + 1 < a.rounds) load_pair(tile * pairs_per_cta + (r + 1) * CONC + g, v);
        pko = group_max2(pko, 1);
        if (t == 0) {
            const float na = fmaxf(1.f, pko.x * inv_m), nb = fmaxf(1.f, pko.y * inv_m);
            if (act_a) {
                const double peak = (double)pk.x * (double)na;
                a.tp_out[(size_t)ch * a.n_frames + fa] = (peak < 1e-10) ? -100.0 : 20.0 * log10(peak);
            }
            if (act_b) {
                const double peak = (double)pk.y * (double)nb;
                a.tp_out[(size_t)ch * a.n_frames + fb] = (peak < 1e-10) ? -100.0 : 20.0 * log10(peak);
            }
        }
        group_sync<TPF>(g);
    }
}

template <int LOG2M>
inline size_t truepeak_smem_bytes() {
    using S = FftShape<LOG2M>;
    return (size_t)S::CONC * (S::BUF + S::M) * sizeof(float2) + (size_t)S::CONC * 2 * (S::TPF / 32) * sizeof(float2) + 16;
}

}
```

Before: 286,700.

## Overlap GEMM with K-weighting, move row-scale computation to true-peak, slim TC epilogue

Several changes land together. The per-hop row-scale (hop_inv) computation moves from the K-weighting kernel into the fp16 true-peak kernel, which now reduces it alongside its sample peak. The K-weighting kernel drops to fewer warps per CTA so one of its CTAs can sit beside the tensor-core GEMM, and a cross-stream event lets the GEMM overlap other work. The GEMM producer warps pack row scales as exponent bytes, software-pipeline global loads against shared-memory stores, and fix the stage index per producer group. The epilogue drains TMEM in 16-column chunks under an 80-register cap. These aim to cut serialization and register pressure, at the cost of more complex scheduling and possible spills.

```diff
diff --git a/audio-analyzer-omega_b200/csrc/blockdft_tc_kernel.cuh b/audio-analyzer-omega_b200/csrc/blockdft_tc_kernel.cuh
--- a/audio-analyzer-omega_b200/csrc/blockdft_tc_kernel.cuh
+++ b/audio-analyzer-omega_b200/csrc/blockdft_tc_kernel.cuh
@@ -118,15 +118,12 @@
     asm volatile("tcgen05.commit.cta_group::1.mbarrier::arrive::one.shared::cluster.b64 [%0];" ::"r"(tc_smem_u32(bar)) : "memory");
 }
 
-__device__ __forceinline__ void tc_tmem_ld32(uint32_t taddr, uint32_t (&v)[32]) {
+__device__ __forceinline__ void tc_tmem_ld16(uint32_t taddr, uint32_t (&v)[16]) {
     asm volatile(
-        "tcgen05.ld.sync.aligned.32x32b.x32.b32 "
-        "{%0, %1, %2, %3, %4, %5, %6, %7, %8, %9, %10, %11, %12, %13, %14, %15, "
-        "%16, %17, %18, %19, %20, %21, %22, %23, %24, %25, %26, %27, %28, %29, %30, %31}, [%32];"
+        "tcgen05.ld.sync.aligned.32x32b.x16.b32 "
+        "{%0, %1, %2, %3, %4, %5, %6, %7, %8, %9, %10, %11, %12, %13, %14, %15}, [%16];"
         : "=r"(v[0]), "=r"(v[1]), "=r"(v[2]), "=r"(v[3]), "=r"(v[4]), "=r"(v[5]), "=r"(v[6]), "=r"(v[7]),
-          "=r"(v[8]), "=r"(v[9]), "=r"(v[10]), "=r"(v[11]), "=r"(v[12]), "=r"(v[13]), "=r"(v[14]), "=r"(v[15]),
-          "=r"(v[16]), "=r"(v[17]), "=r"(v[18]), "=r"(v[19]), "=r"(v[20]), "=r"(v[21]), "=r"(v[22]), "=r"(v[23]),
-          "=r"(v[24]), "=r"(v[25]), "=r"(v[26]), "=r"(v[27]), "=r"(v[28]), "=r"(v[29]), "=r"(v[30]), "=r"(v[31])
+          "=r"(v[8]), "=r"(v[9]), "=r"(v[10]), "=r"(v[11]), "=r"(v[12]), "=r"(v[13]), "=r"(v[14]), "=r"(v[15])
         : "r"(taddr) : "memory");
 }
 
@@ -191,11 +188,14 @@
 #pragma unroll
         for (int q = 0; q < PER; ++q) {
             if (q >= nbin) break;
-            float2 u[B];
-#pragma unroll
-            for (int b = 0; b < B; ++b) u[b] = Sf[b * TC_XROW + q * B + b];
-#pragma unroll
-            for (int w = B / 2; w > 0; w >>= 1)
+            float2 u[B / 2];
+#pragma unroll
+            for (int b = 0; b < B / 2; ++b) {
+                const float2 lo = Sf[b * TC_XROW + q * B + b], hi = Sf[(b + B / 2) * TC_XROW + q * B + b + B / 2];
+                u[b] = make_float2(lo.x + hi.x, lo.y + hi.y);
+            }
+#pragma unroll
+            for (int w = B / 4; w > 0; w >>= 1)
 #pragma unroll
                 for (int b = 0; b < w; ++b) { u[b].x += u[b + w].x; u[b].y += u[b + w].y; }
             float2* dst = a.X + ((size_t)ch * a.nkx + xb0 + q) * a.n_frames + f;
@@ -205,7 +205,7 @@
     }
 }
 
-__global__ void __launch_bounds__(TC_CTA_THREADS, 1)
+__global__ void __maxnreg__(80)
 blockdft_tc_kernel(const __grid_constant__ BlockDftTcArgs a) {
     extern __shared__ __align__(16) uint8_t tc_smem_raw[];
     uint8_t* tiles = tc_smem_raw + ((1024u - (tc_smem_u32(tc_smem_raw) & 1023u)) & 1023u);
@@ -296,71 +296,73 @@
         constexpr int NQ = TC_BM * 4 / PGT;
         constexpr int PF4 = TC_F16 ? 2 : 1;
         const int pg = tid / PGT, tg = tid % PGT;
-        int a_off[NQ];
-#pragma unroll
-        for (int q = 0; q < NQ; ++q) a_off[q] = tc_sw64_offset((tg + PGT * q) >> 2, (tg + PGT * q) & 3);
-        int it = 0;
-        for (int tile = blockIdx.x; tile < a.n_tiles; tile += gridDim.x, ++it) {
+        static_assert((PGT / 4) % 8 == 0 && NQ % 4 == 0, "pieces of a thread must be whole swizzle row groups apart");
+        constexpr int NH = NQ / 2;
+        const int a_off0 = tc_sw64_offset(tg >> 2, tg & 3);
+        const int hop4 = a.hop / 4;
+        const int s = pg;
+        uint8_t* const st = tiles + s * TC_STAGE_BYTES;
+        for (int tile = blockIdx.x; tile < a.n_tiles; tile += gridDim.x) {
             const int bid = tile / a.n_halves;
             const int row0 = (bid % tiles_per_ch) * TC_BM;
             const int ch = bid / tiles_per_ch;
-            const float* xa = a.x + (long long)ch * a.ch_stride + (long long)a.j0 * a.hop;
-            const float4* a_src[NQ];
-            float sc[NQ];
+            const float4* xa = reinterpret_cast<const float4*>(a.x + (long long)ch * a.ch_stride + (long long)a.j0 * a.hop) +
+                               (tg & 3) * PF4;
+            const int src0 = (row0 + (tg >> 2)) * hop4;
+            const int src_last = (a.nb - 1) * hop4;
+            uint32_t sce[NQ / 4] = {};
 #pragma unroll
             for (int q = 0; q < NQ; ++q) {
-                const int p = tg + PGT * q;
-                int r = row0 + (p >> 2);
-                if (r >= a.nb) r = a.nb - 1;
-                a_src[q] = reinterpret_cast<const float4*>(xa + (long long)r * a.hop) + (p & 3) * PF4;
 #if TC_F16
-                sc[q] = __ldg(a.row_inv + (size_t)ch * a.nb + r);
-#else
-                sc[q] = 1.f;
-#endif
-            }
-#if TC_F16
-#pragma unroll
-            for (int q = 0; q < NQ; ++q) sc[q] = __uint_as_float(0x7F000000u - __float_as_uint(sc[q]));
-#endif
-            const int kcg0 = it * n_kc;
+                const int r = min(row0 + (tg >> 2) + q * (PGT / 4), a.nb - 1);
+                const uint32_t inv = __float_as_uint(__ldg(a.row_inv + (size_t)ch * a.nb + r));
+                sce[q / 4] |= ((0x7F000000u - inv) >> 23) << (8 * (q % 4));
+#else
+                sce[q / 4] |= 127u << (8 * (q % 4));
+#endif
+            }
+            const int kcg0 = (tile - (int)blockIdx.x) / (int)gridDim.x * n_kc;
             for (int kc = ((pg - kcg0) % TC_PG + TC_PG) % TC_PG; kc < n_kc; kc += TC_PG) {
                 const int kcg = kcg0 + kc;
-                const int s = kcg % TC_STAGES;
-                uint8_t* st = tiles + s * TC_STAGE_BYTES;
-                float4 cur[NQ][PF4];
+                const float4* xk = xa + kc * (TC_KC / 4);
+                auto load = [&](int q, float4 (&v)[PF4]) {
 #ifndef TC_EXPERIMENT_NO_LDG
 #pragma unroll
-                for (int q = 0; q < NQ; ++q)
-#pragma unroll
-                    for (int h = 0; h < PF4; ++h) cur[q][h] = __ldg(a_src[q] + kc * (TC_KC / 4) + h);
-#else
-#pragma unroll
-                for (int q = 0; q < NQ; ++q)
-#pragma unroll
-                    for (int h = 0; h < PF4; ++h) cur[q][h] = make_float4(0.f, 0.f, 0.f, 0.f);
-#endif
+                    for (int h = 0; h < PF4; ++h) v[h] = __ldg(xk + min(src0 + q * (PGT / 4) * hop4, src_last) + h);
+#else
+#pragma unroll
+                    for (int h = 0; h < PF4; ++h) v[h] = make_float4(0.f, 0.f, 0.f, 0.f);
+#endif
+                };
+                auto store = [&](int q, const float4 (&v)[PF4]) {
+                    uint8_t* dst = st + a_off0 + q * (PGT / 32) * 512;
+#if TC_F16
+                    const float sq = __uint_as_float(((sce[q / 4] >> (8 * (q % 4))) & 0xFFu) << 23);
+                    uint4 hi, lo;
+                    tc_split_h2(v[0].x * sq, v[0].y * sq, hi.x, lo.x);
+                    tc_split_h2(v[0].z * sq, v[0].w * sq, hi.y, lo.y);
+                    tc_split_h2(v[1].x * sq, v[1].y * sq, hi.z, lo.z);
+                    tc_split_h2(v[1].z * sq, v[1].w * sq, hi.w, lo.w);
+                    *reinterpret_cast<uint4*>(dst) = hi;
+                    *reinterpret_cast<uint4*>(dst + TC_A_BYTES) = lo;
+#else
+                    float4 hi, lo;
+                    hi.x = __uint_as_float(__float_as_uint(v[0].x) & 0xFFFFE000u); lo.x = v[0].x - hi.x;
+                    hi.y = __uint_as_float(__float_as_uint(v[0].y) & 0xFFFFE000u); lo.y = v[0].y - hi.y;
+                    hi.z = __uint_as_float(__float_as_uint(v[0].z) & 0xFFFFE000u); lo.z = v[0].z - hi.z;
+                    hi.w = __uint_as_float(__float_as_uint(v[0].w) & 0xFFFFE000u); lo.w = v[0].w - hi.w;
+                    *reinterpret_cast<float4*>(dst) = hi;
+                    *reinterpret_cast<float4*>(dst + TC_A_BYTES) = lo;
+#endif
+                };
+                float4 cur[NH][PF4];
+#pragma unroll
+                for (int q = 0; q < NH; ++q) load(q, cur[q]);
                 if (kcg >= TC_STAGES) tc_mbar_wait(bar_m + s, (uint32_t)(kcg / TC_STAGES - 1) & 1);
 #pragma unroll
-                for (int q = 0; q < NQ; ++q) {
-#if TC_F16
-                    uint4 hi, lo;
-                    tc_split_h2(cur[q][0].x * sc[q], cur[q][0].y * sc[q], hi.x, lo.x);
-                    tc_split_h2(cur[q][0].z * sc[q], cur[q][0].w * sc[q], hi.y, lo.y);
-                    tc_split_h2(cur[q][1].x * sc[q], cur[q][1].y * sc[q], hi.z, lo.z);
-                    tc_split_h2(cur[q][1].z * sc[q], cur[q][1].w * sc[q], hi.w, lo.w);
-                    *reinterpret_cast<uint4*>(st + a_off[q]) = hi;
-                    *reinterpret_cast<uint4*>(st + TC_A_BYTES + a_off[q]) = lo;
-#else
-                    float4 hi, lo;
-                    hi.x = __uint_as_float(__float_as_uint(cur[q][0].x) & 0xFFFFE000u); lo.x = cur[q][0].x - hi.x;
-                    hi.y = __uint_as_float(__float_as_uint(cur[q][0].y) & 0xFFFFE000u); lo.y = cur[q][0].y - hi.y;
-                    hi.z = __uint_as_float(__float_as_uint(cur[q][0].z) & 0xFFFFE000u); lo.z = cur[q][0].z - hi.z;
-                    hi.w = __uint_as_float(__float_as_uint(cur[q][0].w) & 0xFFFFE000u); lo.w = cur[q][0].w - hi.w;
-                    *reinterpret_cast<float4*>(st + a_off[q]) = hi;
-                    *reinterpret_cast<float4*>(st + TC_A_BYTES + a_off[q]) = lo;
-#endif
-                }
+                for (int q = 0; q < NH; ++q) { store(q, cur[q]); load(q + NH, cur[q]); }
+#pragma unroll
+                for (int q = 0; q < NH; ++q) store(q + NH, cur[q]);
                 asm volatile("fence.proxy.async.shared::cta;" ::: "memory");
                 __syncwarp();
                 if (lane == 0) tc_mbar_arrive(bar_a + s);
@@ -391,14 +393,15 @@
             tc_mbar_wait(bar_full, (uint32_t)it & 1);
             asm volatile("tcgen05.fence::after_thread_sync;" ::: "memory");
             TC_STAMP(it == 1 && tid == TC_WARP_EPI * 32, 3);
-            uint32_t v[32], c[32];
-            tc_tmem_ld32(taddr0, v);
-            tc_tmem_ld32(taddr0 + TC_BN, c);
+            uint32_t v[16], c[16];
+            tc_tmem_ld16(taddr0, v);
+            tc_tmem_ld16(taddr0 + TC_BN, c);
 #pragma unroll 1
-            for (int cg = 0; cg < NCG; ++cg) {
-                TC_STAMP(it == 1 && cg == 2 && tid == TC_WARP_EPI * 32, 8);
+            for (int hh = 0; hh < 2 * NCG; ++hh) {
+                const int cg = hh >> 1, part = hh & 1;
+                TC_STAMP(it == 1 && hh == 4 && tid == TC_WARP_EPI * 32, 8);
                 asm volatile("tcgen05.wait::ld.sync.aligned;" ::: "memory");
-                TC_STAMP(it == 1 && cg == 2 && tid == TC_WARP_EPI * 32, 9);
+                TC_STAMP(it == 1 && hh == 4 && tid == TC_WARP_EPI * 32, 9);
                 const int gi = half * (TC_BN / 32) + grp * NCG + cg;
                 const int B = a.X ? a.gB[gi] : 0;
 #ifdef TC_EXPERIMENT_NO_EPI
@@ -408,31 +411,32 @@
 #endif
                 if (a.X) {
                     if (live) {
-#pragma unroll
-                        for (int i = 0; i < 16; ++i)
-                            S[(r + TC_SPAD) * TC_XROW + i] = make_float2(tc_acc(v[2 * i], c[2 * i], rs), tc_acc(v[2 * i + 1], c[2 * i + 1], rs));
+                        float2* Sr = S + (r + TC_SPAD) * TC_XROW + part * 8;
+#pragma unroll
+                        for (int i = 0; i < 8; ++i)
+                            Sr[i] = make_float2(tc_acc(v[2 * i], c[2 * i], rs), tc_acc(v[2 * i + 1], c[2 * i + 1], rs));
                     }
                 } else if (row < a.nb) {
-                    float4* dst = reinterpret_cast<float4*>(qrow + (grp * NCG + cg) * 32);
-#pragma unroll
-                    for (int i = 0; i < 8; ++i)
+                    float4* dst = reinterpret_cast<float4*>(qrow + (grp * NCG + cg) * 32 + part * 16);
+#pragma unroll
+                    for (int i = 0; i < 4; ++i)
                         dst[i] = make_float4(tc_acc(v[4 * i], c[4 * i], rs), tc_acc(v[4 * i + 1], c[4 * i + 1], rs),
                                              tc_acc(v[4 * i + 2], c[4 * i + 2], rs), tc_acc(v[4 * i + 3], c[4 * i + 3], rs));
                 }
-                TC_STAMP(it == 1 && cg == 2 && tid == TC_WARP_EPI * 32, 10);
-                if (cg + 1 < NCG) {
-                    tc_tmem_ld32(taddr0 + (uint32_t)((cg + 1) * 32), v);
-                    tc_tmem_ld32(taddr0 + (uint32_t)(TC_BN + (cg + 1) * 32), c);
+                TC_STAMP(it == 1 && hh == 4 && tid == TC_WARP_EPI * 32, 10);
+                if (hh + 1 < 2 * NCG) {
+                    tc_tmem_ld16(taddr0 + (uint32_t)((hh + 1) * 16), v);
+                    tc_tmem_ld16(taddr0 + (uint32_t)(TC_BN + (hh + 1) * 16), c);
                 } else {
                     asm volatile("tcgen05.fence::before_thread_sync;" ::: "memory");
                     __syncwarp();
                     if (lane == 0) tc_mbar_arrive(bar_empty);
                     TC_STAMP(it == 1 && tid == TC_WARP_EPI * 32, 4);
                 }
-                if (a.X) {
-                    TC_STAMP(it == 1 && cg == 2 && tid == TC_WARP_EPI * 32, 11);
+                if (a.X && part == 1) {
+                    TC_STAMP(it == 1 && hh == 5 && tid == TC_WARP_EPI * 32, 11);
                     asm volatile("bar.sync %0, 128;" ::"r"(grp + 1) : "memory");
-                    TC_STAMP(it == 1 && cg == 2 && tid == TC_WARP_EPI * 32, 12);
+                    TC_STAMP(it == 1 && hh == 5 && tid == TC_WARP_EPI * 32, 12);
                     if (live) {
                         const int nbin = a.gN[gi], xb0 = a.gX[gi];
                         if (B == 16) tc_frame_sums<16>(a, S, r, row0, ch, nbin, xb0, a.gS[gi]);
@@ -440,9 +444,9 @@
                         else if (B == 4) tc_frame_sums<4>(a, S, r, row0, ch, nbin, xb0);
                         else tc_frame_sums<2>(a, S, r, row0, ch, nbin, xb0);
                     }
-                    TC_STAMP(it == 1 && cg == 2 && tid == TC_WARP_EPI * 32, 13);
+                    TC_STAMP(it == 1 && hh == 5 && tid == TC_WARP_EPI * 32, 13);
                     asm volatile("bar.sync %0, 128;" ::"r"(grp + 1) : "memory");
-                    TC_STAMP(it == 1 && cg == 2 && tid == TC_WARP_EPI * 32, 14);
+                    TC_STAMP(it == 1 && hh == 5 && tid == TC_WARP_EPI * 32, 14);
                 }
             }
             TC_STAMP(it == 1 && tid == TC_WARP_EPI * 32, 5);
@@ -454,6 +458,6 @@
         asm volatile("tcgen05.dealloc.cta_group::1.sync.aligned.b32 %0, %1;" ::"r"(tmem), "n"(TC_TMEM_COLS) : "memory");
 }
 
-inline size_t blockdft_tc_smem_bytes() { return (size_t)TC_STAGES * TC_STAGE_BYTES + (TC_EPI_WARPS / 4) * TC_STRIP_BYTES + (3 * TC_STAGES + 2) * 8 + 16 + 1024; }
-
-}
+constexpr size_t blockdft_tc_smem_bytes() { return (size_t)TC_STAGES * TC_STAGE_BYTES + (TC_EPI_WARPS / 4) * TC_STRIP_BYTES + (3 * TC_STAGES + 2) * 8 + 16 + 1024; }
+
+}
diff --git a/audio-analyzer-omega_b200/csrc/kweight32_kernel.cuh b/audio-analyzer-omega_b200/csrc/kweight32_kernel.cuh
--- a/audio-analyzer-omega_b200/csrc/kweight32_kernel.cuh
+++ b/audio-analyzer-omega_b200/csrc/kweight32_kernel.cuh
@@ -1,7 +1,6 @@
 #pragma once
 #include <cuda_runtime.h>
 #include "kweight_kernel.cuh"
-#include "blockdft_tc_kernel.cuh"
 
 namespace o4 {
 
@@ -20,8 +19,6 @@
     const float* hann;
     double* lufs_out;
     int rms_gate, _align;
-    float* hop_inv;
-    int hop_inv_nb, hop_inv_j0;
     Kw32Sec s[2];
 };
 
@@ -194,9 +191,14 @@
     }
 }
 
-constexpr int KW32_WARPS = 4;
+#ifndef KW32_WARPS
+#define KW32_WARPS 2
+#endif
 #ifndef KW32_MIN_BLOCKS
-#define KW32_MIN_BLOCKS 3
+#define KW32_MIN_BLOCKS (12 / KW32_WARPS)
+#endif
+#ifndef KW32_SMEM_PAD
+#define KW32_SMEM_PAD 0
 #endif
 
 __global__ void __launch_bounds__(KW32_WARPS * 32, KW32_MIN_BLOCKS)
@@ -229,15 +231,6 @@
         float4 tmp[KW_W / 4 / 32];
 #pragma unroll
         for (int j = 0; j < KW_W / 4 / 32; ++j) tmp[j] = __ldg(px + lane + 32 * j);
-        if (a.hop_inv) {
-            float m = 0.f;
-#pragma unroll
-            for (int j = 3 * KW_W / 4 / 4 / 32; j < KW_W / 4 / 32; ++j)
-                m = fmaxf(fmaxf(m, fmaxf(fabsf(tmp[j].x), fabsf(tmp[j].y))), fmaxf(fabsf(tmp[j].z), fabsf(tmp[j].w)));
-#pragma unroll
-            for (int o = 16; o > 0; o >>= 1) m = fmaxf(m, __shfl_xor_sync(0xffffffffu, m, o));
-            if (lane == 0) a.hop_inv[(size_t)ch * a.hop_inv_nb + (f - a.hop_inv_j0)] = hop_row_scale(m);
-        }
         if (lane < KW_PAD) stg[KW_STG_SHIFT + lane] = 0.f;
         if (lane < KW_SLACK + KW_PAD + KW_STG_SHIFT) stg[KW_STG_SHIFT + KW_PAD + KW_W + lane] = 0.f;
 #pragma unroll
@@ -295,8 +288,8 @@
     }
 }
 
-inline size_t kweight32_smem_bytes() {
-    return (size_t)32 * KW_L * sizeof(float) + (size_t)KW32_WARPS * KW_STG * sizeof(float);
-}
-
-}
+constexpr size_t kweight32_smem_bytes() {
+    return (size_t)32 * KW_L * sizeof(float) + (size_t)KW32_WARPS * KW_STG * sizeof(float) + KW32_SMEM_PAD;
+}
+
+}
diff --git a/audio-analyzer-omega_b200/csrc/omega4_cuda.cu b/audio-analyzer-omega_b200/csrc/omega4_cuda.cu
--- a/audio-analyzer-omega_b200/csrc/omega4_cuda.cu
+++ b/audio-analyzer-omega_b200/csrc/omega4_cuda.cu
@@ -27,6 +27,9 @@
 #include "waterfall_kernel.cuh"
 
 using namespace o4;
+
+static_assert(blockdft_tc_smem_bytes() + 1024 + kweight32_smem_bytes() + 1024 <= 233472,
+              "a K-weighting CTA no longer fits beside the tensor-core GEMM");
 
 static thread_local std::string g_err;
 
@@ -185,6 +188,7 @@
 static int launch_kweight32(const Kweight32Args& a, cudaStream_t s) {
     const size_t smem = kweight32_smem_bytes();
     CK(cudaFuncSetAttribute(kweight32_kernel, cudaFuncAttributeMaxDynamicSharedMemorySize, (int)smem));
+    CK(cudaFuncSetAttribute(kweight32_kernel, cudaFuncAttributePreferredSharedMemoryCarveout, cudaSharedmemCarveoutMaxShared));
     const int fpc = a.frames_per_warp * KW32_WARPS;
     const long long grid = (long long)((a.n_frames + fpc - 1) / fpc) * a.n_ch;
     if (grid <= 0) return OMEGA4_OK;
@@ -373,22 +377,27 @@
 struct KernelTime { char name[32]; cudaEvent_t e0, e1; };
 
 struct SideCtx {
-    cudaStream_t side = nullptr;
-    cudaEvent_t ev_fork = nullptr, ev_tp = nullptr, ev_join = nullptr;
+    cudaStream_t side = nullptr, gemm = nullptr;
+    cudaEvent_t ev_fork = nullptr, ev_tp = nullptr, ev_join = nullptr, ev_gemm = nullptr, ev_gemm_done = nullptr;
     int ensure() {
         if (side) return OMEGA4_OK;
+        int least = 0, greatest = 0;
+        CK(cudaDeviceGetStreamPriorityRange(&least, &greatest));
         CK(cudaStreamCreateWithFlags(&side, cudaStreamNonBlocking));
+        CK(cudaStreamCreateWithPriority(&gemm, cudaStreamNonBlocking, greatest));
         CK(cudaEventCreateWithFlags(&ev_fork, cudaEventDisableTiming));
         CK(cudaEventCreateWithFlags(&ev_tp, cudaEventDisableTiming));
         CK(cudaEventCreateWithFlags(&ev_join, cudaEventDisableTiming));
+        CK(cudaEventCreateWithFlags(&ev_gemm, cudaEventDisableTiming));
+        CK(cudaEventCreateWithFlags(&ev_gemm_done, cudaEventDisableTiming));
         return OMEGA4_OK;
     }
     void release() {
         if (side) cudaStreamDestroy(side);
-        if (ev_fork) cudaEventDestroy(ev_fork);
-        if (ev_tp) cudaEventDestroy(ev_tp);
-        if (ev_join) cudaEventDestroy(ev_join);
-        side = nullptr; ev_fork = ev_tp = ev_join = nullptr;
+        if (gemm) cudaStreamDestroy(gemm);
+        for (cudaEvent_t e : {ev_fork, ev_tp, ev_join, ev_gemm, ev_gemm_done})
+            if (e) cudaEventDestroy(e);
+        side = gemm = nullptr; ev_fork = ev_tp = ev_join = ev_gemm = ev_gemm_done = nullptr;
     }
 };
 
@@ -983,19 +992,112 @@
         if (use_sparse[r]) { const int j = first[r] + 1 - set.sp[set.of_res[r]].B; if (j < sp_j0) sp_j0 = j; }
     const int sp_nb = any_sparse ? n_hops - sp_j0 : 0;
     float* row_inv = nullptr;
-    int inv_from_kw = -1;
 #if TC_F16
     if (tensor && any_sparse && sp_nb > 0) {
         int rc = p->scratch_inv.ensure((size_t)n_ch * sp_nb * sizeof(float)); if (rc) return rc;
         row_inv = (float*)p->scratch_inv.p;
     }
 #endif
+    const int j0 = sp_j0, nb = sp_nb;
+    const bool fusedx = tensor && set.fusable;
+    const float* Q = nullptr;
+    size_t qbytes = 0;
+    if (any_sparse && nb > 0) {
+        qbytes = fusedx ? (size_t)n_ch * set.nkx * n_hops * sizeof(float2) : (size_t)n_ch * nb * set.qs * sizeof(float);
+        int rc = qbuf->ensure(qbytes);
+        if (rc) return rc;
+        Q = (float*)qbuf->p;
+    }
+    const long long need_m = (long long)p->W - hist;
+    const int first_m = need_m <= 0 ? 0 : (int)((need_m + p->hop - 1) / p->hop - 1);
+    const bool exact_tp = (flags & OMEGA4_FLAG_EXACT_TRUE_PEAK) || getenv("OMEGA4_TP_F32");
+    const int inv_from_tp = (want_meters && row_inv && !exact_tp && p->hop * 4 == p->W && first_m < n_hops && first_m >= j0 &&
+                             !getenv("OMEGA4_NO_SCALE_FOLD")) ? first_m : -1;
+    const bool overlap = tensor && any_sparse && nb > 0 && want_meters && !concurrent && use_kweight32(p);
+    if (overlap) { int rc = sc->ensure(); if (rc) return rc; }
+    auto launch_tc_gemm = [&](cudaStream_t gs) -> int {
+        BlockDftTcArgs g;
+        memset(&g, 0, sizeof g);
+        g.x = x; g.ch_stride = ch_stride; g.hop = p->hop; g.n_ch = n_ch; g.j0 = j0; g.nb = nb;
+        g.n_halves = set.n_halves; g.Eimg = set.Eimg; g.Q = (float*)qbuf->p; g.qs = set.qs;
+#if TC_F16
+        {
+            HopScaleArgs h;
+            h.x = x; h.ch_stride = ch_stride; h.hop = p->hop; h.n_ch = n_ch; h.j0 = j0; h.nb = nb;
+            h.ncols = inv_from_tp >= 0 ? inv_from_tp - j0 : nb;
+            h.inv = row_inv;
+            g.row_inv = h.inv; g.e_inv = set.e_inv;
+            const long long rows = (long long)n_ch * h.ncols;
+            if (rows > 0) {
+                Bracket b(p, gs, timing, "blockdft_row_scale");
+                hopblock_scale_kernel<<<(unsigned)((rows + 7) / 8), 256, 0, gs>>>(h);
+                CK(cudaGetLastError());
+            }
+        }
+#endif
+        if (fusedx) {
+            g.X = (float2*)qbuf->p; g.n_frames = n_hops; g.nkx = set.nkx;
+            memcpy(g.gB, set.gB, sizeof g.gB); memcpy(g.gX, set.gX, sizeof g.gX); memcpy(g.gN, set.gN, sizeof g.gN);
+            memcpy(g.gS, set.gS, sizeof g.gS);
+            CK(cudaMemsetAsync(qbuf->p, 0, qbytes, gs));
+        }
+        const size_t smem = blockdft_tc_smem_bytes();
+        CK(cudaFuncSetAttribute(blockdft_tc_kernel, cudaFuncAttributeMaxDynamicSharedMemorySize, (int)smem));
+        const long long n_tiles = (long long)((nb + TC_BM - 1) / TC_BM) * n_ch * set.n_halves;
+        if (n_tiles > 2147483647LL) return fail(OMEGA4_ERR_INVALID, "blockdft grid too large");
+        g.n_tiles = (int)n_tiles;
+        static int n_sm = 0;
+        if (!n_sm) { int dev = 0; CK(cudaGetDevice(&dev)); CK(cudaDeviceGetAttribute(&n_sm, cudaDevAttrMultiProcessorCount, dev)); }
+        const bool persistent = !getenv("OMEGA4_TC_ONE_TILE_PER_CTA");
+        const long long grid = persistent ? std::min<long long>(n_tiles, n_sm) : n_tiles;
+        Bracket b(p, gs, timing, "blockdft_tc_gemm");
+        blockdft_tc_kernel<<<(unsigned)grid, TC_CTA_THREADS, smem, gs>>>(g);
+        CK(cudaGetLastError());
+#ifdef TC_TIMELINE
+        {
+            static long long h[64][16];
+            CK(cudaStreamSynchronize(gs));
+            CK(cudaMemcpyFromSymbol(h, tc_tl, sizeof h));
+            const int n = (int)std::min<long long>(64, (grid + 3) / 4);
+            const char* nm[12] = {"wait_empty+operands", "mma_issue_loop", "commit->full_seen", "tmem_drain", "epilogue_rest", "tile_period",
+                                  "cg2 wait::ld", "cg2 acc+sts", "cg2 ld issue", "cg2 bar1", "cg2 sums", "cg2 bar2"};
+            const int from[12] = {0, 1, 2, 3, 4, 0, 8, 9, 10, 11, 12, 13}, to[12] = {1, 2, 3, 4, 5, 6, 9, 10, 11, 12, 13, 14};
+            for (int k = 0; k < 12; ++k) {
+                std::vector<long long> d;
+                for (int i = 0; i < n; ++i) d.push_back(h[i][to[k]] - h[i][from[k]]);
+                std::sort(d.begin(), d.end());
+                fprintf(stderr, "tc_timeline %-20s median %lld  p10 %lld  p90 %lld\n", nm[k], d[n / 2], d[n / 10], d[n * 9 / 10]);
+            }
+        }
+#endif
+        return OMEGA4_OK;
+    };
     if (want_meters) {
         const size_t nser = (size_t)n_ch * n_hops * sizeof(double);
         if (!lufs) { int rc = p->scratch_lufs.ensure(nser); if (rc) return rc; lufs = (double*)p->scratch_lufs.p; }
         if (!tp) { int rc = p->scratch_tp.ensure(nser); if (rc) return rc; tp = (double*)p->scratch_tp.p; }
-        long long need = (long long)p->W - hist;
-        const int first_m = need <= 0 ? 0 : (int)((need + p->hop - 1) / p->hop - 1);
+        {
+            TruePeakArgs t;
+            memset(&t, 0, sizeof t);
+            t.x = x; t.x_is_f64 = 0; t.ch_stride = ch_stride; t.frame_stride = p->hop;
+            t.frame_off0 = (long long)p->hop - p->W;
+            t.n_ch = n_ch; t.n_frames = n_hops; t.first_frame = first_m;
+            t.rounds = default_rounds((n_hops + 1) / 2, 2);
+            t.window = p->hann32; t.twM = p->tw_meter.twM; t.rot = p->tp_rot; t.rot_h = p->tp_rot_h;
+            fill_truepeak_steps(&t);
+            t.tp_out = tp;
+            if (inv_from_tp >= 0) { t.hop_inv = row_inv; t.hop_inv_nb = nb; t.hop_inv_j0 = j0; }
+            Bracket b(p, s, timing, "true_peak");
+            int rc = exact_tp ? launch_truepeak(t, s) : launch_truepeak16(t, s);
+            if (rc) return rc;
+        }
+        if (overlap) {
+            CK(cudaEventRecord(sc->ev_gemm, s));
+            CK(cudaStreamWaitEvent(sc->gemm, sc->ev_gemm, 0));
+            int rc = launch_tc_gemm(sc->gemm);
+            if (rc) return rc;
+            CK(cudaEventRecord(sc->ev_gemm_done, sc->gemm));
+        }
         if (use_kweight32(p)) {
             Kweight32Args k;
             memset(&k, 0, sizeof k);
@@ -1004,10 +1106,6 @@
             k.n_ch = n_ch; k.n_frames = n_hops; k.first_frame = first_m;
             k.frames_per_warp = n_hops >= 64 ? 8 : (n_hops >= 8 ? 2 : 1);
             k.hann = p->hann32; k.lufs_out = lufs; k.rms_gate = p->kw_gate;
-            if (row_inv && !concurrent && p->hop * 4 == p->W && first_m < n_hops && !getenv("OMEGA4_NO_SCALE_FOLD")) {
-                k.hop_inv = row_inv; k.hop_inv_nb = sp_nb; k.hop_inv_j0 = sp_j0;
-                inv_from_kw = first_m;
-            }
             build_kw32(p->kw[0], &k.s[0]); build_kw32(p->kw[1], &k.s[1]);
             Bracket b(p, ms, timing, "kweight_lufs");
             int rc = launch_kweight32(k, ms);
@@ -1023,21 +1121,6 @@
             fill_weighting(p, &k);
             Bracket b(p, ms, timing, "kweight_lufs");
             int rc = launch_kweight(k, ms);
-            if (rc) return rc;
-        }
-        {
-            TruePeakArgs t;
-            memset(&t, 0, sizeof t);
-            t.x = x; t.x_is_f64 = 0; t.ch_stride = ch_stride; t.frame_stride = p->hop;
-            t.frame_off0 = (long long)p->hop - p->W;
-            t.n_ch = n_ch; t.n_frames = n_hops; t.first_frame = first_m;
-            t.rounds = default_rounds((n_hops + 1) / 2, 2);
-            t.window = p->hann32; t.twM = p->tw_meter.twM; t.rot = p->tp_rot; t.rot_h = p->tp_rot_h;
-            fill_truepeak_steps(&t);
-            t.tp_out = tp;
-            Bracket b(p, s, timing, "true_peak");
-            const bool exact_tp = (flags & OMEGA4_FLAG_EXACT_TRUE_PEAK) || getenv("OMEGA4_TP_F32");
-            int rc = exact_tp ? launch_truepeak(t, s) : launch_truepeak16(t, s);
             if (rc) return rc;
         }
         if (meters) {
@@ -1091,80 +1174,21 @@
         if (rc) return rc;
     }
     if (any_sparse) {
-        const int j0 = sp_j0, nb = sp_nb;
-        const float* Q = nullptr;
-        const bool fusedx = tensor && set.fusable;
-        if (nb > 0) {
-            const size_t qbytes = fusedx ? (size_t)n_ch * set.nkx * n_hops * sizeof(float2)
-                                         : (size_t)n_ch * nb * set.qs * sizeof(float);
-            int rc = qbuf->ensure(qbytes);
-            if (rc) return rc;
-            Q = (float*)qbuf->p;
+        if (nb > 0 && !overlap) {
             if (tensor) {
-                BlockDftTcArgs g;
-                memset(&g, 0, sizeof g);
-                g.x = x; g.ch_stride = ch_stride; g.hop = p->hop; g.n_ch = n_ch; g.j0 = j0; g.nb = nb;
-                g.n_halves = set.n_halves; g.Eimg = set.Eimg; g.Q = (float*)qbuf->p; g.qs = set.qs;
-#if TC_F16
-                {
-                    HopScaleArgs h;
-                    h.x = x; h.ch_stride = ch_stride; h.hop = p->hop; h.n_ch = n_ch; h.j0 = j0; h.nb = nb;
-                    h.ncols = inv_from_kw >= 0 ? inv_from_kw - j0 : nb;
-                    h.inv = row_inv;
-                    g.row_inv = h.inv; g.e_inv = set.e_inv;
-                    const long long rows = (long long)n_ch * h.ncols;
-                    if (rows > 0) {
-                        Bracket b(p, s, timing, "blockdft_row_scale");
-                        hopblock_scale_kernel<<<(unsigned)((rows + 7) / 8), 256, 0, s>>>(h);
-                        CK(cudaGetLastError());
-                    }
-                }
-#endif
-                if (fusedx) {
-                    g.X = (float2*)qbuf->p; g.n_frames = n_hops; g.nkx = set.nkx;
-                    memcpy(g.gB, set.gB, sizeof g.gB); memcpy(g.gX, set.gX, sizeof g.gX); memcpy(g.gN, set.gN, sizeof g.gN);
-                    memcpy(g.gS, set.gS, sizeof g.gS);
-                    CK(cudaMemsetAsync(qbuf->p, 0, qbytes, s));
-                }
-                const size_t smem = blockdft_tc_smem_bytes();
-                CK(cudaFuncSetAttribute(blockdft_tc_kernel, cudaFuncAttributeMaxDynamicSharedMemorySize, (int)smem));
-                const long long n_tiles = (long long)((nb + TC_BM - 1) / TC_BM) * n_ch * set.n_halves;
-                if (n_tiles > 2147483647LL) return fail(OMEGA4_ERR_INVALID, "blockdft grid too large");
-                g.n_tiles = (int)n_tiles;
-                static int n_sm = 0;
-                if (!n_sm) { int dev = 0; CK(cudaGetDevice(&dev)); CK(cudaDeviceGetAttribute(&n_sm, cudaDevAttrMultiProcessorCount, dev)); }
-                const bool persistent = !getenv("OMEGA4_TC_ONE_TILE_PER_CTA");
-                const long long grid = persistent ? std::min<long long>(n_tiles, n_sm) : n_tiles;
-                Bracket b(p, s, timing, "blockdft_tc_gemm");
-                blockdft_tc_kernel<<<(unsigned)grid, TC_CTA_THREADS, smem, s>>>(g);
-                CK(cudaGetLastError());
-#ifdef TC_TIMELINE
-                {
-                    static long long h[64][16];
-                    CK(cudaStreamSynchronize(s));
-                    CK(cudaMemcpyFromSymbol(h, tc_tl, sizeof h));
-                    const int n = (int)std::min<long long>(64, (grid + 3) / 4);
-                    const char* nm[12] = {"wait_empty+operands", "mma_issue_loop", "commit->full_seen", "tmem_drain", "epilogue_rest", "tile_period",
-                                          "cg2 wait::ld", "cg2 acc+sts", "cg2 ld issue", "cg2 bar1", "cg2 sums", "cg2 bar2"};
-                    const int from[12] = {0, 1, 2, 3, 4, 0, 8, 9, 10, 11, 12, 13}, to[12] = {1, 2, 3, 4, 5, 6, 9, 10, 11, 12, 13, 14};
-                    for (int k = 0; k < 12; ++k) {
-                        std::vector<long long> d;
-                        for (int i = 0; i < n; ++i) d.push_back(h[i][to[k]] - h[i][from[k]]);
-                        std::sort(d.begin(), d.end());
-                        fprintf(stderr, "tc_timeline %-20s median %lld  p10 %lld  p90 %lld\n", nm[k], d[n / 2], d[n / 10], d[n * 9 / 10]);
-                    }
-                }
-#endif
+                int rc = launch_tc_gemm(s);
+                if (rc) return rc;
             } else {
                 BlockDftGemmArgs g;
                 memset(&g, 0, sizeof g);
                 g.x = x; g.ch_stride = ch_stride; g.hop = p->hop; g.n_ch = n_ch; g.j0 = j0; g.nb = nb;
                 g.E = set.E; g.Q = (float*)qbuf->p;
                 Bracket b(p, s, timing, "blockdft_gemm");
-                rc = launch_blockdft_gemm(set.qs, g, s);
+                int rc = launch_blockdft_gemm(set.qs, g, s);
                 if (rc) return rc;
             }
         }
+        if (overlap) CK(cudaStreamWaitEvent(s, sc->ev_gemm_done, 0));
         for (int r = 0; r < p->n_res; ++r) {
             if (!use_sparse[r]) continue;
             const ResInfo& ri = p->res[r];
diff --git a/audio-analyzer-omega_b200/csrc/truepeak16_kernel.cuh b/audio-analyzer-omega_b200/csrc/truepeak16_kernel.cuh
--- a/audio-analyzer-omega_b200/csrc/truepeak16_kernel.cuh
+++ b/audio-analyzer-omega_b200/csrc/truepeak16_kernel.cuh
@@ -1,6 +1,7 @@
 #pragma once
 #include <cuda_fp16.h>
 #include "truepeak_kernel.cuh"
+#include "blockdft_tc_kernel.cuh"
 
 namespace o4 {
 
@@ -154,7 +155,7 @@
     const int t = tid % TPF;
     c2h* Xh = reinterpret_cast<c2h*>(bufs + (size_t)g * (BUF + M));
     c2h* Zc = Xh + BUF;
-    float4* red = red_all + g * 2 * WARPS;
+    float4* red = red_all + g * 3 * WARPS;
 
     const int pairs_per_cta = a.rounds * CONC;
     const int n_pairs = (a.n_frames + 1) >> 1;
@@ -171,7 +172,7 @@
         pack_local_twiddles<LOG2M>(stf, st);
     }
     const float inv_m = 1.0f / (float)M;
-    auto group_max4 = [&](float4 v, int slot) -> float4 {
+    auto warp_max4 = [](float4& v) {
 #pragma unroll
         for (int o = 16; o > 0; o >>= 1) {
             v.x = fmaxf(v.x, __shfl_xor_sync(0xffffffffu, v.x, o));
@@ -179,8 +180,8 @@
             v.z = fmaxf(v.z, __shfl_xor_sync(0xffffffffu, v.z, o));
             v.w = fmaxf(v.w, __shfl_xor_sync(0xffffffffu, v.w, o));
         }
-        if ((t & 31) == 0) red[slot * WARPS + (t >> 5)] = v;
-        group_sync<TPF>(g);
+    };
+    auto slot_max4 = [&](int slot) -> float4 {
         float4 m = red[slot * WARPS];
 #pragma unroll
         for (int w = 1; w < WARPS; ++w) {
@@ -189,14 +190,26 @@
         }
         return m;
     };
+    auto group_max4 = [&](float4 v, int slot, float4& u, bool also) -> float4 {
+        warp_max4(v);
+        if (also) warp_max4(u);
+        if ((t & 31) == 0) {
+            red[slot * WARPS + (t >> 5)] = v;
+            if (also) red[2 * WARPS + (t >> 5)] = u;
+        }
+        group_sync<TPF>(g);
+        if (also && t == 0) u = slot_max4(2);
+        return slot_max4(slot);
+    };
 
     const int zt = zaddr<LOG2M>(t);
-    auto load_pair = [&](int pi, float2 (&v)[16], bool& act_a, bool& act_b) {
+    auto load_pair = [&](int pi, float2 (&v)[16], float2& hm, bool& act_a, bool& act_b) {
         const int fa = 2 * pi, fb = fa + 1;
         act_a = (fa < a.n_frames) && (fa >= a.first_frame);
         act_b = (fb < a.n_frames) && (fb >= a.first_frame);
 #pragma unroll
         for (int j = 0; j < 16; ++j) v[j] = make_float2(0.f, 0.f);
+        hm = make_float2(0.f, 0.f);
         if (!(act_a || act_b)) return;
         const float* pa = reinterpret_cast<const float*>(a.x) + (long long)ch * a.ch_stride + a.frame_off0 + (long long)fa * a.frame_stride + t;
         const float* pb = pa + a.frame_stride;
@@ -205,6 +218,8 @@
             if (act_a) v[j].x = __ldg(pa + j * TPF);
             if (act_b) v[j].y = __ldg(pb + j * TPF);
         }
+#pragma unroll
+        for (int j = 12; j < 16; ++j) { hm.x = fmaxf(hm.x, fabsf(v[j].x)); hm.y = fmaxf(hm.y, fabsf(v[j].y)); }
         if (a.window) {
 #pragma unroll
             for (int j = 0; j < 16; ++j) { const float w = __ldg(a.window + t + j * TPF); v[j].x *= w; v[j].y *= w; }
@@ -219,9 +234,9 @@
         float4 pk4 = make_float4(0.f, 0.f, 0.f, 0.f);
         c2h h[16];
         {
-            float2 va[16], vb[16];
-            load_pair(pa_i, va, aa, ab);
-            if (has_b) load_pair(pb_i, vb, ba, bb);
+            float2 va[16], vb[16], hma, hmb = make_float2(0.f, 0.f);
+            load_pair(pa_i, va, hma, aa, ab);
+            if (has_b) load_pair(pb_i, vb, hmb, ba, bb);
             else {
 #pragma unroll
                 for (int j = 0; j < 16; ++j) vb[j] = make_float2(0.f, 0.f);
@@ -231,7 +246,16 @@
                 pk4.x = fmaxf(pk4.x, fabsf(va[j].x)); pk4.y = fmaxf(pk4.y, fabsf(va[j].y));
                 pk4.z = fmaxf(pk4.z, fabsf(vb[j].x)); pk4.w = fmaxf(pk4.w, fabsf(vb[j].y));
             }
-            pk4 = group_max4(pk4, 0);
+            float4 hm4 = make_float4(hma.x, hma.y, hmb.x, hmb.y);
+            pk4 = group_max4(pk4, 0, hm4, a.hop_inv != nullptr);
+            if (a.hop_inv && t == 0) {
+                const float hm[4] = {hm4.x, hm4.y, hm4.z, hm4.w};
+                const bool act[4] = {aa, ab, ba, bb};
+                const int fr[4] = {2 * pa_i, 2 * pa_i + 1, 2 * pb_i, 2 * pb_i + 1};
+#pragma unroll
+                for (int i = 0; i < 4; ++i)
+                    if (act[i]) a.hop_inv[(size_t)ch * a.hop_inv_nb + (fr[i] - a.hop_inv_j0)] = hop_row_scale(hm[i]);
+            }
             const float s0 = pk4.x > 1e-20f ? 1.f / pk4.x : 0.f, s1 = pk4.y > 1e-20f ? 1.f / pk4.y : 0.f;
             const float s2 = pk4.z > 1e-20f ? 1.f / pk4.z : 0.f, s3 = pk4.w > 1e-20f ? 1.f / pk4.w : 0.f;
 #pragma unroll
@@ -260,7 +284,8 @@
             }
         }
         const float2 fre = __half22float2(mre), fim = __half22float2(mim);
-        const float4 pko = group_max4(make_float4(fre.x, fim.x, fre.y, fim.y), 1);
+        float4 unused;
+        const float4 pko = group_max4(make_float4(fre.x, fim.x, fre.y, fim.y), 1, unused, false);
         if (t == 0) {
             const float pk[4] = {pk4.x, pk4.y, pk4.z, pk4.w};
             const float po[4] = {pko.x, pko.y, pko.z, pko.w};
@@ -280,7 +305,7 @@
 template <int LOG2M>
 inline size_t truepeak16_smem_bytes() {
     using S = FftShape<LOG2M>;
-    return (size_t)S::CONC * (S::BUF + S::M) * sizeof(float2) + (size_t)S::CONC * 2 * (S::TPF / 32) * sizeof(float4) + 16;
-}
-
-}
+    return (size_t)S::CONC * (S::BUF + S::M) * sizeof(float2) + (size_t)S::CONC * 3 * (S::TPF / 32) * sizeof(float4) + 16;
+}
+
+}
diff --git a/audio-analyzer-omega_b200/csrc/truepeak_kernel.cuh b/audio-analyzer-omega_b200/csrc/truepeak_kernel.cuh
--- a/audio-analyzer-omega_b200/csrc/truepeak_kernel.cuh
+++ b/audio-analyzer-omega_b200/csrc/truepeak_kernel.cuh
@@ -20,6 +20,8 @@
     double* tp_out;
     float2 step[3][16];
     float nyq[3];
+    float* hop_inv;
+    int hop_inv_nb, hop_inv_j0;
 };
 
 template <int LOG2M>
```

Result: slower. 282,900, median of 6 (-1.3%).
